# NathanBWaters/playaid_core

Hardware: AMD Instinct MI355X
Metric: 1080p frames/sec end-to-end (higher is better)
Workload: dtype f32; 1 GPU; configs[1]: 64 x 1080x1920 BGR frames per GPU per clip; parallelism=single GPU, lanes=2, ingest=raw BGR frames resident in HBM

## Files before the change

include/playaid_hip.h:

```cpp
#ifndef PLAYAID_HIP_H
#define PLAYAID_HIP_H

#include <stddef.h>
#include <stdint.h>

#ifdef __cplusplus
extern "C" {
#endif

#define PA_ABI_VERSION 15
#define PA_WEIGHT_MAGIC 0x31574150
#define PA_LSTM_MAGIC 0x314c4150
#define PA_ENCODER_MAGIC 0x31454150
#define PA_FEATURE_STRIDE 1024
#define PA_CROP 128

typedef enum pa_status {
    PA_OK = 0,
    PA_ERR_INVALID_ARG = -1,
    PA_ERR_HIP = -2,
    PA_ERR_BAD_WEIGHTS = -3,
    PA_ERR_CAPACITY = -4,
    PA_ERR_NO_DEVICE = -5,
    PA_ERR_NOT_READY = -6,
// ... 142 lines not shown
int pa_detector_layer_forms(const pa_detector* h, int32_t* forms, int32_t cap);

int pa_clean_detections(pa_engine* e, const float* dets, const int32_t* counts, int32_t n_labels, int32_t max_det, int32_t n_decoded_frames,
                        double* labels, int32_t* pixel_frame, double* pixel_box, int32_t* crop_kind, float* crop_row, int32_t* info4,
                        void* stream);

int pa_detector_plan(pa_engine* e, const int32_t* pixel_frame, const double* pixel_box, const int32_t* crop_kind, const int32_t* info4,
                     int32_t n_labels, int32_t* det_index, int32_t* src_own, int32_t* rep_entry, double* rep_boxes, int32_t* rep_src,
                     int32_t* words5, void* stream);
int pa_detector_plan_desc(pa_engine* e, pa_crop_image* desc, const int32_t* crop_kind, int32_t n_frames, int32_t step_frames,
                          long long region_bytes, const int32_t* rep_entry, int32_t n_rep, long long rep_base, void* stream);
int pa_square_crops_src(pa_engine* e, const uint8_t* frames, int32_t n_src, int32_t height, int32_t width, const double* boxes,
                        const int32_t* src_frame, int32_t n, int32_t padding, int32_t swap_rb, uint8_t* crops, int32_t* status, void* stream);

int pa_save_one_box_crops(pa_engine* e, const uint8_t* frames, int32_t n_src, int32_t height, int32_t width, const float* dets,
                          const int32_t* counts, int32_t max_det, const int32_t* det_index, const int32_t* src_frame, int32_t n,
                          int32_t jpeg_quality, uint8_t* images, size_t images_capacity, pa_crop_image* desc, void* stream);

int pa_project_boxes(pa_engine* e, const double* log_rows, int32_t n_rows, double* boxes, void* stream);


int pa_clip_begin(pa_engine* e, int32_t clip_frames);
int pa_clip_begin_batch(pa_engine* e, int32_t n_clips, int32_t clip_frames);

int pa_backbone_frames(pa_engine* e, const uint8_t* frames, int32_t n, int32_t height, int32_t width,
                       const double* boxes, int32_t frame0, uint8_t* crops_rgb, int32_t* status,
                       void* stream);

int pa_preprocess_frames(pa_engine* e, const uint8_t* frames, int32_t n, int32_t height, int32_t width,
                         const double* boxes, int32_t slot, uint8_t* crops_rgb, int32_t* status,
                         void* stream);
int pa_backbone_slot(pa_engine* e, int32_t slot, int32_t n, int32_t frame0, void* stream);


typedef struct pa_crop_window {
    int64_t offset;
    int32_t pitch;
    int32_t rows;
    int64_t src_offset;
    int32_t src_pitch;
    int32_t row_bytes;
} pa_crop_window;
int pa_upload_crop_windows(pa_engine* e, const uint8_t* frames_host, int32_t n, int32_t height, int32_t width,
                           const double* boxes_host, int32_t padding, uint8_t* windows_dev, size_t windows_capacity,
                           pa_crop_window* desc_host, pa_crop_window* desc_dev, size_t* bytes_used, void* stream);
int pa_preprocess_windows(pa_engine* e, const uint8_t* windows_dev, const pa_crop_window* desc_dev, int32_t n, int32_t height,
                          int32_t width, const double* boxes, int32_t slot, uint8_t* crops_rgb, int32_t* status, void* stream);


typedef struct pa_mjpeg pa_mjpeg;
int pa_mjpeg_create(int32_t device, int32_t max_frames, int32_t max_height, int32_t max_width, size_t max_bytes, pa_mjpeg** out);
void pa_mjpeg_destroy(pa_mjpeg* h);
const char* pa_mjpeg_last_error(const pa_mjpeg* h);
int pa_mjpeg_probe(const uint8_t* data_host, size_t nbytes, int32_t* info8, char* why, size_t why_bytes);
int pa_mjpeg_set_sync_rounds(pa_mjpeg* h, int32_t rounds);
int pa_mjpeg_last_sync_rounds(const pa_mjpeg* h);
int pa_mjpeg_set_groups(pa_mjpeg* h, int32_t groups);
int pa_mjpeg_debug_counters(unsigned long long* out8_host);
int pa_mjpeg_decode(pa_mjpeg* h, const uint8_t* data_host, const int64_t* spans_host, int32_t n, int32_t height, int32_t width,
                    int32_t rgb, uint8_t* frames_dev, int32_t* status_dev, void* stream);


typedef struct pa_jpeg_file {
    int64_t offset;
    int32_t nbytes;
    int32_t reserved;
} pa_jpeg_file;
typedef struct pa_jpegenc pa_jpegenc;
int pa_jpegenc_create(int32_t device, int32_t max_images, int64_t max_blocks, size_t scratch_bytes, pa_jpegenc** out);
void pa_jpegenc_destroy(pa_jpegenc* h);
const char* pa_jpegenc_last_error(const pa_jpegenc* h);
int pa_jpeg_header(int32_t height, int32_t width, int32_t quality, int32_t subsampling, uint8_t* out_host, size_t cap, int32_t* nbytes);
size_t pa_jpeg_file_bytes_bound(int32_t height, int32_t width, int32_t subsampling);
int pa_jpegenc_encode(pa_jpegenc* h, const uint8_t* images, size_t images_bytes, const pa_crop_image* desc, int32_t n, int32_t max_height,
                      int32_t max_width, int32_t bgr, int32_t quality, int32_t subsampling, uint8_t* files, size_t files_capacity,
                      pa_jpeg_file* out, void* stream);
int pa_jpegenc_overflows(pa_jpegenc* h, int32_t* count_host, void* stream);


typedef struct pa_jpegdec pa_jpegdec;
int pa_jpegdec_create(int32_t device, int32_t max_images, int64_t max_blocks, size_t max_bytes, pa_jpegdec** out);
void pa_jpegdec_destroy(pa_jpegdec* h);
const char* pa_jpegdec_last_error(const pa_jpegdec* h);
int pa_jpegdec_set_sync_rounds(pa_jpegdec* h, int32_t rounds);
int pa_jpegdec_plan(const uint8_t* data_host, const int64_t* spans_host, int32_t n, pa_crop_image* desc_host, size_t* images_bytes,
                    int64_t* blocks, char* why, size_t why_bytes);
int pa_jpegdec_decode(pa_jpegdec* h, const uint8_t* data_host, const int64_t* spans_host, int32_t n, int32_t bgr, uint8_t* images_dev,
                      size_t images_capacity, pa_crop_image* desc_dev, int32_t* status_dev, void* stream);

int pa_backbone_frames_indexed(pa_engine* e, const uint8_t* frames, int32_t n, int32_t height, int32_t width,
                               const double* boxes, const int32_t* frame_ids, uint8_t* crops_rgb,
                               int32_t* status, void* stream);
int pa_clip_mark_ready(pa_engine* e, const int32_t* frame_ids_host, int32_t n);
int pa_device_errors(pa_engine* e, int32_t* bad_frame_ids_host, void* stream);

int pa_backbone_frames_src(pa_engine* e, const uint8_t* frames, int32_t n_src, int32_t height, int32_t width,
                           const double* boxes, const int32_t* src_frame, int32_t n, int32_t frame0,
                           uint8_t* crops_rgb, int32_t* status, void* stream);

int pa_head_frames(pa_engine* e, int32_t frame_num_lo, int32_t frame_num_hi, pa_record* records,
                   float* logp, void* stream);

int pa_infer_clip(pa_engine* e, const uint8_t* frames, int32_t n, int32_t height, int32_t width,
                  const double* boxes, pa_record* records, float* logp, uint8_t* crops_rgb,
                  int32_t* status, void* stream);

int pa_features_export(pa_engine* e, int32_t frame0, int32_t n, float* feats, void* stream);
int pa_features_import(pa_engine* e, int32_t frame0, int32_t n, const float* feats, void* stream);

int pa_crop_resize_width(pa_engine* e, const uint8_t* frames, int32_t n, int32_t height, int32_t width, const int32_t* rects_host,
                         int32_t n_rects, int32_t out_w, uint8_t* out, int32_t out_h_cap, int32_t* out_h_host, void* stream);

int pa_backbone_windows(pa_engine* e, const float* x, int32_t n_crops, float* feats, void* stream);

#define PA_TRACE_STAGES 20
int pa_backbone_trace(pa_engine* e, const float* x, int32_t n_crops, int32_t stage, void* out, size_t out_bytes, void* aux,
                      size_t aux_bytes, void* stream);

typedef struct pa_lstm pa_lstm;
size_t pa_lstm_blob_bytes(int32_t input_dim, int32_t hidden_dim, int32_t num_layers, int32_t num_actions);
int pa_lstm_create(int32_t device, int32_t input_dim, int32_t hidden_dim, int32_t num_layers, int32_t num_actions,
                   int32_t max_rows, const void* blob_host, size_t blob_bytes, pa_lstm** out);
void pa_lstm_destroy(pa_lstm* h);
const char* pa_lstm_last_error(const pa_lstm* h);
int pa_lstm_forward(pa_lstm* h, const float* x, int32_t ld, int32_t seq_len, int32_t batch, float* logp, void* stream);
int pa_lstm_last_status(pa_lstm* h);
typedef enum pa_lstm_form {
    PA_LSTM_FORM_NOT_RUN = 0,
    PA_LSTM_FORM_STEPS = 1,
    PA_LSTM_FORM_U1 = 2,
    PA_LSTM_FORM_U2 = 3,
    PA_LSTM_FORM_U4 = 4,
    PA_LSTM_FORM_U8 = 5,
    PA_LSTM_FORM_MFMA = 6
} pa_lstm_form;
int pa_lstm_layer_forms(const pa_lstm* h, int32_t* forms, int32_t cap);

typedef struct pa_conv_desc {
    int32_t kind;
    int32_t cin, cout;
    int32_t ksize, stride;
    int32_t in_hw;
    int32_t in_buf, in_pad;
    int32_t out_buf, out_pad;
    int32_t res_buf;
    int32_t relu;
    int64_t w_off, b_off;
} pa_conv_desc;
typedef struct pa_convnet pa_convnet;
int pa_convnet_create(int32_t device, const pa_conv_desc* descs, int32_t n_descs, const int64_t* buf_floats_per_crop,
                      int32_t n_bufs, const float* weights_host, size_t n_weights, int32_t max_crops, pa_convnet** out);
int pa_convnet_create_dtype(int32_t device, const pa_conv_desc* descs, int32_t n_descs, const int64_t* buf_floats_per_crop,
                            int32_t n_bufs, const float* weights_host, size_t n_weights, int32_t max_crops, int32_t compute_dtype,
                            pa_convnet** out);
void pa_convnet_destroy(pa_convnet* h);
const char* pa_convnet_last_error(const pa_convnet* h);
int pa_convnet_forward(pa_convnet* h, const float* x, int32_t n, float* out, int32_t out_floats_per_crop, void* stream);
int pa_convnet_trace(pa_convnet* h, const float* x, int32_t n, int32_t last_row, int32_t buf, void* out, size_t out_bytes, void* stream);
typedef enum pa_cn_form {
    PA_CN_FORM_NOT_RUN = 0,
    PA_CN_FORM_STEM_POOL = 1,
    PA_CN_FORM_AVGPOOL = 2,
    PA_CN_FORM_WINO = 3,
    PA_CN_FORM_PATCH = 4,
    PA_CN_FORM_IGEMM_128x128 = 5,
    PA_CN_FORM_IGEMM_128x64 = 6,
    PA_CN_FORM_IGEMM_64x64 = 7,
    PA_CN_FORM_PSGEMM = 8,
    PA_CN_FORM_BGEMM = 9,
    PA_CN_FORM_BGEMM_SPLITK = 10,
    PA_CN_FORM_AVGPOOL_BF16 = 11
} pa_cn_form;
#define PA_CN_FORM_STEM_POOL_ANY 12
int pa_convnet_layer_forms(const pa_convnet* h, int32_t* forms, int32_t cap);

size_t pa_wino_weight_floats(int32_t cin, int32_t cout);
int pa_wino_channels_per_workgroup(int32_t cout, int64_t sub_blocks);
int pa_wino_transform_weights(const float* w_host, int32_t cin, int32_t cout, int32_t bn, float* ug_host);
int pa_wino_conv3x3(const float* x, const float* ug, const float* bias, const float* residual, float* out, int32_t n,
                    int32_t height, int32_t width, int32_t cin, int32_t cout, int32_t bn, int32_t in_px_stride,
                    int32_t out_px_stride, int32_t out_pad, int32_t act, int32_t res_after, void* stream);
int pa_wino_conv3x3_splitk(const float* x, const float* ug, const float* bias, const float* residual, float* out, int32_t n,
                           int32_t height, int32_t width, int32_t cin, int32_t cout, int32_t bn, int32_t in_px_stride, int32_t out_px_stride,
                           int32_t out_pad, int32_t act, int32_t res_after, float* slab, size_t slab_floats, int32_t* tickets,
                           int32_t n_tickets, void* stream);

size_t pa_conv_weight_bytes(int32_t cin, int32_t cout, int32_t ksize, int32_t compute_dtype, int32_t has_residual);
int pa_conv_pack_weights(const float* w_host, int32_t cin, int32_t cout, int32_t ksize, int32_t compute_dtype, int32_t has_residual,
                         void* out_host);
int pa_conv2d(const float* x, const void* w, const float* bias, const float* residual, float* out, int32_t n, int32_t height,
              int32_t width, int32_t cin, int32_t cout, int32_t ksize, int32_t stride, int32_t in_pad, int32_t in_px_stride,
              int32_t out_px_stride, int32_t out_pad, int32_t act, int32_t res_after, int32_t compute_dtype, void* stream);
int pa_conv2d_branch(const float* x, const void* w, const float* bias, const float* residual, float* out, const float* w2, float* out2,
                     int32_t n, int32_t height, int32_t width, int32_t cin, int32_t cout, int32_t ksize, int32_t stride, int32_t in_pad,
                     int32_t in_px_stride, int32_t out_px_stride, int32_t out_pad, int32_t act, int32_t res_after, int32_t compute_dtype,
                     void* stream);

int pa_stem_int_pack_weights(const float* w_host, uint16_t* out_host);
int pa_stem_int(const uint8_t* crops_u8, const void* w_slices, const float* bias, void* packed, float* out, int32_t n, void* stream);

typedef struct pa_encoder pa_encoder;
size_t pa_encoder_blob_bytes(int32_t in_dim, int32_t hidden_dim, int32_t slots, int32_t enc_dim, int32_t num_layers,
                             int32_t ff_dim, int32_t num_actions);
int pa_encoder_create(int32_t device, int32_t in_dim, int32_t hidden_dim, int32_t slots, int32_t enc_dim, int32_t num_heads,
                      int32_t num_layers, int32_t ff_dim, int32_t num_actions, int32_t max_rows, const void* blob_host,
                      size_t blob_bytes, pa_encoder** out);
void pa_encoder_destroy(pa_encoder* h);
const char* pa_encoder_last_error(const pa_encoder* h);
int pa_encoder_forward(pa_encoder* h, const float* feats, int32_t ld, int32_t seq_len, int32_t batch, float* logp, void* stream);


int pa_profile_enable(pa_engine* e, int32_t on);
int pa_profile_read(pa_engine* e, pa_kernel_stat* stats, int32_t max_stats, int32_t* n_stats);

int pa_set_crop_jpeg_quality(pa_engine* e, int32_t quality);

int pa_stream_spin(pa_engine* e, int32_t microseconds, void* stream);

int pa_stream_gate(pa_engine* e, int32_t max_microseconds, void* stream);
int pa_stream_gate_open(pa_engine* e);

int pa_stream_sync(pa_engine* e, void* stream);


typedef struct pa_eval pa_eval;
typedef struct pa_eval_totals {
    int64_t rows, correct, ignored, bad_labels;
    double nll_sum, conf_sum;
} pa_eval_totals;
#define PA_EVAL_IGNORE (-100)
int pa_eval_create(int32_t device, int32_t num_actions, pa_eval** out);
void pa_eval_destroy(pa_eval* h);
int pa_eval_reset(pa_eval* h, void* stream);
int pa_eval_update(pa_eval* h, const float* logp_dev, int32_t ld, int32_t n, const int32_t* labels_dev, int32_t label_stride,
                   void* stream);
int pa_eval_read(pa_eval* h, pa_eval_totals* totals_host, int64_t* confusion_host, void* stream);


#define PA_ANNOT_MAX_ITEMS 16
typedef struct pa_annot pa_annot;
typedef struct pa_annot_item {
    int32_t box[4];
    int32_t draw_box;
    int32_t line_width;
    int32_t has_color;
    int32_t text_off;
    int32_t text_len;
    uint8_t rgb[3];
    uint8_t reserved;
} pa_annot_item;
int pa_annot_create(int32_t device, const uint8_t* atlas_host, int32_t cell_w, int32_t cell_h, int32_t first_char, int32_t n_chars,
                    int32_t max_frames, int32_t max_items, int32_t max_text, pa_annot** out);
int pa_annotate_frames(pa_annot* h, const uint8_t* frames_in, int32_t n, int32_t height, int32_t width, const pa_annot_item* items_host,
                       const int32_t* counts_host, const uint8_t* text_host, int32_t text_bytes, int32_t pad_left, int32_t pad_right,
                       int32_t pad_bottom, uint8_t* frames_out, void* stream);
void pa_annot_destroy(pa_annot* h);


typedef struct pa_head_trainer pa_head_trainer;
typedef struct pa_adam_config {
    float lr, beta1, beta2, eps;
} pa_adam_config;
typedef struct pa_train_stats {
    float loss;
    int32_t valid;
    int32_t correct;
    int32_t pad;
} pa_train_stats;
#define PA_TRAIN_WEIGHTS 0
#define PA_TRAIN_M 1
#define PA_TRAIN_V 2
#define PA_TRAIN_RAW 16
int pa_head_trainer_create(pa_engine* e, const pa_adam_config* cfg, int32_t max_batch, pa_head_trainer** out);
void pa_head_trainer_destroy(pa_head_trainer* t);
const char* pa_head_trainer_last_error(const pa_head_trainer* t);
int64_t pa_head_trainer_steps(const pa_head_trainer* t);
int pa_head_train_step(pa_head_trainer* t, const float* feats, int32_t n_rows, const int32_t* gather, const int32_t* labels, int32_t batch,
                       int32_t apply, float* grads_out, pa_train_stats* stats_dev, void* stream);
int pa_head_trainer_read(pa_head_trainer* t, int32_t which, float* out_dev, size_t floats, void* stream);


typedef struct pa_lstm_trainer pa_lstm_trainer;
int pa_lstm_trainer_create(pa_lstm* h, const pa_adam_config* cfg, pa_lstm_trainer** out);
void pa_lstm_trainer_destroy(pa_lstm_trainer* t);
const char* pa_lstm_trainer_last_error(const pa_lstm_trainer* t);
int64_t pa_lstm_trainer_steps(const pa_lstm_trainer* t);
int pa_lstm_train_step(pa_lstm_trainer* t, const float* x, int32_t ld, int32_t seq_len, int32_t batch, const int32_t* labels, int32_t apply,
                       float* grads_out, pa_train_stats* stats_dev, void* stream);
int pa_lstm_trainer_read(pa_lstm_trainer* t, int32_t which, float* out_dev, size_t floats, void* stream);
size_t pa_lstm_trainer_floats(const pa_lstm* h);


typedef struct pa_encoder_trainer pa_encoder_trainer;
int pa_encoder_trainer_create(pa_encoder* h, const pa_adam_config* cfg, float dropout, uint64_t seed, pa_encoder_trainer** out);
void pa_encoder_trainer_destroy(pa_encoder_trainer* t);
const char* pa_encoder_trainer_last_error(const pa_encoder_trainer* t);
int64_t pa_encoder_trainer_steps(const pa_encoder_trainer* t);
int pa_encoder_train_step(pa_encoder_trainer* t, const float* feats, int32_t ld, int32_t seq_len, int32_t batch, const int32_t* labels,
                          int32_t apply, float* grads_out, pa_train_stats* stats_dev, void* stream);
int pa_encoder_trainer_read(pa_encoder_trainer* t, int32_t which, float* out_dev, size_t floats, void* stream);
size_t pa_encoder_trainer_floats(const pa_encoder* h);
int32_t pa_encoder_trainer_max_windows(const pa_encoder* h);

#ifdef __cplusplus
}
#endif
#endif
```

playaid_core_amd/_build.py:

```python
from __future__ import annotations

import os
import subprocess
import sys

HERE = os.path.dirname(os.path.abspath(__file__))
CSRC = os.path.join(HERE, "csrc")
LIB = os.path.join(HERE, "libplayaid_hip.so")
ARCH = "gfx950"

SOURCES = [
    ("igemm.hip", []),
    ("pigemm.hip", []),
    ("psgemm.hip", []),
    ("bgemm.hip", []),
    ("igemm_bf16.hip", []),
    ("patchconv.hip", []),
    ("patchconv_bf16.hip", []),
    ("wino.hip", []),
    ("stem.hip", []),
    ("stem_pool.hip", []),
    ("stem_pool_any.hip", []),
    ("misc.hip", []),
    ("preprocess.hip", ["-ffp-contract=off"]),
    ("crop_sized.hip", ["-ffp-contract=off"]),
    ("detect.hip", ["-ffp-contract=off"]),
    ("conv_rows.hip", []),
    ("lstm.hip", []),
    ("convnet.hip", []),
    ("transformer.hip", []),
    ("metrics.hip", []),
    ("jpeg.hip", ["-ffp-contract=off"]),
    ("mjpeg.hip", []),
    ("savebox.hip", ["-ffp-contract=off"]),
    ("jpegenc.hip", ["-ffp-contract=off"]),
    ("jpegdec.hip", []),
    ("yolo.hip", ["-ffp-contract=off"]),
    ("annotate.hip", []),
    ("head_train.hip", []),
    ("lstm_train.hip", []),
    ("encoder_train.hip", []),
    ("pa_api.hip", []),
]


def _newer(target: str, deps) -> bool:
    if not os.path.exists(target):
        return False
    t = os.path.getmtime(target)
    return all(os.path.getmtime(d) <= t for d in deps)


def build(force: bool = False, verbose: bool = False) -> str:
    hipcc = os.environ.get("HIPCC", "hipcc")
    headers = [os.path.join(CSRC, "pa_kernels.h"), os.path.join(CSRC, "gemm_tile.h"), os.path.join(CSRC, "engine_plan.h"), os.path.join(CSRC, "conv_rows.h"), os.path.join(CSRC, "pgemm_common.h"), os.path.join(CSRC, "tile_common.h"), os.path.join(CSRC, "crop_common.h"), os.path.join(CSRC, "jpeg_dct.h"), os.path.join(CSRC, "jpeg_entropy.h"), os.path.join(CSRC, "train_common.h"), os.path.join(CSRC, "lstm_handle.h"), os.path.join(CSRC, "encoder_handle.h"), os.path.join(HERE, "..", "include", "playaid_hip.h")]
    objs = []
    rebuilt = False
    for src, extra in SOURCES:
        s = os.path.join(CSRC, src)
        o = os.path.join(CSRC, src.replace(".hip", ".o"))
        objs.append(o)
        if force or not _newer(o, [s] + headers + [os.path.abspath(__file__)]):
            cmd = [hipcc, f"--offload-arch={ARCH}", "-O3", "-fPIC", "-std=c++17", "-c", s, "-o", o] + extra
            if verbose:
                print(" ".join(cmd), flush=True)
            subprocess.check_call(cmd)
            rebuilt = True
    if rebuilt or force or not _newer(LIB, objs):
        cmd = [hipcc, f"--offload-arch={ARCH}", "-shared", "-fPIC", "-o", LIB] + objs
        if verbose:
            print(" ".join(cmd), flush=True)
        subprocess.check_call(cmd)
    return LIB


if __name__ == "__main__":
    print(build(force="--force" in sys.argv, verbose=True))
```

playaid_core_amd/_lib.py:

```python
from __future__ import annotations

import ctypes as C
import os

HERE = os.path.dirname(os.path.abspath(__file__))
LIB_PATH = os.environ.get("PA_LIB_PATH") or os.path.join(HERE, "libplayaid_hip.so")

PA_ABI_VERSION = 15
PA_DTYPE_F32 = 0
PA_DTYPE_BF16 = 1
PA_DTYPE_EMULATED_F32 = 2
DTYPES = {"f32": PA_DTYPE_F32, "bf16": PA_DTYPE_BF16, "emulated_f32": PA_DTYPE_EMULATED_F32}
PA_WEIGHT_MAGIC = 0x31574150
PA_LSTM_MAGIC = 0x314C4150
PA_ENCODER_MAGIC = 0x31454150
PA_FEATURE_STRIDE = 1024
PA_TRACE_STAGES = 20
DET_FORMS = ("not_run", "stem_direct", "stem_bf16", "wino", "patch", "pgemm", "pgemm_up", "psgemm", "psgemm_up", "igemm", "sppf",
             "maxpool", "upsample", "absorbed", "decode", "bgemm", "bgemm_up")
CN_FORMS = ("not_run", "stem_pool", "avgpool", "wino", "patch", "igemm_128x128", "igemm_128x64", "igemm_64x64", "psgemm",
            "bgemm", "bgemm_splitk", "avgpool_bf16")
PA_CN_FORM_STEM_POOL_ANY = 12
CN_FORM_NAMES = CN_FORMS + ("stem_pool_any",)
LSTM_FORMS = ("not_run", "steps", "u1", "u2", "u4", "u8", "mfma")

PA_OK = 0
PA_ERR_INVALID_ARG = -1
PA_ERR_HIP = -2
PA_ERR_BAD_WEIGHTS = -3
PA_ERR_CAPACITY = -4
PA_ERR_NO_DEVICE = -5
PA_ERR_NOT_READY = -6
PA_ERR_BAD_LABELS = -7
PA_EVAL_IGNORE = -100
PA_ANNOT_MAX_ITEMS = 16
PA_TRAIN_WEIGHTS = 0
PA_TRAIN_M = 1
PA_TRAIN_V = 2
PA_TRAIN_RAW = 16

PA_CROP_OK = 0
PA_CROP_EMPTY = 1
PA_CROP_BAD_BOX = 2
PA_CROP_UPSCALE = 3
PA_CROP_FILTER_TOO_WIDE = 4
PA_CROP_BAD_FRAME = 5
PA_CROP_SIZE_MIN = 16
PA_CROP_SIZE_MAX = 512


class HipLibraryError(RuntimeError):
    pass


class pa_config(C.Structure):
    _fields_ = [
        ("abi_version", C.c_int32),
        ("device_id", C.c_int32),
        ("sequence_length", C.c_int32),
        ("frame_delta", C.c_int32),
        ("num_actions", C.c_int32),
        ("num_fighters", C.c_int32),
        ("crop_padding", C.c_int32),
        ("max_batch_frames", C.c_int32),
        ("max_clip_frames", C.c_int32),
        ("max_frame_height", C.c_int32),
        ("max_frame_width", C.c_int32),
        ("fighter_class_ids", C.c_int32 * 4),
        ("compute_dtype", C.c_int32),
    ]


class pa_record(C.Structure):
    _fields_ = [
        ("char_id", C.c_int32),
        ("action_id", C.c_int32),
        ("prob", C.c_float),
        ("status", C.c_int32),
    ]


class pa_crop_image(C.Structure):
    _fields_ = [("offset", C.c_int64), ("height", C.c_int32), ("width", C.c_int32)]


class pa_jpeg_file(C.Structure):
    _fields_ = [("offset", C.c_int64), ("nbytes", C.c_int32), ("reserved", C.c_int32)]


class pa_crop_window(C.Structure):
    _fields_ = [("offset", C.c_int64), ("pitch", C.c_int32), ("rows", C.c_int32), ("src_offset", C.c_int64),
                ("src_pitch", C.c_int32), ("row_bytes", C.c_int32)]


class pa_conv_desc(C.Structure):
    _fields_ = [(n, C.c_int32) for n in ("kind", "cin", "cout", "ksize", "stride", "in_hw", "in_buf", "in_pad", "out_buf", "out_pad",
                                        "res_buf", "relu")] + [("w_off", C.c_int64), ("b_off", C.c_int64)]


class pa_net_layer(C.Structure):
    _fields_ = [(n, C.c_int32) for n in ("kind", "cin", "cout", "ksize", "stride", "in_h", "in_w", "in_buf", "in_coff", "in_cstride", "in_pad",
                                        "out_buf", "out_coff", "out_cstride", "out_pad", "res_buf", "res_coff", "act", "res_after",
                                        "reserved")] + [("w_off", C.c_int64), ("b_off", C.c_int64), ("aux", C.c_float * 8)]


class pa_eval_totals(C.Structure):
    _fields_ = [("rows", C.c_int64), ("correct", C.c_int64), ("ignored", C.c_int64), ("bad_labels", C.c_int64),
                ("nll_sum", C.c_double), ("conf_sum", C.c_double)]


class pa_annot_item(C.Structure):
    _fields_ = [("box", C.c_int32 * 4), ("draw_box", C.c_int32), ("line_width", C.c_int32), ("has_color", C.c_int32),
                ("text_off", C.c_int32), ("text_len", C.c_int32), ("rgb", C.c_uint8 * 3), ("reserved", C.c_uint8)]


class pa_adam_config(C.Structure):
    _fields_ = [("lr", C.c_float), ("beta1", C.c_float), ("beta2", C.c_float), ("eps", C.c_float)]


class pa_train_stats(C.Structure):
    _fields_ = [("loss", C.c_float), ("valid", C.c_int32), ("correct", C.c_int32), ("pad", C.c_int32)]


class pa_kernel_stat(C.Structure):
    _fields_ = [
        ("name", C.c_char * 48),
        ("launches", C.c_int32),
        ("total_ms", C.c_float),
        ("flops", C.c_double),
        ("bytes", C.c_double),
        ("flops_executed", C.c_double),
    ]


_P = C.c_void_p
SYMBOLS = [
    ("pa_create", C.c_int, [C.POINTER(pa_config), _P, C.c_size_t, C.POINTER(_P)]),
    ("pa_create_from_arena", C.c_int, [C.POINTER(pa_config), _P, C.c_size_t, C.POINTER(_P)]),
    ("pa_weights_arena_bytes", C.c_size_t, [_P]),
    ("pa_weights_export", C.c_int, [_P, _P, C.c_size_t, _P]),
    ("pa_destroy", None, [_P]),
    ("pa_last_error", C.c_char_p, [_P]),
    ("pa_status_string", C.c_char_p, [C.c_int]),
    ("pa_abi_version", C.c_int, []),
    ("pa_weight_blob_bytes", C.c_size_t, [C.c_int, C.c_int]),
    ("pa_infer_windows", C.c_int, [_P, _P, C.c_int32, _P, _P]),
    ("pa_square_crops", C.c_int, [_P, _P, C.c_int32, C.c_int32, C.c_int32, _P, C.c_int32, C.c_int32, _P, _P, _P]),
    ("pa_square_crops_sized", C.c_int, [_P, _P, C.c_int32, C.c_int32, C.c_int32, _P, C.c_int32, C.c_int32, C.c_int32, _P, _P, _P]),
    ("pa_runner_inputs", C.c_int, [_P, _P, C.c_size_t, _P, C.c_int32, C.c_int32, _P, _P, _P]),
    ("pa_backbone_crop_images", C.c_int, [_P, _P, C.c_size_t, _P, C.c_int32, C.c_int32, _P, _P, _P]),
    ("pa_detect_postprocess", C.c_int, [_P, _P, C.c_int32, C.c_int32, C.c_int32, C.c_float, C.c_float, C.c_uint32, C.c_int32,
                                        C.c_int32, C.c_int32, C.c_int32, C.c_int32, _P, _P, _P]),
    ("pa_detect_postprocess_classes", C.c_int, [_P, _P, C.c_int32, C.c_int32, C.c_int32, C.c_float, C.c_float, _P, C.c_int32,
                                                C.c_int32, C.c_int32, C.c_int32, C.c_int32, _P, _P, _P]),
    ("pa_detector_create", C.c_int, [C.c_int32, C.POINTER(pa_net_layer), C.c_int32, C.POINTER(C.c_int64), C.c_int32, _P, C.c_size_t,
                                     C.c_int32, C.c_int32, C.c_int32, C.c_int32, C.POINTER(_P)]),
    ("pa_detector_create_dtype", C.c_int, [C.c_int32, C.POINTER(pa_net_layer), C.c_int32, C.POINTER(C.c_int64), C.c_int32, _P, C.c_size_t,
                                           C.c_int32, C.c_int32, C.c_int32, C.c_int32, C.c_int32, C.POINTER(_P)]),
    ("pa_detector_destroy", None, [_P]),
    ("pa_detector_last_error", C.c_char_p, [_P]),
    ("pa_detector_rows", C.c_int, [_P]),
    ("pa_detector_forward", C.c_int, [_P, _P, C.c_int32, C.c_int32, C.c_int32, _P, _P]),
    ("pa_detector_forward_timed", C.c_int, [_P, _P, C.c_int32, C.c_int32, C.c_int32, _P, _P, _P, C.c_int32]),
    ("pa_detector_trace", C.c_int, [_P, _P, C.c_int32, C.c_int32, C.c_int32, C.c_int32, C.c_int32, C.c_int32, C.c_int32, _P, C.c_size_t, _P,
                                    _P, _P]),
    ("pa_detector_layer_forms", C.c_int, [_P, _P, C.c_int32]),
    ("pa_clean_detections", C.c_int, [_P, _P, _P, C.c_int32, C.c_int32, C.c_int32, _P, _P, _P, _P, _P, _P, _P]),
    ("pa_save_one_box_crops", C.c_int, [_P, _P, C.c_int32, C.c_int32, C.c_int32, _P, _P, C.c_int32, _P, _P, C.c_int32, C.c_int32, _P,
                                        C.c_size_t, _P, _P]),
    ("pa_project_boxes", C.c_int, [_P, _P, C.c_int32, _P, _P]),
    ("pa_clip_begin", C.c_int, [_P, C.c_int32]),
    ("pa_clip_begin_batch", C.c_int, [_P, C.c_int32, C.c_int32]),
    ("pa_backbone_frames", C.c_int, [_P, _P, C.c_int32, C.c_int32, C.c_int32, _P, C.c_int32, _P, _P, _P]),
    ("pa_preprocess_frames", C.c_int, [_P, _P, C.c_int32, C.c_int32, C.c_int32, _P, C.c_int32, _P, _P, _P]),
    ("pa_backbone_slot", C.c_int, [_P, C.c_int32, C.c_int32, C.c_int32, _P]),
    ("pa_upload_crop_windows", C.c_int, [_P, _P, C.c_int32, C.c_int32, C.c_int32, _P, C.c_int32, _P, C.c_size_t, _P, _P,
                                         C.POINTER(C.c_size_t), _P]),
    ("pa_preprocess_windows", C.c_int, [_P, _P, _P, C.c_int32, C.c_int32, C.c_int32, _P, C.c_int32, _P, _P, _P]),
    ("pa_backbone_frames_indexed", C.c_int, [_P, _P, C.c_int32, C.c_int32, C.c_int32, _P, _P, _P, _P, _P]),
    ("pa_clip_mark_ready", C.c_int, [_P, _P, C.c_int32]),
    ("pa_device_errors", C.c_int, [_P, C.POINTER(C.c_int32), _P]),
    ("pa_backbone_frames_src", C.c_int, [_P, _P, C.c_int32, C.c_int32, C.c_int32, _P, _P, C.c_int32, C.c_int32, _P, _P, _P]),
    ("pa_head_frames", C.c_int, [_P, C.c_int32, C.c_int32, _P, _P, _P]),
    ("pa_infer_clip", C.c_int, [_P, _P, C.c_int32, C.c_int32, C.c_int32, _P, _P, _P, _P, _P, _P]),
    ("pa_features_export", C.c_int, [_P, C.c_int32, C.c_int32, _P, _P]),
    ("pa_features_import", C.c_int, [_P, C.c_int32, C.c_int32, _P, _P]),
    ("pa_profile_enable", C.c_int, [_P, C.c_int32]),
    ("pa_profile_read", C.c_int, [_P, C.POINTER(pa_kernel_stat), C.c_int32, C.POINTER(C.c_int32)]),
    ("pa_set_crop_jpeg_quality", C.c_int, [_P, C.c_int32]),
    ("pa_stream_spin", C.c_int, [_P, C.c_int32, _P]),
    ("pa_stream_gate", C.c_int, [_P, C.c_int32, _P]),
    ("pa_stream_gate_open", C.c_int, [_P]),
    ("pa_stream_sync", C.c_int, [_P, _P]),
    ("pa_backbone_windows", C.c_int, [_P, _P, C.c_int32, _P, _P]),
    ("pa_backbone_trace", C.c_int, [_P, _P, C.c_int32, C.c_int32, _P, C.c_size_t, _P, C.c_size_t, _P]),
    ("pa_lstm_blob_bytes", C.c_size_t, [C.c_int32, C.c_int32, C.c_int32, C.c_int32]),
    ("pa_lstm_create", C.c_int, [C.c_int32, C.c_int32, C.c_int32, C.c_int32, C.c_int32, C.c_int32, _P, C.c_size_t, C.POINTER(_P)]),
    ("pa_lstm_destroy", None, [_P]),
    ("pa_lstm_last_error", C.c_char_p, [_P]),
    ("pa_lstm_last_status", C.c_int, [_P]),
    ("pa_lstm_forward", C.c_int, [_P, _P, C.c_int32, C.c_int32, C.c_int32, _P, _P]),
    ("pa_lstm_layer_forms", C.c_int, [_P, _P, C.c_int32]),
    ("pa_convnet_create", C.c_int, [C.c_int32, C.POINTER(pa_conv_desc), C.c_int32, C.POINTER(C.c_int64), C.c_int32, _P, C.c_size_t,
                                    C.c_int32, C.POINTER(_P)]),
    ("pa_convnet_create_dtype", C.c_int, [C.c_int32, C.POINTER(pa_conv_desc), C.c_int32, C.POINTER(C.c_int64), C.c_int32, _P, C.c_size_t,
                                          C.c_int32, C.c_int32, C.POINTER(_P)]),
    ("pa_convnet_destroy", None, [_P]),
    ("pa_convnet_last_error", C.c_char_p, [_P]),
    ("pa_convnet_forward", C.c_int, [_P, _P, C.c_int32, _P, C.c_int32, _P]),
    ("pa_convnet_trace", C.c_int, [_P, _P, C.c_int32, C.c_int32, C.c_int32, _P, C.c_size_t, _P]),
    ("pa_convnet_layer_forms", C.c_int, [_P, _P, C.c_int32]),
    ("pa_detector_plan", C.c_int, [_P] * 5 + [C.c_int32] + [_P] * 7),
    ("pa_detector_plan_desc", C.c_int, [_P, _P, _P, C.c_int32, C.c_int32, C.c_longlong, _P, C.c_int32, C.c_longlong, _P]),
    ("pa_square_crops_src", C.c_int, [_P, _P, C.c_int32, C.c_int32, C.c_int32, _P, _P, C.c_int32, C.c_int32, C.c_int32, _P, _P, _P]),
    ("pa_wino_weight_floats", C.c_size_t, [C.c_int32, C.c_int32]),
    ("pa_wino_channels_per_workgroup", C.c_int, [C.c_int32, C.c_int64]),
    ("pa_wino_transform_weights", C.c_int, [_P, C.c_int32, C.c_int32, C.c_int32, _P]),
    ("pa_wino_conv3x3", C.c_int, [_P, _P, _P, _P, _P] + [C.c_int32] * 11 + [_P]),
    ("pa_conv_weight_bytes", C.c_size_t, [C.c_int32] * 5),
    ("pa_conv_pack_weights", C.c_int, [_P] + [C.c_int32] * 5 + [_P]),
    ("pa_conv2d", C.c_int, [_P, _P, _P, _P, _P] + [C.c_int32] * 14 + [_P]),
    ("pa_conv2d_branch", C.c_int, [_P, _P, _P, _P, _P, _P, _P] + [C.c_int32] * 14 + [_P]),
    ("pa_stem_int_pack_weights", C.c_int, [_P, _P]),
    ("pa_stem_int", C.c_int, [_P, _P, _P, _P, _P, C.c_int32, _P]),
    ("pa_wino_conv3x3_splitk", C.c_int, [_P, _P, _P, _P, _P] + [C.c_int32] * 11 + [_P, C.c_size_t, _P, C.c_int32, _P]),
    ("pa_crop_resize_width", C.c_int, [_P, _P, C.c_int32, C.c_int32, C.c_int32, C.POINTER(C.c_int32), C.c_int32, C.c_int32, _P, C.c_int32,
                                       C.POINTER(C.c_int32), _P]),
    ("pa_encoder_blob_bytes", C.c_size_t, [C.c_int32] * 7),
    ("pa_encoder_create", C.c_int, [C.c_int32] * 10 + [_P, C.c_size_t, C.POINTER(_P)]),
    ("pa_encoder_destroy", None, [_P]),
    ("pa_encoder_last_error", C.c_char_p, [_P]),
    ("pa_encoder_forward", C.c_int, [_P, _P, C.c_int32, C.c_int32, C.c_int32, _P, _P]),
    ("pa_mjpeg_create", C.c_int, [C.c_int32, C.c_int32, C.c_int32, C.c_int32, C.c_size_t, C.POINTER(_P)]),
    ("pa_mjpeg_destroy", None, [_P]),
    ("pa_mjpeg_last_error", C.c_char_p, [_P]),
    ("pa_mjpeg_probe", C.c_int, [_P, C.c_size_t, C.POINTER(C.c_int32), C.c_char_p, C.c_size_t]),
    ("pa_mjpeg_set_sync_rounds", C.c_int, [_P, C.c_int32]),
    ("pa_mjpeg_set_groups", C.c_int, [_P, C.c_int32]),
    ("pa_mjpeg_last_sync_rounds", C.c_int, [_P]),
    ("pa_mjpeg_debug_counters", C.c_int, [_P]),
    ("pa_mjpeg_decode", C.c_int, [_P, _P, _P, C.c_int32, C.c_int32, C.c_int32, C.c_int32, _P, _P, _P]),
    ("pa_jpegenc_create", C.c_int, [C.c_int32, C.c_int32, C.c_int64, C.c_size_t, C.POINTER(_P)]),
    ("pa_jpegenc_destroy", None, [_P]),
    ("pa_jpegenc_last_error", C.c_char_p, [_P]),
    ("pa_jpeg_header", C.c_int, [C.c_int32, C.c_int32, C.c_int32, C.c_int32, _P, C.c_size_t, C.POINTER(C.c_int32)]),
    ("pa_jpeg_file_bytes_bound", C.c_size_t, [C.c_int32, C.c_int32, C.c_int32]),
    ("pa_jpegenc_encode", C.c_int, [_P, _P, C.c_size_t, _P, C.c_int32, C.c_int32, C.c_int32, C.c_int32, C.c_int32, C.c_int32, _P, C.c_size_t,
                                    _P, _P]),
    ("pa_jpegenc_overflows", C.c_int, [_P, C.POINTER(C.c_int32), _P]),
    ("pa_jpegdec_create", C.c_int, [C.c_int32, C.c_int32, C.c_int64, C.c_size_t, C.POINTER(_P)]),
    ("pa_jpegdec_destroy", None, [_P]),
    ("pa_jpegdec_last_error", C.c_char_p, [_P]),
    ("pa_jpegdec_set_sync_rounds", C.c_int, [_P, C.c_int32]),
    ("pa_jpegdec_plan", C.c_int, [_P, _P, C.c_int32, _P, C.POINTER(C.c_size_t), C.POINTER(C.c_int64), C.c_char_p, C.c_size_t]),
    ("pa_jpegdec_decode", C.c_int, [_P, _P, _P, C.c_int32, C.c_int32, _P, C.c_size_t, _P, _P, _P]),
    ("pa_eval_create", C.c_int, [C.c_int32, C.c_int32, C.POINTER(_P)]),
    ("pa_eval_destroy", None, [_P]),
    ("pa_eval_reset", C.c_int, [_P, _P]),
    ("pa_eval_update", C.c_int, [_P, _P, C.c_int32, C.c_int32, _P, C.c_int32, _P]),
    ("pa_eval_read", C.c_int, [_P, C.POINTER(pa_eval_totals), _P, _P]),
    ("pa_annot_create", C.c_int, [C.c_int32, _P] + [C.c_int32] * 7 + [C.POINTER(_P)]),
    ("pa_annotate_frames", C.c_int, [_P, _P, C.c_int32, C.c_int32, C.c_int32, _P, _P, _P] + [C.c_int32] * 4 + [_P, _P]),
    ("pa_annot_destroy", None, [_P]),
    ("pa_head_trainer_create", C.c_int, [_P, C.POINTER(pa_adam_config), C.c_int32, C.POINTER(_P)]),
    ("pa_head_trainer_destroy", None, [_P]),
    ("pa_head_trainer_last_error", C.c_char_p, [_P]),
    ("pa_head_trainer_steps", C.c_int64, [_P]),
    ("pa_head_train_step", C.c_int, [_P, _P, C.c_int32, _P, _P, C.c_int32, C.c_int32, _P, _P, _P]),
    ("pa_head_trainer_read", C.c_int, [_P, C.c_int32, _P, C.c_size_t, _P]),
    ("pa_lstm_trainer_create", C.c_int, [_P, C.POINTER(pa_adam_config), C.POINTER(_P)]),
    ("pa_lstm_trainer_destroy", None, [_P]),
    ("pa_lstm_trainer_last_error", C.c_char_p, [_P]),
    ("pa_lstm_trainer_steps", C.c_int64, [_P]),
    ("pa_lstm_train_step", C.c_int, [_P, _P, C.c_int32, C.c_int32, C.c_int32, _P, C.c_int32, _P, _P, _P]),
    ("pa_lstm_trainer_read", C.c_int, [_P, C.c_int32, _P, C.c_size_t, _P]),
    ("pa_lstm_trainer_floats", C.c_size_t, [_P]),
    ("pa_encoder_trainer_create", C.c_int, [_P, C.POINTER(pa_adam_config), C.c_float, C.c_uint64, C.POINTER(_P)]),
    ("pa_encoder_trainer_destroy", None, [_P]),
    ("pa_encoder_trainer_last_error", C.c_char_p, [_P]),
    ("pa_encoder_trainer_steps", C.c_int64, [_P]),
    ("pa_encoder_train_step", C.c_int, [_P, _P, C.c_int32, C.c_int32, C.c_int32, _P, C.c_int32, _P, _P, _P]),
    ("pa_encoder_trainer_read", C.c_int, [_P, C.c_int32, _P, C.c_size_t, _P]),
    ("pa_encoder_trainer_floats", C.c_size_t, [_P]),
    ("pa_encoder_trainer_max_windows", C.c_int32, [_P]),
]

_lib = None


def load() -> C.CDLL:
    global _lib
    if _lib is not None:
        return _lib
    import torch

    if not os.path.exists(LIB_PATH):
        raise HipLibraryError(
            f"{LIB_PATH} not found: build it with `python -m playaid_core_amd._build` "
            "(hipcc, --offload-arch=gfx950). There is no CPU fallback for this path."
        )
    try:
        lib = C.CDLL(LIB_PATH)
    except OSError as exc:
        raise HipLibraryError(f"cannot load {LIB_PATH}: {exc}") from exc
    for name, restype, argtypes in SYMBOLS:
        try:
            fn = getattr(lib, name)
        except AttributeError as exc:
            raise HipLibraryError(f"{LIB_PATH} does not export {name}") from exc
        fn.restype = restype
        fn.argtypes = argtypes
    if lib.pa_abi_version() != PA_ABI_VERSION:
        raise HipLibraryError("libplayaid_hip.so ABI version mismatch; rebuild it")
    _lib = lib
    return lib
```

playaid_core_amd/csrc/engine_plan.h:

```cpp
#pragma once
#include "gemm_tile.h"

#include <algorithm>
#include <cstddef>
#include <cstdlib>

namespace pa {

struct EngineKnobs {
    int patch = 1;
    int bf16_patch = 1;
    int bf16_t256 = 1;
    int s2_pgemm = 2;
    int stem_igemm = 0;
    int stem_pool = 1;
    int pool_overlap = 1;
    int ds_side = 0;
    int stem_int = 1;
    int wino = 1;
    int wino_min_hw = 4;
    int wino_ds = 1;
    int bf16_ds_fuse = 1;
    int f32_ds_fuse = 1;
    bool profile_layers = false;
    int force_tile = -1;
    int force_splitk = 0;
    int fc_splitk = 0;
    int head_splitk = 0;
    int interleave = 0;
};

inline int env_int(const char* name, int unset) {
    const char* v = getenv(name);
    return v ? atoi(v) : unset;
}
inline int env_min1(const char* name) {
    const char* v = getenv(name);
    return v ? std::max(1, atoi(v)) : 0;
}

inline EngineKnobs engine_knobs() {
    static const EngineKnobs once = [] {
        EngineKnobs k;
        k.patch = env_int("PA_PATCH", k.patch);
        k.bf16_patch = env_int("PA_BF16_PATCH", k.bf16_patch);
        k.bf16_t256 = env_int("PA_BF16_T256", k.bf16_t256);
        k.s2_pgemm = env_int("PA_S2_PGEMM", k.s2_pgemm);
        k.stem_igemm = env_int("PA_STEM_IGEMM", k.stem_igemm);
        k.stem_pool = env_int("PA_STEM_POOL", k.stem_pool);
        k.pool_overlap = env_int("PA_POOL_OVERLAP", k.pool_overlap);
        k.ds_side = env_int("PA_DS_SIDE", k.ds_side);
        k.stem_int = env_int("PA_STEM_INT", k.stem_int);
        k.wino = env_int("PA_WINO", k.wino);
        k.wino_min_hw = env_int("PA_WINO_MIN_HW", k.wino_min_hw);
        k.wino_ds = env_int("PA_WINO_DS", k.wino_ds);
        k.bf16_ds_fuse = env_int("PA_BF16_DS_FUSE", k.bf16_ds_fuse);
        k.f32_ds_fuse = env_int("PA_F32_DS_FUSE", k.f32_ds_fuse);
        return k;
    }();
    EngineKnobs k = once;
    const char* pl = getenv("PA_PROFILE_LAYERS");
    k.profile_layers = pl && pl[0] == '1';
    k.force_tile = env_int("PA_FORCE_TILE", -1);
    k.force_splitk = env_min1("PA_FORCE_SPLITK");
    k.fc_splitk = env_min1("PA_FC_SPLITK");
    k.head_splitk = env_min1("PA_HEAD_SPLITK");
    k.interleave = env_int("PA_INTERLEAVE", 0);
    return k;
}

enum ComputeDtype { DT_F32, DT_EMULATED_F32, DT_BF16 };

struct EngineForms {
    bool stem_fused;
    bool stem_int;
    bool opener_branch;
};
inline EngineForms engine_forms(const EngineKnobs& k, ComputeDtype dt) {
    EngineForms f;
    f.stem_fused = k.stem_pool && !k.stem_igemm;
    f.stem_int = dt != DT_BF16 && k.stem_int && f.stem_fused;
    f.opener_branch = dt == DT_BF16 ? k.bf16_ds_fuse != 0 : dt == DT_F32 && k.f32_ds_fuse && !k.ds_side && k.s2_pgemm;
    return f;
}

enum BranchPlace {
    BRANCH_NONE,
    BRANCH_SECOND_K,
    BRANCH_OWN_GEMM,
    BRANCH_OPENER,
    BRANCH_OPENER_PROBE,
};
enum BranchLaunch {
    BL_NONE,
    BL_SECOND_K,
    BL_GEMM_BEFORE,
    BL_STORED,
    BL_ON_OPENER,
    BL_GEMM_BEHIND,
};

struct LayerDesc {
    int cin = 0, cout = 0, kh = 0, kw = 0, stride = 1;
    int in_hw = 0, out_hw = 0;
    int in_pad = 0, out_pad = 0;
    int off = 0;
    int taps = 0, kw_taps = 0, chunk = 0;
    int in_px_stride = 0;
    int relu = 1;
    double k_alg = 0;
    GemmTile tile = TILE_128x64;
    int splitk = 1;
    bool forced = false;
    bool adds_residual = false;
    bool wino = false;
    bool split = false;
    struct {
        BranchPlace place = BRANCH_NONE;
        int c = 0, hw = 0, stride = 1;
        bool split = false;
    } branch;
    BranchPlace carries = BRANCH_NONE;
};

inline void choose_tile(int M, int N, int nk, GemmTile* tile, int* splitk) {
    *tile = im2col_tile(M, N);
    const int tm = (M + 127) / 128;
    const int tiles = *tile == TILE_128x128 ? tm * (N / 128) : *tile == TILE_128x64 ? tm * (N / 64) : ((M + 63) / 64) * (N / 64);
    int sk = 1;
    while (tiles * sk < 512 && nk / (sk * 2) >= 8) sk *= 2;
    *splitk = sk;
}

inline LayerDesc conv_desc(const EngineKnobs& k, ComputeDtype dt, int max_crops, int cin, int cout, int ksize, int stride, int in_hw, bool residual) {
    LayerDesc L;
    L.cin = cin; L.cout = cout; L.kh = L.kw = ksize; L.stride = stride;
    L.in_hw = in_hw; L.out_hw = in_hw / stride;
    L.adds_residual = residual;
    if (ksize == 7) {
        L.in_pad = 3; L.out_pad = 1; L.off = 0;
        L.taps = 7; L.kw_taps = 1; L.chunk = 32; L.in_px_stride = 4;
    } else if (ksize == 3) {
        L.in_pad = 1; L.out_pad = 1; L.off = 0;
        L.taps = 9; L.kw_taps = 3; L.chunk = cin; L.in_px_stride = cin;
    } else {
        L.in_pad = 1; L.out_pad = 1; L.off = 1;
        L.taps = 1; L.kw_taps = 1; L.chunk = cin; L.in_px_stride = cin;
    }
    L.k_alg = (double)cin * ksize * ksize;
    choose_tile(max_crops * L.out_hw * L.out_hw, cout, L.taps * L.chunk / ((dt == DT_BF16 && ksize == 3) ? 64 : 32), &L.tile, &L.splitk);
    if (k.force_tile >= 0 && k.force_tile <= 4 && !(k.force_tile == 0 && cout % 128 != 0)) { L.tile = (GemmTile)k.force_tile; L.forced = true; }
    if (k.force_splitk) { L.splitk = k.force_splitk; L.forced = true; }
    return L;
}

inline LayerDesc fc_desc(const EngineKnobs& k, int n_pad) {
    LayerDesc L;
    L.cin = 512; L.cout = n_pad; L.kh = L.kw = 1;
    L.in_hw = L.out_hw = 1;
    L.taps = 1; L.kw_taps = 1; L.chunk = 512; L.in_px_stride = 512;
    L.relu = 0;
    L.k_alg = 512.0 * 1000.0 / n_pad;
    L.tile = TILE_64x64;
    L.splitk = k.fc_splitk ? k.fc_splitk : 4;
    L.forced = true;
    return L;
}

inline bool wino_layer(const EngineKnobs& k, ComputeDtype dt, const LayerDesc& L) {
    return dt != DT_BF16 && L.kh == 3 && L.stride == 1 && k.wino && L.out_hw >= k.wino_min_hw && L.out_hw % 4 == 0;
}

inline bool opener_can_carry(const LayerDesc& opener, const LayerDesc& conv2, bool same_input, bool extras) {
    return same_input && opener.stride == 2 && opener.cout == conv2.cout && opener.out_hw == conv2.out_hw && opener.out_pad == conv2.out_pad &&
           opener.chunk == conv2.branch.c && !opener.forced && extras;
}

inline BranchPlace place_branch(const EngineKnobs& k, ComputeDtype dt, const LayerDesc& opener, const LayerDesc& conv2, bool same_input, int li) {
    if (dt != DT_BF16 && !conv2.wino) return BRANCH_SECOND_K;
    const bool extras = dt == DT_BF16 ? opener.chunk % 64 == 0
                                      : li < 3 && opener.kh == 3 && opener.cin == conv2.branch.c && opener.in_hw == conv2.branch.hw && opener.in_pad == 1;
    if (!engine_forms(k, dt).opener_branch || !opener_can_carry(opener, conv2, same_input, extras)) return BRANCH_OWN_GEMM;
    return dt == DT_BF16 && k.bf16_ds_fuse == 2 ? BRANCH_OPENER_PROBE : BRANCH_OPENER;
}

enum ConvForm { CONV_PSGEMM, CONV_BF16_PATCH, CONV_BF16_IM2COL, CONV_WINO, CONV_PATCH, CONV_PGEMM, CONV_IM2COL };

struct LaunchAccount {
    double flops = 0, bytes = 0;
    double flops_executed = 0;
};

struct BranchPlan {
    GemmTile tile = TILE_128x64;
    bool psgemm = false;
    LaunchAccount acct;
};
inline BranchPlan plan_branch(bool bf, bool psgemm, int ncrops, int M, int N, int hw, int c, int stride) {
    BranchPlan b;
    b.psgemm = psgemm;
    int sk;
    if (!bf) choose_tile(M, N, c / 32, &b.tile, &sk);
    b.acct.flops = b.acct.flops_executed = 2.0 * M * N * c;
    b.acct.bytes = (bf ? 2.0 : 4.0) * ((double)ncrops * hw * hw * c / (stride * stride) + (double)M * N + (double)N * c);
    return b;
}

inline BranchPlan plan_branch(ComputeDtype dt, const LayerDesc& conv2, int ncrops) {
    return plan_branch(dt == DT_BF16, dt == DT_EMULATED_F32 && conv2.branch.split, ncrops, ncrops * conv2.out_hw * conv2.out_hw, conv2.cout,
                       conv2.branch.hw, conv2.branch.c, conv2.branch.stride);
}

struct ConvPlan {
    ConvForm form = CONV_IM2COL;
    int M = 0, N = 0, ktot = 0;
    GemmTile tile = TILE_64x64;
    int splitk = 1;
    bool tile_256 = false;
    int patch_bm = 0;
    int pgemm_bm = 0;
    BranchLaunch branch = BL_NONE;
    LaunchAccount acct;
    BranchPlan branch_gemm;
};

inline ConvPlan plan_conv(const EngineKnobs& k, ComputeDtype dt, const LayerDesc& L, int ncrops, size_t slab_floats, bool branch_on_side) {
    ConvPlan P;
    const bool bf = dt == DT_BF16 && L.kh == 3;
    const bool emu = dt == DT_EMULATED_F32;
    const BranchPlace place = L.branch.place;
    const bool stored = place == BRANCH_OWN_GEMM || place == BRANCH_OPENER || place == BRANCH_OPENER_PROBE;
    P.M = ncrops * L.out_hw * L.out_hw;
    P.N = L.cout;
    P.ktot = L.taps * L.chunk;
    if (place == BRANCH_OPENER || (stored && !bf && branch_on_side)) {
        P.branch = BL_STORED;
    } else if (stored) {
        P.branch = BL_GEMM_BEFORE;
        P.branch_gemm = plan_branch(dt, L, ncrops);
    } else if (place == BRANCH_SECOND_K) {
        P.branch = BL_SECOND_K;
        P.ktot += L.branch.c;
    }
    const bool second_k = P.branch == BL_SECOND_K, has_residual = L.adds_residual || stored;
    P.tile = L.tile;
    P.splitk = L.splitk;
    if (!L.forced) choose_tile(P.M, P.N, P.ktot / (bf ? 64 : 32), &P.tile, &P.splitk);
    if ((size_t)P.splitk * P.M * P.N > slab_floats) P.splitk = 1;
    const bool f32_opener = !bf && !emu && L.carries == BRANCH_OPENER;
    const bool f32_here = f32_opener && P.splitk <= 1;
    const bool bf_opener = bf && L.carries == BRANCH_OPENER;
    const bool branch_here = bf_opener || f32_here;
    if (bf && L.carries != BRANCH_NONE) {
        P.tile = (P.N % 128 == 0 && ((P.M + 127) / 128) * (P.N / 128) >= 256) ? TILE_128x128 : TILE_128x64;
        P.splitk = 1;
    }
    const double es = bf ? 2 : 4;
    const double k_main = (stored ? L.k_alg - L.branch.c : L.k_alg) + (branch_here ? L.cin : 0);
    P.acct.flops = P.acct.flops_executed = 2.0 * P.M * P.N * k_main;
    P.acct.bytes = es * ((double)ncrops * L.in_hw * L.in_hw * L.cin + (double)P.M * P.N * ((has_residual || branch_here) ? 2 : 1) + (double)P.N * k_main +
                         (second_k ? (double)ncrops * L.branch.hw * L.branch.hw * L.branch.c : 0.0));
    if (emu && L.split && !second_k && !has_residual) {
        P.form = CONV_PSGEMM;
    } else if (bf) {
        P.form = (k.bf16_patch && L.stride == 1 && !second_k) ? CONV_BF16_PATCH : CONV_BF16_IM2COL;
        P.tile_256 = k.bf16_t256 && !bf_opener && P.tile == TILE_128x128 && P.splitk == 1 && ((P.M + 255) / 256) * (P.N / 128) >= 256;
    } else if (L.wino && !second_k) {
        P.form = CONV_WINO;
        P.acct.flops_executed = P.acct.flops * 4.0 / 9.0;
    } else if (k.patch && L.kh == 3 && L.stride == 1) {
        P.form = CONV_PATCH;
        P.patch_bm = P.tile == TILE_64x64 || P.tile == TILE_64x64_K64 ? 64 : 128;
        const int howo = L.out_hw * L.out_hw, in_w2 = L.out_hw + 2;
        const int px128 = howo >= 128 ? (128 / L.out_hw + 2) * in_w2 : (128 / howo) * in_w2 * in_w2;
        if (P.patch_bm == 128 && px128 > 224) P.patch_bm = 64;
    } else if (k.s2_pgemm && L.kh == 3 && L.stride == 2 && !second_k && !has_residual && P.splitk <= 1) {
        P.form = CONV_PGEMM;
        P.pgemm_bm = k.s2_pgemm == 2 ? 64 : 0;
    }
    if (bf_opener || (f32_here && P.form == CONV_PGEMM)) P.branch = BL_ON_OPENER;
    else if (f32_opener) P.branch = BL_GEMM_BEHIND;
    if (f32_opener) P.branch_gemm = plan_branch(false, false, ncrops, P.M, P.N, L.in_hw, L.cin, L.stride);
    return P;
}

}
```

playaid_core_amd/csrc/pa_api.hip:

```cpp
#include "../../include/playaid_hip.h"
#include "conv_rows.h"
#include "engine_plan.h"
#include "train_common.h"

#include <algorithm>
#include <cmath>
#include <cstdio>
#include <cstdlib>
#include <cstring>
#include <string>
#include <vector>

using namespace pa;

namespace {

constexpr int WINO_TICKETS = 4096;

struct ConvLayer : LayerDesc {
    std::string name;
    float* in = nullptr;
    float* out = nullptr;
    float* residual = nullptr;
    float* wgt = nullptr;
    float* wino_wgt = nullptr;
    int wino_bn = 0;
    float* bias = nullptr;
    unsigned short* split_wgt = nullptr;
    struct {
        float* src = nullptr;
        float* wgt = nullptr;
        float* out = nullptr;
        unsigned short* split_wgt = nullptr;
    } ds;
    int carries_of = -1;
};

struct ProfEntry {
    int name_id;
    hipEvent_t start, stop;
    double flops, bytes;
    double flops_executed;
};

}

struct pa_engine {
    pa_config cfg;
    std::string last_error;
    int max_crops = 0;
    EngineKnobs knobs;
    ComputeDtype dtype = DT_F32;
    bool emu = false;
    bool bf16 = false;
    int cache_rows = 0;
    int clip_frames = 0;
    int sub_frames = 0;
    int* gate_flag = nullptr;
    int jpeg_quality = 0;
    int32_t* jpeg_qtab = nullptr;
    uint8_t* crops_tmp = nullptr;
    std::vector<char> ready;
    std::vector<void*> allocs;
    uint8_t* arena = nullptr;
    size_t arena_cap = 0, arena_used = 0;
    std::vector<uint8_t> arena_stage;
    bool adopt = false;
    int32_t* dev_errors = nullptr;
    int32_t* savebox_rects = nullptr;
    double* clean_g6 = nullptr;
    size_t clean_g6_cap = 0;
    float* x0 = nullptr;
    float* x0_slot[2] = {nullptr, nullptr};
    bool stem_int = false;
    uint16_t* xi_slot[2] = {nullptr, nullptr};
    int slot_form[2] = {0, 0};
    uint16_t* stem_wgt_int = nullptr;
    int32_t* pre_status[2] = {nullptr, nullptr};
    float* pooled = nullptr;
    float* feats_tmp = nullptr;
    float* cache = nullptr;
    int32_t* cache_status = nullptr;
    float* h1 = nullptr;
    int32_t* gather = nullptr;
    int gather_key[4] = {-1, -1, -1, -1};
    float* slab = nullptr;
    size_t slab_floats = 0;
    float* wino_tickets = nullptr;
    std::vector<ConvLayer> convs;
    ConvLayer fc;
    float* stem_wgt_bf16 = nullptr;
    float* c1 = nullptr;
    float* p1 = nullptr;
    float* layer4_out = nullptr;
    float* w1d = nullptr;
    float* b1d = nullptr;
    float *w2 = nullptr, *b2 = nullptr, *w3 = nullptr, *b3 = nullptr;
    GemmTile head_tile = TILE_64x64;
    int head_splitk = 16;
    CropPlan* plans = nullptr;
    int32_t* coef = nullptr;
    int coef_dim = 0;
    int32_t* coef_cache = nullptr;
    int coef_cache_pad = -1, coef_cache_dmax = 0;
    AreaTabPacked* area_tabs = nullptr;
    uint8_t* hop = nullptr;
    uint8_t *t1 = nullptr, *t2 = nullptr;
    size_t t_stride = 0;
    int32_t* status_tmp = nullptr;
    int32_t* fallback = nullptr;
    hipStream_t side = nullptr;
    hipEvent_t ev_fork = nullptr, ev_join = nullptr;
    hipEvent_t ev_ds_fork = nullptr, ev_ds_join = nullptr;
    bool profiling = false;
    std::vector<std::string> prof_names;
    std::vector<ProfEntry> prof_log;
    std::vector<hipEvent_t> event_pool;
};

namespace {

int fail(pa_engine* e, int code, const std::string& msg) {
    if (e) e->last_error = msg;
    return code;
}

float* slot_dst(pa_engine* e, int slot) {
    e->slot_form[slot] = e->stem_int ? 2 : 0;
    return e->stem_int ? reinterpret_cast<float*>(e->xi_slot[slot]) : e->x0_slot[slot];
}
const float* slot_src(const pa_engine* e, int slot) {
    return e->slot_form[slot] == 2 ? reinterpret_cast<const float*>(e->xi_slot[slot]) : e->x0_slot[slot];
}
int input_form(const pa_engine* e, const void* x) {
    if (x && e->stem_int && (x == e->xi_slot[0] || x == e->xi_slot[1])) return 2;
    return e->bf16 ? 1 : 0;
}

#define HIPCHK(e, call)                                                                              \
    do {                                                                                             \
        hipError_t err__ = (call);                                                                   \
        if (err__ != hipSuccess)                                                                     \
            return fail((e), PA_ERR_HIP, std::string(#call) + ": " + hipGetErrorString(err__));      \
    } while (0)

template <typename T>
int dev_alloc(pa_engine* e, T** ptr, size_t count, bool zero) {
    void* p = nullptr;
    size_t bytes = count * sizeof(T);
    if (bytes == 0) bytes = sizeof(T);
    HIPCHK(e, hipMalloc(&p, bytes));
    e->allocs.push_back(p);
    if (zero) HIPCHK(e, hipMemset(p, 0, bytes));
    *ptr = reinterpret_cast<T*>(p);
    return PA_OK;
}

int arena_put(pa_engine* e, void** dst, const void* host, size_t bytes) {
    const size_t off = (e->arena_used + 255) & ~(size_t)255;
    if (off + bytes > e->arena_cap) return fail(e, PA_ERR_BAD_WEIGHTS, "weight arena overflow");
    e->arena_used = off + bytes;
    *dst = e->arena + off;
    if (!e->adopt) memcpy(e->arena_stage.data() + off, host, bytes);
    return PA_OK;
}

int upload(pa_engine* e, float** dst, const std::vector<float>& host) {
    return arena_put(e, reinterpret_cast<void**>(dst), host.data(), host.size() * sizeof(float));
}

int upload_bf16(pa_engine* e, float** dst, const std::vector<float>& host) {
    std::vector<uint16_t> h(host.size());
    if (!e->adopt)
        for (size_t i = 0; i < host.size(); ++i) h[i] = bf16_rne(host[i]);
    return arena_put(e, reinterpret_cast<void**>(dst), h.data(), h.size() * sizeof(uint16_t));
}

int upload_split(pa_engine* e, unsigned short** dst, const std::vector<float>& host, int cout, int ktot, bool residual) {
    std::vector<unsigned short> h(psgemm_weight_elems(cout, ktot, residual), 0);
    if (h.empty()) return PA_ERR_INVALID_ARG;
    if (!e->adopt) psgemm_pack_weights(host.data(), cout, ktot, residual, h.data());
    return arena_put(e, reinterpret_cast<void**>(dst), h.data(), h.size() * sizeof(unsigned short));
}

struct BlobReader {
    const float* base;
    size_t pos, limit;
    bool dry;
    const float* take(size_t n) {
        if (pos + n > limit) return nullptr;
        const float* r = dry ? base : base + pos;
        pos += n;
        return r;
    }
};

size_t blob_float_count(int S, int A) {
    size_t n = 0;
    auto conv = [&](int co, int ci, int k) { n += (size_t)co * ci * k * k; };
    auto bn = [&](int c) { n += 4 * (size_t)c; };
    conv(64, 3, 7);
    bn(64);
    int cin = 64;
    const int widths[4] = {64, 128, 256, 512};
    for (int li = 0; li < 4; ++li) {
        const int co = widths[li];
        for (int b = 0; b < 2; ++b) {
            const int ci = b == 0 ? cin : co;
            conv(co, ci, 3);
            bn(co);
            conv(co, co, 3);
            bn(co);
            if (b == 0 && li > 0) {
                conv(co, ci, 1);
                bn(co);
            }
        }
        cin = co;
    }
    n += 1000 * 512 + 1000;
    n += (size_t)512 * 1000 * S + 512;
    n += 128 * 512 + 128;
    n += (size_t)A * 128 + A;
    return n;
}

bool fold_conv(BlobReader& br, const ConvLayer& L, std::vector<float>& w_out, std::vector<float>& b_out) {
    const size_t wn = (size_t)L.cout * L.cin * L.kh * L.kw;
    const float* w = br.take(wn);
    const float* gamma = br.take(L.cout);
    const float* beta = br.take(L.cout);
    const float* mean = br.take(L.cout);
    const float* var = br.take(L.cout);
    if (!w || !gamma || !beta || !mean || !var) return false;
    const int ktot = L.taps * L.chunk;
    w_out.assign((size_t)L.cout * ktot, 0.f);
    b_out.assign(L.cout, 0.f);
    if (br.dry) return true;
    const bool stem = (L.kh == 7);
    for (int co = 0; co < L.cout; ++co) {
        const double scale = (double)gamma[co] / std::sqrt((double)var[co] + 1e-5);
        b_out[co] = (float)((double)beta[co] - (double)mean[co] * scale);
        for (int ci = 0; ci < L.cin; ++ci)
            for (int ky = 0; ky < L.kh; ++ky)
                for (int kx = 0; kx < L.kw; ++kx) {
                    const double v = (double)w[(((size_t)co * L.cin + ci) * L.kh + ky) * L.kw + kx] * scale;
                    size_t k;
                    if (stem)
                        k = (size_t)ky * L.chunk + kx * 4 + ci;
                    else
                        k = (size_t)(ky * L.kw + kx) * L.chunk + ci;
                    w_out[(size_t)co * ktot + k] = (float)v;
                }
    }
    return true;
}

int prof_name_id(pa_engine* e, const char* name) {
    for (size_t i = 0; i < e->prof_names.size(); ++i)
        if (e->prof_names[i] == name) return (int)i;
    e->prof_names.push_back(name);
    return (int)e->prof_names.size() - 1;
}

hipEvent_t get_event(pa_engine* e) {
    if (!e->event_pool.empty()) {
        hipEvent_t ev = e->event_pool.back();
        e->event_pool.pop_back();
        return ev;
    }
    hipEvent_t ev;
    if (hipEventCreate(&ev) != hipSuccess) return nullptr;
    return ev;
}

struct ProfScope {
    pa_engine* e;
    hipStream_t s;
    ProfEntry ent;
    bool on;
    ProfScope(pa_engine* e_, hipStream_t s_, const char* name, double flops, double bytes, double executed = -1.0)
        : e(e_), s(s_), on(e_->profiling) {
        if (!on) return;
        ent.name_id = prof_name_id(e, name);
        ent.flops = flops;
        ent.flops_executed = executed >= 0.0 ? executed : flops;
        ent.bytes = bytes;
        ent.start = get_event(e);
        ent.stop = get_event(e);
        if (!ent.start || !ent.stop) {
            on = false;
            return;
        }
        (void)hipEventRecord(ent.start, s);
    }
    ~ProfScope() {
        if (!on) return;
        (void)hipEventRecord(ent.stop, s);
        e->prof_log.push_back(ent);
    }
};

float* buf_at(float* base, size_t elems, bool bf) { return reinterpret_cast<float*>(reinterpret_cast<char*>(base) + elems * (bf ? 2 : 4)); }

bool branch_on_side(const pa_engine* e, hipStream_t s) { return e->knobs.ds_side && !e->profiling && !e->bf16 && e->side && s != e->side; }

int run_branch_gemm(pa_engine* e, const ConvLayer& L, const BranchPlan& b, int crop0, int ncrops, size_t slab_off, hipStream_t s, const char* prof_name) {
    const int hw = L.branch.hw, c = L.branch.c, out_w = L.out_hw + 2 * L.out_pad;
    const size_t out_crop = (size_t)out_w * out_w * L.cout;
    GemmParams d = conv_row_params({ ncrops,  hw, hw, 1, c,
                                     c, L.cout, 1, L.branch.stride,
                                     L.out_pad, L.cout,  0, 0});
    d.act = buf_at(L.ds.src, (size_t)crop0 * (hw + 2) * (hw + 2) * c, e->bf16);
    d.wgt = L.ds.wgt;
    d.out = buf_at(L.ds.out, crop0 * out_crop, e->bf16);
    d.slab = e->slab + slab_off;
    ProfScope ps(e, s, prof_name, b.acct.flops, b.acct.bytes);
    if (e->bf16) HIPCHK(e, launch_igemm_bf16(d, b.tile, s));
    else if (b.psgemm) HIPCHK(e, launch_psgemm(d, L.ds.split_wgt, (size_t)ncrops * out_crop, 0, s));
    else HIPCHK(e, launch_igemm(d, b.tile, s));
    return PA_OK;
}

int run_conv(pa_engine* e, const ConvLayer& L, int crop0, int ncrops, size_t slab_off, hipStream_t s, const char* prof_name) {
    const size_t slab_avail = e->slab_floats > slab_off ? e->slab_floats - slab_off : 0;
    const ConvPlan P = plan_conv(e->knobs, e->dtype, L, ncrops, slab_avail, branch_on_side(e, s));
    const bool bf = e->bf16 && L.kh == 3;
    const int in_w = L.in_hw + 2 * L.in_pad;
    const int out_w = L.out_hw + 2 * L.out_pad;
    const size_t in_crop = (size_t)in_w * in_w * L.in_px_stride;
    const size_t out_crop = (size_t)out_w * out_w * L.cout;
    GemmParams p;
    memset(&p, 0, sizeof(p));
    p.act = buf_at(L.in, crop0 * in_crop, bf);
    p.wgt = L.wgt;
    p.bias = L.bias;
    p.residual = L.residual ? buf_at(L.residual, crop0 * out_crop, bf) : nullptr;
    p.out = buf_at(L.out, crop0 * out_crop, bf);
    p.slab = e->slab + slab_off;
    p.gather = nullptr;
    p.M = P.M;
    p.N = P.N;
    p.taps = L.taps;
    p.kw_taps = L.kw_taps;
    p.chunk = L.chunk;
    p.ktot = P.ktot;
    p.skip_w = L.kh == 7;
    p.howo = L.out_hw * L.out_hw;
    p.wo = L.out_hw;
    p.in_px_stride = L.in_px_stride;
    p.in_row_stride = in_w * L.in_px_stride;
    p.in_img_stride = (int)in_crop;
    p.stride = L.stride;
    p.off_y = L.off;
    p.off_x = L.off;
    p.out_px_stride = L.cout;
    p.out_row_stride = out_w * L.cout;
    p.out_img_stride = (int)out_crop;
    p.out_pad = L.out_pad;
    p.relu = L.relu;
    p.splitk = P.splitk;
    if (P.branch == BL_GEMM_BEFORE) {
        const int rc = run_branch_gemm(e, L, P.branch_gemm, crop0, ncrops, slab_off, s, prof_name);
        if (rc) return rc;
    }
    if (P.branch == BL_GEMM_BEFORE || P.branch == BL_STORED) {
        p.residual = buf_at(L.ds.out, crop0 * out_crop, bf);
    } else if (P.branch == BL_SECOND_K) {
        const int w2 = L.branch.hw + 2;
        p.act2 = buf_at(L.ds.src, (size_t)crop0 * w2 * w2 * L.branch.c, bf);
        p.k2_steps = L.branch.c / (bf ? 64 : 32);
        p.in2_px_stride = L.branch.c;
        p.in2_row_stride = w2 * L.branch.c;
        p.in2_img_stride = w2 * w2 * L.branch.c;
        p.stride2 = L.branch.stride;
        p.off2 = 1;
    }
    const ConvLayer* C2 = L.carries_of >= 0 ? &e->convs[L.carries_of] : nullptr;
    if (bf && P.branch == BL_ON_OPENER) {
        p.wgt2 = C2->ds.wgt;
        p.out2 = buf_at(C2->ds.out, crop0 * out_crop, bf);
    }
    bool branch_left = P.branch == BL_GEMM_BEHIND;
    {
        ProfScope ps(e, s, prof_name, P.acct.flops, P.acct.bytes, P.acct.flops_executed);
        hipError_t pe = hipErrorInvalidValue;
        if (P.form == CONV_PSGEMM) {
            pe = launch_psgemm(p, L.split_wgt, (size_t)ncrops * out_crop, 0, s);
        } else if (P.form == CONV_WINO) {
            WinoParams q = wino_params(p, ncrops, L.out_hw, L.out_hw, L.cin, L.wino_wgt, L.wino_bn);
            if (e->wino_tickets && e->slab) {
                q.slab = e->slab + slab_off;
                q.slab_floats = e->slab_floats > slab_off ? std::min(e->slab_floats - slab_off, e->slab_floats / 2) : 0;
                q.tickets = reinterpret_cast<int32_t*>(e->wino_tickets) + (slab_off ? WINO_TICKETS : 0);
                q.tickets_cap = WINO_TICKETS;
            }
            pe = launch_wino3x3(q, s);
        } else if (bf) {
            if (P.form == CONV_BF16_PATCH) pe = launch_conv3x3_bf16_patch(p, s);
            if (pe == hipErrorInvalidValue) pe = launch_igemm_bf16(p, P.tile_256 ? TILE_256x128 : P.tile, s);
        } else {
            if (P.form == CONV_PATCH) pe = launch_conv3x3_patch(p, P.patch_bm, s);
            if (P.form == CONV_PGEMM && P.branch == BL_ON_OPENER) {
                p.wgt2 = C2->ds.wgt;
                p.out2 = buf_at(C2->ds.out, crop0 * out_crop, bf);
                pe = launch_pgemm(p, 64, s);
                branch_left = pe != hipSuccess;
                p.wgt2 = nullptr;
                p.out2 = nullptr;
            }
            if (P.form == CONV_PGEMM && pe == hipErrorInvalidValue) pe = launch_pgemm(p, P.pgemm_bm, s);
            if (pe == hipErrorInvalidValue) pe = launch_igemm(p, P.tile, s);
        }
        HIPCHK(e, pe);
    }
    if (branch_left) return run_branch_gemm(e, *C2, P.branch_gemm, crop0, ncrops, slab_off, s, e->knobs.profile_layers ? C2->name.c_str() : prof_name);
    return PA_OK;
}

int run_backbone_part(pa_engine* e, int crop0, int ncrops, const float* x_in, float* feats_out, size_t slab_off, hipStream_t s,
                      int stop = PA_TRACE_STAGES) {
    int rc;
    ConvLayer stem = e->convs[0];
    stem.in = const_cast<float*>(x_in);
    const EngineKnobs& K = e->knobs;
    auto stem_part = [&](int c0, int n, hipStream_t st) -> int {
        if (K.stem_igemm && !e->bf16) return run_conv(e, stem, c0, n, slab_off, st, "igemm_conv7x7_stem");
        StemParams sp;
        memset(&sp, 0, sizeof(sp));
        sp.x = x_in + (size_t)c0 * 134 * 134 * 4;
        sp.wgt = stem.wgt;
        sp.bias = stem.bias;
        sp.out = reinterpret_cast<float*>(reinterpret_cast<char*>(e->c1) + (size_t)c0 * 66 * 66 * 64 * (e->bf16 ? 2 : 4));
        sp.tiles = n * 32;
        sp.out_bf16 = e->bf16 ? 1 : 0;
        const double px = (double)n * 64 * 64;
        ProfScope ps(e, st, "stem_conv7x7", 2.0 * px * 64 * 147, 4.0 * ((double)n * 128 * 128 * 3 + px * 64 + 64.0 * 147));
        HIPCHK(e, launch_stem7x7(sp, st));
        return PA_OK;
    };
    auto pool_part = [&](int c0, int n, hipStream_t st) -> int {
        ProfScope ps(e, st, "maxpool3x3", 0.0, (e->bf16 ? 2.0 : 4.0) * n * (64.0 * 64 * 64 + 32.0 * 32 * 64));
        if (e->bf16)
            HIPCHK(e, launch_maxpool_bf16(reinterpret_cast<uint16_t*>(e->c1) + (size_t)c0 * 66 * 66 * 64,
                                          reinterpret_cast<uint16_t*>(e->p1) + (size_t)c0 * 34 * 34 * 64, n, st));
        else
            HIPCHK(e, launch_maxpool(e->c1 + (size_t)c0 * 66 * 66 * 64, e->p1 + (size_t)c0 * 34 * 34 * 64, n, st));
        return PA_OK;
    };
    const int x_form = input_form(e, x_in);
    if (engine_forms(K, e->dtype).stem_fused) {
        StemPoolParams sp;
        memset(&sp, 0, sizeof(sp));
        const size_t es_in = x_form ? 2 : 4, es_out = e->bf16 ? 2 : 4;
        sp.x = reinterpret_cast<const char*>(x_in) + (size_t)crop0 * 134 * 134 * 4 * es_in;
        sp.wgt = x_form == 2 ? (const void*)e->stem_wgt_int : e->bf16 ? (const void*)e->stem_wgt_bf16 : (const void*)stem.wgt;
        sp.bias = stem.bias;
        sp.out = reinterpret_cast<char*>(e->p1) + (size_t)crop0 * 34 * 34 * 64 * es_out;
        sp.crops = ncrops;
        sp.in_bf16 = x_form;
        sp.out_bf16 = e->bf16 ? 1 : 0;
        const double px = (double)ncrops * 64 * 64;
        ProfScope ps(e, s, "stem_conv7x7_pool", 2.0 * px * 64 * 147,
                     (double)es_in * ((double)ncrops * 128 * 128 * 4 + 64.0 * 147 * (x_form == 2 ? 3 : 1)) + (double)es_out * ncrops * 32 * 32 * 64);
        HIPCHK(e, launch_stem_pool(sp, s));
    } else if (x_form == 2) {
        return fail(e, PA_ERR_INVALID_ARG, "integer pixels reached an unfused stem (PA_STEM_POOL=0 / PA_STEM_IGEMM=1 switch the integer stem off)");
    } else if (e->bf16) {
        return fail(e, PA_ERR_INVALID_ARG, "the bf16 path has no unfused stem (PA_STEM_POOL=0 / PA_STEM_IGEMM=1 are fp32 A/B knobs)");
    } else if (K.pool_overlap && !e->profiling && !K.interleave && e->side && s != e->side && ncrops >= 64) {
        const int half = (ncrops / 2 + 7) & ~7;
        if ((rc = stem_part(crop0, half, s))) return rc;
        HIPCHK(e, hipEventRecord(e->ev_fork, s));
        HIPCHK(e, hipStreamWaitEvent(e->side, e->ev_fork, 0));
        if ((rc = pool_part(crop0, half, e->side))) return rc;
        HIPCHK(e, hipEventRecord(e->ev_join, e->side));
        if ((rc = stem_part(crop0 + half, ncrops - half, s))) return rc;
        if ((rc = pool_part(crop0 + half, ncrops - half, s))) return rc;
        HIPCHK(e, hipStreamWaitEvent(s, e->ev_join, 0));
    } else {
        if ((rc = stem_part(crop0, ncrops, s))) return rc;
        if ((rc = pool_part(crop0, ncrops, s))) return rc;
    }
    if (stop <= 1) return PA_OK;
    const bool on_side = branch_on_side(e, s);
    for (size_t i = 1; i < e->convs.size(); ++i) {
        const ConvLayer& L = e->convs[i];
        const char* pn = K.profile_layers ? L.name.c_str() : (L.kh == 3 ? "igemm_conv3x3" : "igemm_conv1x1_ds");
        const bool side_next = on_side && i + 1 < e->convs.size() && e->convs[i + 1].branch.place == BRANCH_OWN_GEMM;
        if (side_next) {
            const ConvLayer& Nx = e->convs[i + 1];
            HIPCHK(e, hipEventRecord(e->ev_ds_fork, s));
            HIPCHK(e, hipStreamWaitEvent(e->side, e->ev_ds_fork, 0));
            if ((rc = run_branch_gemm(e, Nx, plan_branch(e->dtype, Nx, ncrops), crop0, ncrops, slab_off, e->side, "igemm_conv1x1_ds"))) return rc;
            HIPCHK(e, hipEventRecord(e->ev_ds_join, e->side));
        }
        if (on_side && L.branch.place == BRANCH_OWN_GEMM) HIPCHK(e, hipStreamWaitEvent(s, e->ev_ds_join, 0));
        if ((rc = run_conv(e, L, crop0, ncrops, slab_off, s, pn))) return rc;
        if (stop <= (int)i + 1) {
            if (side_next) HIPCHK(e, hipStreamWaitEvent(s, e->ev_ds_join, 0));
            return PA_OK;
        }
    }
    {
        ProfScope ps(e, s, "avgpool", 0.0, ncrops * ((e->bf16 ? 2.0 : 4.0) * 16.0 * 512 + 4.0 * 512));
        if (e->bf16)
            HIPCHK(e, launch_avgpool_bf16(reinterpret_cast<uint16_t*>(e->layer4_out) + (size_t)crop0 * 36 * 512,
                                          e->pooled + (size_t)crop0 * 512, ncrops, s));
        else
            HIPCHK(e, launch_avgpool(e->layer4_out + (size_t)crop0 * 36 * 512, e->pooled + (size_t)crop0 * 512, ncrops, s));
    }
    if (stop <= 18) return PA_OK;
    ConvLayer fc = e->fc;
    fc.out = feats_out;
    rc = run_conv(e, fc, crop0, ncrops, slab_off, s, "igemm_fc");
    return rc;
}

int run_backbone(pa_engine* e, int ncrops, const float* x_in, float* feats_out, hipStream_t s, int stop = PA_TRACE_STAGES) {
    if (!e->knobs.interleave || ncrops < 64 || !e->side) return run_backbone_part(e, 0, ncrops, x_in, feats_out, 0, s, stop);
    const int half = (ncrops / 2 + 7) & ~7;
    HIPCHK(e, hipEventRecord(e->ev_fork, s));
    HIPCHK(e, hipStreamWaitEvent(e->side, e->ev_fork, 0));
    int rc = run_backbone_part(e, 0, half, x_in, feats_out, 0, s, stop);
    if (rc) return rc;
    rc = run_backbone_part(e, half, ncrops - half, x_in, feats_out, e->slab_floats / 2, e->side, stop);
    if (rc) return rc;
    HIPCHK(e, hipEventRecord(e->ev_join, e->side));
    HIPCHK(e, hipStreamWaitEvent(s, e->ev_join, 0));
    return PA_OK;
}

int run_head(pa_engine* e, int nwin, const float* feats, const int32_t* gather, const int32_t* crop_status,
             pa_record* records, float* logp, hipStream_t s) {
    const int S = e->cfg.sequence_length;
    GemmParams p;
    memset(&p, 0, sizeof(p));
    p.act = feats;
    p.wgt = e->w1d;
    p.bias = e->b1d;
    p.out = e->h1;
    p.slab = e->slab;
    p.gather = gather;
    p.M = nwin;
    p.N = 512;
    p.taps = S;
    p.kw_taps = 1;
    p.chunk = PA_FEATURE_STRIDE;
    p.ktot = S * PA_FEATURE_STRIDE;
    p.howo = 1;
    p.wo = 1;
    p.in_px_stride = PA_FEATURE_STRIDE;
    p.out_px_stride = 512;
    p.out_row_stride = 512;
    p.out_img_stride = 512;
    p.relu = 1;
    p.splitk = e->head_splitk;
    if ((size_t)p.splitk * p.M * p.N > e->slab_floats) p.splitk = 1;
    int32_t splitk_used = 1;
    p.defer_reduce = 1;
    p.splitk_used = &splitk_used;
    {
        ProfScope ps(e, s, "igemm_conv1d_head", 2.0 * nwin * 512.0 * 1000.0 * S,
                     4.0 * (512.0 * 1000 * S + (double)nwin * S * 1000 + nwin * 512.0));
        HIPCHK(e, launch_igemm(p, e->head_tile, s));
    }
    HeadParams h;
    memset(&h, 0, sizeof(h));
    h.h1 = splitk_used > 1 ? nullptr : e->h1;
    h.slab = e->slab;
    h.b1 = e->b1d;
    h.splitk = splitk_used;
    h.w2 = e->w2;
    h.b2 = e->b2;
    h.w3 = e->w3;
    h.b3 = e->b3;
    h.logp = logp;
    h.records = records;
    h.crop_status = crop_status;
    h.gather = gather;
    h.nwin = nwin;
    h.num_actions = e->cfg.num_actions;
    h.fighters = e->cfg.num_fighters;
    h.seq = S;
    for (int i = 0; i < 4; ++i) h.class_ids[i] = e->cfg.fighter_class_ids[i];
    {
        ProfScope ps(e, s, "head_mlp_logsoftmax", 2.0 * nwin * (512.0 * 128 + 128.0 * e->cfg.num_actions),
                     4.0 * (nwin * 512.0 + 512.0 * 128 + 128.0 * e->cfg.num_actions));
        HIPCHK(e, launch_head_mlp(h, s));
    }
    return PA_OK;
}

int run_preprocess(pa_engine* e, const uint8_t* frames, int n, int height, int width, const double* boxes, int padding,
                   int swap_rb, uint8_t* crops_u8, float* crops_f32, int32_t* status, hipStream_t s,
                   const int32_t* src_frame = nullptr, int n_src = 0, const pa_crop_window* windows = nullptr) {
    PreprocParams p;
    memset(&p, 0, sizeof(p));
    p.frames = frames;
    p.windows = reinterpret_cast<const CropWindow*>(windows);
    p.boxes = boxes;
    p.src_frame = src_frame;
    p.n_src = src_frame ? n_src : n;
    p.n_frames = n;
    p.height = height;
    p.width = width;
    p.fighters = e->cfg.num_fighters;
    p.padding = padding;
    p.swap_rb = swap_rb;
    p.plans = e->plans;
    p.coef = e->coef;
    p.coef_dim = e->coef_dim;
    p.coef_cache = e->coef_cache_pad == padding ? e->coef_cache : nullptr;
    p.coef_cache_pad = padding;
    p.coef_cache_dmax = e->coef_cache_dmax;
    p.area_tabs = e->area_tabs;
    p.hop = e->hop;
    p.t1 = e->t1;
    p.t2 = e->t2;
    p.t_stride = e->t_stride;
    p.crops_u8 = crops_u8;
    p.crops_f32 = crops_f32;
    p.crops_f32_is_bf16 = input_form(e, crops_f32);
    p.status = status;
    p.fallback_count = e->fallback;
    p.fallback_list = e->fallback + 4;
    const double ncrops = (double)n * e->cfg.num_fighters;
    ProfScope ps(e, s, "preprocess_crops", 0.0, ncrops * (375.0 * 375 * 3 + 49152.0 * 5));
    if (e->jpeg_quality > 0 && !p.crops_u8) p.crops_u8 = e->crops_tmp;
    HIPCHK(e, launch_preprocess(p, s));
    if (e->jpeg_quality > 0) {
        JpegParams j;
        memset(&j, 0, sizeof(j));
        j.crops_u8 = p.crops_u8;
        j.qtab = e->jpeg_qtab;
        j.x0 = crops_f32;
        j.x0_bf16 = input_form(e, crops_f32);
        j.bgr = swap_rb ? 0 : 1;
        ProfScope pj(e, s, "jpeg_roundtrip", 0.0, ncrops * 49152.0 * 2);
        HIPCHK(e, launch_jpeg_roundtrip(j, (int)ncrops, s));
    }
    return PA_OK;
}

}


extern "C" {

int pa_abi_version(void) { return PA_ABI_VERSION; }

const char* pa_status_string(int status) {
    switch (status) {
        case PA_OK: return "ok";
        case PA_ERR_INVALID_ARG: return "invalid argument";
        case PA_ERR_HIP: return "HIP runtime error";
        case PA_ERR_BAD_WEIGHTS: return "weight blob does not match the expected layout";
        case PA_ERR_CAPACITY: return "request exceeds the capacity the engine was created with";
        case PA_ERR_NO_DEVICE: return "no usable HIP device";
        case PA_ERR_NOT_READY: return "features of a required frame are not in the cache";
        case PA_ERR_BAD_LABELS: return "labels outside [0, num_actions) were skipped";
        default: return "unknown status";
    }
}

const char* pa_last_error(const pa_engine* e) { return e ? e->last_error.c_str() : "null engine"; }

size_t pa_weight_blob_bytes(int S, int A) { return 8 * sizeof(int32_t) + blob_float_count(S, A) * sizeof(float); }

}

namespace {

int create_impl(const pa_config* cfg, const void* blob, size_t src_bytes, const void* arena_dev, pa_engine** out) {
    if (!cfg || (!blob && !arena_dev) || !out) return PA_ERR_INVALID_ARG;
    *out = nullptr;
    if (cfg->abi_version != PA_ABI_VERSION) return PA_ERR_INVALID_ARG;
    const int S = cfg->sequence_length, A = cfg->num_actions, F = cfg->num_fighters;
    if (S < 1 || S % 2 == 0 || S > 15 || A < 1 || A > 64 || F < 1 || F > 4 || cfg->max_batch_frames < 1 ||
        cfg->max_clip_frames < 1 || cfg->max_frame_height < 1 || cfg->max_frame_width < 1 || cfg->crop_padding < 0 ||
        (cfg->compute_dtype != PA_DTYPE_F32 && cfg->compute_dtype != PA_DTYPE_BF16 && cfg->compute_dtype != PA_DTYPE_EMULATED_F32))
        return PA_ERR_INVALID_ARG;
    const int32_t* hdr = reinterpret_cast<const int32_t*>(blob);
    if (blob && (src_bytes != pa_weight_blob_bytes(S, A) || hdr[0] != PA_WEIGHT_MAGIC || hdr[1] != 1 || hdr[2] != S || hdr[3] != A))
        return PA_ERR_BAD_WEIGHTS;
    pa_engine* e = new pa_engine();
    e->cfg = *cfg;
    e->bf16 = cfg->compute_dtype == PA_DTYPE_BF16;
    e->emu = cfg->compute_dtype == PA_DTYPE_EMULATED_F32;
    e->dtype = e->bf16 ? DT_BF16 : e->emu ? DT_EMULATED_F32 : DT_F32;
    e->adopt = blob == nullptr;
    e->knobs = engine_knobs();
    const EngineKnobs& K = e->knobs;
    *out = e;
    {
        int ndev = 0;
        const hipError_t derr = hipGetDeviceCount(&ndev);
        if (derr != hipSuccess || ndev <= 0 || cfg->device_id < 0 || cfg->device_id >= ndev)
            return fail(e, PA_ERR_NO_DEVICE,
                        std::string("hipGetDeviceCount: ") + hipGetErrorString(derr) + ", devices=" + std::to_string(ndev) +
                            ", requested device " + std::to_string(cfg->device_id));
    }
    HIPCHK(e, hipSetDevice(cfg->device_id));
    HIPCHK(e, preprocess_init_device());
    const int NC = cfg->max_batch_frames * F;
    e->max_crops = NC;
    e->cache_rows = cfg->max_clip_frames * F;
    int rc;
#define ALLOC(ptr, count, zero)                         \
    do {                                                \
        rc = dev_alloc(e, &(ptr), (size_t)(count), zero); \
        if (rc != PA_OK) return rc;                     \
    } while (0)

    ALLOC(e->x0_slot[0], (size_t)NC * 134 * 134 * 4, true);
    ALLOC(e->x0_slot[1], (size_t)NC * 134 * 134 * 4, true);
    e->x0 = e->x0_slot[0];
    e->stem_int = engine_forms(K, e->dtype).stem_int;
    if (e->stem_int) {
        ALLOC(e->xi_slot[0], (size_t)NC * 134 * 134 * 4, true);
        ALLOC(e->xi_slot[1], (size_t)NC * 134 * 134 * 4, true);
    }
    ALLOC(e->savebox_rects, (size_t)NC * 4, true);
    ALLOC(e->pre_status[0], (size_t)NC, true);
    ALLOC(e->pre_status[1], (size_t)NC, true);
    ALLOC(e->c1, (size_t)NC * 66 * 66 * 64, true);
    ALLOC(e->p1, (size_t)NC * 34 * 34 * 64, true);
    ALLOC(e->pooled, (size_t)NC * 512, true);
    ALLOC(e->feats_tmp, (size_t)NC * PA_FEATURE_STRIDE, true);
    ALLOC(e->jpeg_qtab, 128, true);
    ALLOC(e->crops_tmp, (size_t)NC * PA_CROP * PA_CROP * 3, true);
    ALLOC(e->cache, (size_t)e->cache_rows * PA_FEATURE_STRIDE, true);
    ALLOC(e->cache_status, (size_t)e->cache_rows, true);
    ALLOC(e->h1, (size_t)NC * 512, true);
    ALLOC(e->gather, (size_t)NC * S, true);
    ALLOC(e->status_tmp, (size_t)NC, true);
    ALLOC(e->dev_errors, 4, true);
    e->clean_g6_cap = (size_t)cfg->max_clip_frames * 8 * 6;
    ALLOC(e->clean_g6, e->clean_g6_cap, false);

    e->arena_cap = pa_weight_blob_bytes(S, A) / 4 * 13 + (1u << 20);
    {
        void* ar = nullptr;
        HIPCHK(e, hipMalloc(&ar, e->arena_cap));
        e->allocs.push_back(ar);
        e->arena = reinterpret_cast<uint8_t*>(ar);
    }
    if (!e->adopt) e->arena_stage.assign(e->arena_cap, 0);
    static const float dry_source[1] = {0.f};
    const float* blob_f = e->adopt ? dry_source : reinterpret_cast<const float*>(hdr + 8);
    BlobReader br{blob_f, 0, blob_float_count(S, A), e->adopt};
    std::vector<float> keep_w, keep_b;
    auto add_conv = [&](const std::string& name, int cin, int cout, int k, int stride, int in_hw, float* in, float* outb,
                        float* residual, int relu, bool keep = false) -> int {
        ConvLayer L;
        static_cast<LayerDesc&>(L) = conv_desc(K, e->dtype, NC, cin, cout, k, stride, in_hw, residual != nullptr);
        L.name = name;
        L.in = in;
        L.out = outb;
        L.residual = residual;
        L.relu = relu;
        std::vector<float> w, b;
        if (!fold_conv(br, L, w, b)) return fail(e, PA_ERR_BAD_WEIGHTS, "weight blob too short at " + name);
        int r2 = PA_OK;
        if (keep) {
            keep_w.swap(w);
            keep_b.swap(b);
        } else {
            r2 = (e->bf16 && k == 3) ? upload_bf16(e, &L.wgt, w) : upload(e, &L.wgt, w);
            if (r2) return r2;
            if (wino_layer(K, e->dtype, L)) {
                L.wino = true;
                L.wino_bn = wino_pick_bn(cout, (long long)NC * (L.out_hw / 4) * (L.out_hw / 4), cin);
                std::vector<float> ug(wino_weight_floats(cin, cout), 0.f);
                if (!br.dry) wino_transform_weights(w.data(), cin, cout, L.wino_bn, ug.data());
                r2 = upload(e, &L.wino_wgt, ug);
                if (r2) return r2;
            }
            L.split = e->emu && k == 3 && stride == 2 && cin % 32 == 0;
            if (L.split && (r2 = upload_split(e, &L.split_wgt, w, cout, 9 * cin, false))) return r2;
            if (e->bf16 && k == 7 && (r2 = upload_bf16(e, &e->stem_wgt_bf16, w))) return r2;
            r2 = upload(e, &L.bias, b);
            if (r2) return r2;
        }
        e->convs.push_back(L);
        return PA_OK;
    };

    rc = add_conv("conv1", 3, 64, 7, 2, 128, e->x0, e->c1, nullptr, 1);
    if (rc) return rc;
    {
        const int widths[4] = {64, 128, 256, 512};
        const int hw_in[4] = {32, 32, 16, 8};
        float* cur = e->p1;
        int cin = 64;
        for (int li = 0; li < 4; ++li) {
            const int co = widths[li];
            const int stride = li == 0 ? 1 : 2;
            const int hw_out = hw_in[li] / stride;
            const size_t buf = (size_t)NC * (hw_out + 2) * (hw_out + 2) * co;
            float *mid, *outA, *outB;
            ALLOC(mid, buf, true);
            ALLOC(outA, buf, true);
            ALLOC(outB, buf, true);
            const std::string pre = "layer" + std::to_string(li + 1);
            rc = add_conv(pre + ".0.conv1", cin, co, 3, stride, hw_in[li], cur, mid, nullptr, 1);
            if (rc) return rc;
            if (li == 0) {
                rc = add_conv(pre + ".0.conv2", co, co, 3, 1, hw_out, mid, outA, cur, 1);
                if (rc) return rc;
            } else {
                rc = add_conv(pre + ".0.conv2", co, co, 3, 1, hw_out, mid, outA, nullptr, 1, true);
                if (rc) return rc;
                ConvLayer D;
                D.name = pre + ".0.downsample";
                D.cin = cin; D.cout = co; D.kh = D.kw = 1; D.taps = 1; D.kw_taps = 1; D.chunk = cin;
                std::vector<float> wd, bd;
                if (!fold_conv(br, D, wd, bd)) return fail(e, PA_ERR_BAD_WEIGHTS, "weight blob too short at " + D.name);
                ConvLayer& L = e->convs.back();
                const int k_main = 9 * co, k_all = k_main + cin;
                std::vector<float> wf((size_t)co * k_all), bf(co);
                for (int o = 0; o < co; ++o) {
                    memcpy(&wf[(size_t)o * k_all], &keep_w[(size_t)o * k_main], sizeof(float) * k_main);
                    memcpy(&wf[(size_t)o * k_all + k_main], &wd[(size_t)o * cin], sizeof(float) * cin);
                    bf[o] = (float)((double)keep_b[o] + (double)bd[o]);
                }
                L.ds.src = cur;
                L.branch.c = cin;
                L.branch.hw = hw_in[li];
                L.branch.stride = stride;
                if (e->bf16) {
                    rc = upload_bf16(e, &L.wgt, keep_w);
                    if (rc) return rc;
                    rc = upload_bf16(e, &L.ds.wgt, wd);
                    if (rc) return rc;
                    ALLOC(L.ds.out, buf, true);
                } else {
                    rc = upload(e, &L.wgt, wf);
                    if (rc) return rc;
                    if (K.wino_ds && wino_layer(K, e->dtype, L)) {
                        L.wino = true;
                        L.wino_bn = wino_pick_bn(co, (long long)NC * (hw_out / 4) * (hw_out / 4), co);
                        std::vector<float> ug(wino_weight_floats(co, co), 0.f);
                        if (!br.dry) wino_transform_weights(keep_w.data(), co, co, L.wino_bn, ug.data());
                        rc = upload(e, &L.wino_wgt, ug);
                        if (rc) return rc;
                        rc = upload(e, &L.ds.wgt, wd);
                        if (rc) return rc;
                        L.branch.split = e->emu;
                        if (e->emu && (rc = upload_split(e, &L.ds.split_wgt, wd, co, cin, false))) return rc;
                        ALLOC(L.ds.out, buf, true);
                    }
                }
                ConvLayer& C1 = e->convs[e->convs.size() - 2];
                L.branch.place = place_branch(K, e->dtype, C1, L, C1.in == cur, li);
                if (L.branch.place == BRANCH_OPENER || L.branch.place == BRANCH_OPENER_PROBE) {
                    C1.carries = L.branch.place;
                    C1.carries_of = (int)e->convs.size() - 1;
                }
                rc = upload(e, &L.bias, bf);
                if (rc) return rc;
                L.k_alg += cin;
            }
            rc = add_conv(pre + ".1.conv1", co, co, 3, 1, hw_out, outA, mid, nullptr, 1);
            if (rc) return rc;
            rc = add_conv(pre + ".1.conv2", co, co, 3, 1, hw_out, mid, outB, outA, 1);
            if (rc) return rc;
            cur = outB;
            cin = co;
        }
        e->layer4_out = cur;
    }
    {
        const float* w = br.take((size_t)1000 * 512);
        const float* b = br.take(1000);
        if (!w || !b) return fail(e, PA_ERR_BAD_WEIGHTS, "weight blob too short at fc");
        std::vector<float> wp((size_t)PA_FEATURE_STRIDE * 512, 0.f), bp(PA_FEATURE_STRIDE, 0.f);
        if (!br.dry) {
            memcpy(wp.data(), w, sizeof(float) * 1000 * 512);
            memcpy(bp.data(), b, sizeof(float) * 1000);
        }
        ConvLayer& L = e->fc;
        static_cast<LayerDesc&>(L) = fc_desc(K, PA_FEATURE_STRIDE);
        L.name = "fc";
        L.in = e->pooled; L.out = nullptr; L.residual = nullptr;
        rc = upload(e, &L.wgt, wp);
        if (rc) return rc;
        rc = upload(e, &L.bias, bp);
        if (rc) return rc;
    }
    {
        const float* w = br.take((size_t)512 * 1000 * S);
        const float* b = br.take(512);
        if (!w || !b) return fail(e, PA_ERR_BAD_WEIGHTS, "weight blob too short at cnn1d");
        std::vector<float> wp((size_t)512 * S * PA_FEATURE_STRIDE, 0.f);
        for (int o = 0; o < 512 && !br.dry; ++o)
            for (int c = 0; c < 1000; ++c)
                for (int t = 0; t < S; ++t)
                    wp[((size_t)o * S + t) * PA_FEATURE_STRIDE + c] = w[((size_t)o * 1000 + c) * S + t];
        rc = upload(e, &e->w1d, wp);
        if (rc) return rc;
        rc = upload(e, &e->b1d, br.dry ? std::vector<float>(512) : std::vector<float>(b, b + 512));
        if (rc) return rc;
        choose_tile(NC, 512, S * 32, &e->head_tile, &e->head_splitk);
        if (e->head_splitk > 16) e->head_splitk = 16;
        if (K.head_splitk) e->head_splitk = K.head_splitk;
    }
    {
        const float* w2 = br.take(128 * 512);
        const float* b2 = br.take(128);
        const float* w3 = br.take((size_t)A * 128);
        const float* b3 = br.take(A);
        if (!w2 || !b2 || !w3 || !b3 || br.pos != br.limit) return fail(e, PA_ERR_BAD_WEIGHTS, "weight blob size mismatch at classifier");
        std::vector<float> w2t((size_t)512 * 128), w3t((size_t)128 * 64, 0.f);
        for (int o = 0; o < 128 && !br.dry; ++o)
            for (int k = 0; k < 512; ++k) w2t[(size_t)k * 128 + o] = w2[(size_t)o * 512 + k];
        for (int a = 0; a < A && !br.dry; ++a)
            for (int k = 0; k < 128; ++k) w3t[(size_t)k * 64 + a] = w3[(size_t)a * 128 + k];
        if ((rc = upload(e, &e->w2, w2t))) return rc;
        if ((rc = upload(e, &e->b2, br.dry ? std::vector<float>(128) : std::vector<float>(b2, b2 + 128)))) return rc;
        if ((rc = upload(e, &e->w3, w3t))) return rc;
        if ((rc = upload(e, &e->b3, br.dry ? std::vector<float>(A) : std::vector<float>(b3, b3 + A)))) return rc;
    }
    if (e->adopt) {
        if (src_bytes != e->arena_used) return fail(e, PA_ERR_BAD_WEIGHTS, "weight arena size does not match this configuration");
        HIPCHK(e, hipMemcpy(e->arena, arena_dev, e->arena_used, hipMemcpyDeviceToDevice));
    } else {
        HIPCHK(e, hipMemcpy(e->arena, e->arena_stage.data(), e->arena_used, hipMemcpyHostToDevice));
        std::vector<uint8_t>().swap(e->arena_stage);
    }
    if (e->stem_int) {
        const size_t nw = (size_t)64 * 224;
        std::vector<float> w(nw);
        HIPCHK(e, hipMemcpy(w.data(), e->convs[0].wgt, nw * sizeof(float), hipMemcpyDeviceToHost));
        std::vector<uint16_t> sl(3 * nw);
        for (size_t i = 0; i < nw; ++i) {
            float x = w[i];
            for (int k = 0; k < 3; ++k) {
                const uint16_t hq = bf16_rne(x);
                sl[k * nw + i] = hq;
                const uint32_t u = (uint32_t)hq << 16;
                float f;
                memcpy(&f, &u, 4);
                x -= f;
            }
        }
        ALLOC(e->stem_wgt_int, 3 * nw, false);
        HIPCHK(e, hipMemcpy(e->stem_wgt_int, sl.data(), sl.size() * sizeof(uint16_t), hipMemcpyHostToDevice));
    }
    {
        size_t need = 0;
        for (const ConvLayer& L : e->convs)
            if (L.splitk > 1) need = std::max(need, (size_t)L.splitk * NC * L.out_hw * L.out_hw * L.cout);
        if (e->fc.splitk > 1) need = std::max(need, (size_t)e->fc.splitk * NC * PA_FEATURE_STRIDE);
        if (e->head_splitk > 1) need = std::max(need, (size_t)e->head_splitk * NC * 512);
        bool any_wino = false;
        for (const ConvLayer& L : e->convs) any_wino = any_wino || L.wino_wgt;
        if (any_wino) {
            need = std::max(need, (size_t)256 * 512 * 32);
            ALLOC(e->wino_tickets, (size_t)2 * WINO_TICKETS, true);
        }
        need *= 2;
        e->slab_floats = need;
        ALLOC(e->slab, need, false);
    }
    e->coef_dim = std::max(cfg->max_frame_height, cfg->max_frame_width);
    e->t_stride = std::max((size_t)cfg->max_frame_height * cfg->max_frame_width * 3, (size_t)(448 + 128) * PA_CROP * 3);
    ALLOC(e->plans, (size_t)NC, true);
    ALLOC(e->fallback, (size_t)NC + 4, true);
    ALLOC(e->coef, (size_t)NC * 2 * e->coef_dim * (2 + PA_KSIZE_MAX), false);
    e->coef_cache_dmax = std::min(std::min(cfg->max_frame_height, cfg->max_frame_width), 1024);
    ALLOC(e->coef_cache, coef_cache_ints(e->coef_cache_dmax), false);
    e->coef_cache_pad = 30;
    HIPCHK(e, launch_build_coef_cache(e->coef_cache, e->coef_cache_pad, e->coef_cache_dmax, nullptr));
    ALLOC(e->area_tabs, (size_t)NC * 2 * PA_CROP, true);
    ALLOC(e->hop, (size_t)NC * PA_HOP_BLOCKS_MAX * PA_HOP_BLOCK_BYTES, true);
    ALLOC(e->t1, (size_t)NC * e->t_stride, false);
    ALLOC(e->t2, (size_t)NC * e->t_stride, false);
#undef ALLOC
    HIPCHK(e, hipStreamCreateWithFlags(&e->side, hipStreamNonBlocking));
    HIPCHK(e, hipEventCreateWithFlags(&e->ev_fork, hipEventDisableTiming));
    HIPCHK(e, hipEventCreateWithFlags(&e->ev_join, hipEventDisableTiming));
    HIPCHK(e, hipEventCreateWithFlags(&e->ev_ds_fork, hipEventDisableTiming));
    HIPCHK(e, hipEventCreateWithFlags(&e->ev_ds_join, hipEventDisableTiming));
    HIPCHK(e, hipDeviceSynchronize());
    return PA_OK;
}

}

extern "C" {

int pa_create(const pa_config* cfg, const void* blob, size_t blob_bytes, pa_engine** out) {
    if (!blob) return PA_ERR_INVALID_ARG;
    return create_impl(cfg, blob, blob_bytes, nullptr, out);
}

int pa_create_from_arena(const pa_config* cfg, const void* arena_dev, size_t arena_bytes, pa_engine** out) {
    if (!arena_dev) return PA_ERR_INVALID_ARG;
    return create_impl(cfg, nullptr, arena_bytes, arena_dev, out);
}

size_t pa_weights_arena_bytes(const pa_engine* e) { return e ? e->arena_used : 0; }

int pa_weights_export(pa_engine* e, void* dst_dev, size_t bytes, void* stream) {
    if (!e || !dst_dev || bytes != e->arena_used) return fail(e, PA_ERR_INVALID_ARG, "pa_weights_export: size must be pa_weights_arena_bytes()");
    HIPCHK(e, hipMemcpyAsync(dst_dev, e->arena, bytes, hipMemcpyDeviceToDevice, (hipStream_t)stream));
    return PA_OK;
}

void pa_destroy(pa_engine* e) {
    if (!e) return;
    (void)hipSetDevice(e->cfg.device_id);
    (void)hipDeviceSynchronize();
    for (ProfEntry& p : e->prof_log) {
        (void)hipEventDestroy(p.start);
        (void)hipEventDestroy(p.stop);
    }
    for (hipEvent_t ev : e->event_pool) (void)hipEventDestroy(ev);
    if (e->ev_fork) (void)hipEventDestroy(e->ev_fork);
    if (e->ev_join) (void)hipEventDestroy(e->ev_join);
    if (e->ev_ds_fork) (void)hipEventDestroy(e->ev_ds_fork);
    if (e->ev_ds_join) (void)hipEventDestroy(e->ev_ds_join);
    if (e->side) (void)hipStreamDestroy(e->side);
    if (e->gate_flag) (void)hipHostFree(e->gate_flag);
    for (void* p : e->allocs) (void)hipFree(p);
    delete e;
}

int pa_infer_windows(pa_engine* e, const float* x, int32_t batch, float* logp, void* stream) {
    if (!e || !x || !logp || batch < 1) return fail(e, PA_ERR_INVALID_ARG, "pa_infer_windows: bad argument");
    const int S = e->cfg.sequence_length;
    hipStream_t s = (hipStream_t)stream;
    const int win_per_pass = e->max_crops / S;
    if (win_per_pass < 1) return fail(e, PA_ERR_CAPACITY, "pa_infer_windows: engine smaller than one window");
    for (int w0 = 0; w0 < batch; w0 += win_per_pass) {
        const int nw = std::min(win_per_pass, batch - w0);
        const int ncrops = nw * S;
        {
            ProfScope ps(e, s, "nchw_to_nhwc4", 0.0, ncrops * (49152.0 * 4 + 134.0 * 134 * 16));
            HIPCHK(e, launch_nchw_to_padded(x + (size_t)w0 * S * 3 * 128 * 128, e->x0, ncrops, e->bf16 ? 1 : 0, s));
        }
        int rc = run_backbone(e, ncrops, e->x0, e->feats_tmp, s);
        if (rc) return rc;
        HIPCHK(e, launch_identity_gather(e->gather, ncrops, s));
        e->gather_key[0] = -1;
        rc = run_head(e, nw, e->feats_tmp, e->gather, nullptr, nullptr, logp + (size_t)w0 * e->cfg.num_actions, s);
        if (rc) return rc;
    }
    return PA_OK;
}

int pa_backbone_windows(pa_engine* e, const float* x, int32_t n_crops, float* feats, void* stream) {
    if (!e || !x || !feats || n_crops < 1) return fail(e, PA_ERR_INVALID_ARG, "pa_backbone_windows: bad argument");
    hipStream_t s = (hipStream_t)stream;
    for (int c0 = 0; c0 < n_crops; c0 += e->max_crops) {
        const int n = std::min(e->max_crops, n_crops - c0);
        {
            ProfScope ps(e, s, "nchw_to_nhwc4", 0.0, n * (49152.0 * 4 + 134.0 * 134 * 16));
            HIPCHK(e, launch_nchw_to_padded(x + (size_t)c0 * 3 * 128 * 128, e->x0, n, e->bf16 ? 1 : 0, s));
        }
        const int rc = run_backbone(e, n, e->x0, feats + (size_t)c0 * PA_FEATURE_STRIDE, s);
        if (rc) return rc;
    }
    return PA_OK;
}

int pa_backbone_trace(pa_engine* e, const float* x, int32_t n_crops, int32_t stage, void* out, size_t out_bytes, void* aux,
                      size_t aux_bytes, void* stream) {
    if (!e || !x || !out) return fail(e, PA_ERR_INVALID_ARG, "pa_backbone_trace: bad argument");
    if (stage < 0 || stage >= PA_TRACE_STAGES) return fail(e, PA_ERR_INVALID_ARG, "pa_backbone_trace: stage out of range");
    if (n_crops < 1 || n_crops > e->max_crops) return fail(e, PA_ERR_INVALID_ARG, "pa_backbone_trace: n_crops outside 1..max_crops");
    if (e->convs.size() != 17) return fail(e, PA_ERR_INVALID_ARG, "pa_backbone_trace: unexpected layer table");
    const size_t n = (size_t)n_crops, es = e->bf16 ? 2 : 4;
    const void* src;
    const void* aux_src = nullptr;
    size_t bytes;
    bool has_branch = false;
    if (stage == 0) {
        src = e->x0;
        bytes = n * 134 * 134 * 4 * es;
    } else if (stage == 1) {
        src = e->p1;
        bytes = n * 34 * 34 * 64 * es;
    } else if (stage <= 17) {
        const ConvLayer& L = e->convs[stage - 1];
        const size_t w = (size_t)L.out_hw + 2 * L.out_pad;
        src = L.out;
        bytes = n * w * w * L.cout * es;
        has_branch = L.branch.place != BRANCH_NONE;
        aux_src = L.ds.out;
    } else if (stage == 18) {
        src = e->pooled;
        bytes = n * 512 * sizeof(float);
    } else {
        src = e->feats_tmp;
        bytes = n * PA_FEATURE_STRIDE * sizeof(float);
    }
    if (out_bytes < bytes) return fail(e, PA_ERR_INVALID_ARG, "pa_backbone_trace: out is smaller than the stage");
    if (has_branch && aux) {
        if (!aux_src) return fail(e, PA_ERR_INVALID_ARG, "pa_backbone_trace: this stage stores no downsample branch");
        if (aux_bytes < bytes) return fail(e, PA_ERR_INVALID_ARG, "pa_backbone_trace: aux is smaller than the stage");
    }
    hipStream_t s = (hipStream_t)stream;
    HIPCHK(e, launch_nchw_to_padded(x, e->x0, n_crops, e->bf16 ? 1 : 0, s));
    if (stage > 0) {
        const int rc = run_backbone(e, n_crops, e->x0, e->feats_tmp, s, stage);
        if (rc) return rc;
    }
    HIPCHK(e, hipMemcpyAsync(out, src, bytes, hipMemcpyDeviceToDevice, s));
    if (has_branch && aux) HIPCHK(e, hipMemcpyAsync(aux, aux_src, bytes, hipMemcpyDeviceToDevice, s));
    return PA_OK;
}

int pa_crop_resize_width(pa_engine* e, const uint8_t* frames, int32_t n, int32_t height, int32_t width, const int32_t* rects_host,
                         int32_t n_rects, int32_t out_w, uint8_t* out, int32_t out_h_cap, int32_t* out_h_host, void* stream) {
    if (!e || !frames || !rects_host || !out || !out_h_host || n < 1 || height < 1 || width < 1 || n_rects < 1 || n_rects > 4 || out_w < 1 ||
        out_h_cap < 1)
        return fail(e, PA_ERR_INVALID_ARG, "pa_crop_resize_width: bad argument");
    RectResizeParams q;
    memset(&q, 0, sizeof(q));
    q.frames = frames;
    q.height = height;
    q.width = width;
    q.n_rects = n_rects;
    q.out_w = out_w;
    q.out_h_cap = out_h_cap;
    q.out = out;
    for (int r = 0; r < n_rects; ++r) {
        const int x1 = rects_host[4 * r], y1 = rects_host[4 * r + 1], x2 = rects_host[4 * r + 2], y2 = rects_host[4 * r + 3];
        if (x1 < 0 || y1 < 0 || x2 > width || y2 > height || x2 <= x1 || y2 <= y1)
            return fail(e, PA_ERR_INVALID_ARG, "pa_crop_resize_width: empty rectangle or outside the frame (cv2.resize raises on an empty image)");
        const double ratio = (double)out_w / (double)(x2 - x1);
        const int oh = (int)((double)(y2 - y1) * ratio);
        if (oh < 1) return fail(e, PA_ERR_INVALID_ARG, "pa_crop_resize_width: destination height 0");
        if (oh > out_h_cap) return fail(e, PA_ERR_CAPACITY, "pa_crop_resize_width: out_h_cap too small");
        q.x1[r] = x1; q.y1[r] = y1; q.x2[r] = x2; q.y2[r] = y2;
        q.out_h[r] = oh;
        out_h_host[r] = oh;
    }
    HIPCHK(e, launch_rect_resize(q, n, (hipStream_t)stream));
    return PA_OK;
}

int pa_square_crops(pa_engine* e, const uint8_t* frames, int32_t n, int32_t height, int32_t width, const double* boxes,
                    int32_t padding, int32_t swap_rb, uint8_t* crops, int32_t* status, void* stream) {
    if (!e || !frames || !boxes || !crops || n < 1 || height < 1 || width < 1 || padding < 0)
        return fail(e, PA_ERR_INVALID_ARG, "pa_square_crops: bad argument");
    if (n > e->cfg.max_batch_frames || height > e->cfg.max_frame_height || width > e->cfg.max_frame_width)
        return fail(e, PA_ERR_CAPACITY, "pa_square_crops: frames exceed engine capacity");
    return run_preprocess(e, frames, n, height, width, boxes, padding, swap_rb, crops, nullptr, status, (hipStream_t)stream);
}

int pa_square_crops_sized(pa_engine* e, const uint8_t* frames, int32_t n, int32_t height, int32_t width, const double* boxes,
                          int32_t padding, int32_t swap_rb, int32_t output_size, uint8_t* crops, int32_t* status, void* stream) {
    if (!e || !frames || !boxes || !crops || n < 1 || height < 1 || width < 1 || padding < 0)
        return fail(e, PA_ERR_INVALID_ARG, "pa_square_crops_sized: bad argument");
    if (output_size < PA_CROP_SIZE_MIN || output_size > PA_CROP_SIZE_MAX)
        return fail(e, PA_ERR_INVALID_ARG, "pa_square_crops_sized: output_size outside " + std::to_string(PA_CROP_SIZE_MIN) + ".." + std::to_string(PA_CROP_SIZE_MAX));
    if (n > e->cfg.max_batch_frames || height > e->cfg.max_frame_height || width > e->cfg.max_frame_width)
        return fail(e, PA_ERR_CAPACITY, "pa_square_crops_sized: frames exceed engine capacity");
    PreprocParams p;
    memset(&p, 0, sizeof(p));
    p.frames = frames;
    p.boxes = boxes;
    p.n_src = n;
    p.n_frames = n;
    p.height = height;
    p.width = width;
    p.fighters = e->cfg.num_fighters;
    p.padding = padding;
    p.swap_rb = swap_rb;
    p.plans = e->plans;
    p.coef = e->coef;
    p.coef_dim = e->coef_dim;
    p.coef_cache = e->coef_cache_pad == padding ? e->coef_cache : nullptr;
    p.coef_cache_pad = padding;
    p.coef_cache_dmax = e->coef_cache_dmax;
    p.t1 = e->t1;
    p.t2 = e->t2;
    p.t_stride = e->t_stride;
    p.crops_u8 = crops;
    p.status = status;
    hipStream_t s = (hipStream_t)stream;
    const double ncrops = (double)n * e->cfg.num_fighters;
    ProfScope ps(e, s, "square_crops_sized", 0.0, ncrops * (375.0 * 375 * 3 * 3 + 3.0 * output_size * output_size));
    HIPCHK(e, launch_crop_sized(p, output_size, s));
    return PA_OK;
}

namespace {
int run_runner_inputs(pa_engine* e, const uint8_t* images, size_t images_bytes, const pa_crop_image* desc, int n, int swap_rb,
                      uint8_t* inputs_u8, float* inputs_f32, int32_t* status, hipStream_t s) {
    RunnerInParams q;
    memset(&q, 0, sizeof(q));
    q.images = images;
    q.images_bytes = (long long)images_bytes;
    q.desc = reinterpret_cast<const CropImageDesc*>(desc);
    q.n = n;
    q.swap_rb = swap_rb;
    q.max_h = e->cfg.max_frame_height;
    q.max_w = e->cfg.max_frame_width;
    q.t1 = e->t1;
    q.t2 = e->t2;
    q.t_stride = e->t_stride;
    q.inputs_u8 = inputs_u8;
    q.inputs_f32 = inputs_f32;
    q.inputs_f32_is_bf16 = input_form(e, inputs_f32);
    q.status = status;
    ProfScope ps(e, s, "runner_inputs", 0.0, (double)images_bytes + (double)n * 49152.0 * 5);
    HIPCHK(e, launch_runner_inputs(q, s));
    return PA_OK;
}
}

int pa_runner_inputs(pa_engine* e, const uint8_t* images, size_t images_bytes, const pa_crop_image* desc, int32_t n_crops,
                     int32_t swap_rb, uint8_t* inputs_u8, int32_t* status, void* stream) {
    static_assert(sizeof(pa_crop_image) == sizeof(CropImageDesc), "descriptor layouts must agree");
    if (!e || !images || !desc || !inputs_u8 || n_crops < 1) return fail(e, PA_ERR_INVALID_ARG, "pa_runner_inputs: bad argument");
    if (n_crops > e->max_crops) return fail(e, PA_ERR_CAPACITY, "pa_runner_inputs: more crops than max_batch_frames * num_fighters");
    return run_runner_inputs(e, images, images_bytes, desc, n_crops, swap_rb, inputs_u8, nullptr, status, (hipStream_t)stream);
}

int pa_backbone_crop_images(pa_engine* e, const uint8_t* images, size_t images_bytes, const pa_crop_image* desc, int32_t n,
                            int32_t frame0, uint8_t* crops_rgb, int32_t* status, void* stream) {
    if (!e || !images || !desc || n < 1 || frame0 < 0) return fail(e, PA_ERR_INVALID_ARG, "pa_backbone_crop_images: bad argument");
    if (e->clip_frames < 1) return fail(e, PA_ERR_INVALID_ARG, "pa_backbone_crop_images: call pa_clip_begin first");
    if (n > e->cfg.max_batch_frames || frame0 + n > e->clip_frames)
        return fail(e, PA_ERR_CAPACITY, "pa_backbone_crop_images: frames exceed engine / clip capacity");
    hipStream_t s = (hipStream_t)stream;
    const int F = e->cfg.num_fighters;
    int rc = run_runner_inputs(e, images, images_bytes, desc, n * F, 1, crops_rgb, slot_dst(e, 0), e->pre_status[0], s);
    if (rc) return rc;
    if (status) HIPCHK(e, hipMemcpyAsync(status, e->pre_status[0], sizeof(int32_t) * n * F, hipMemcpyDeviceToDevice, s));
    return pa_backbone_slot(e, 0, n, frame0, stream);
}

namespace {
void host_slice(const double* b, int W, int H, int pad, int* sy0, int* sx0, int* sh, int* sw) {
    *sy0 = *sx0 = *sh = *sw = 0;
    const double v[4] = {b[0] * W, b[1] * H, b[2] * W, b[3] * H};
    int iv[4];
    for (int k = 0; k < 4; ++k) {
        if (!(v[k] > -2.0e9 && v[k] < 2.0e9)) return;
        iv[k] = (int)v[k];
    }
    const int cx = iv[0], cy = iv[1], d = iv[2] > iv[3] ? iv[2] : iv[3];
    if (d <= 0 || d > 16384) return;
    const int half = d / 2;
    auto np_slice = [](int start, int stop, int size, int* s0, int* len) {
        if (start > size) start = size;
        if (stop < 0) {
            stop += size;
            if (stop < 0) stop = 0;
        }
        if (stop > size) stop = size;
        *s0 = start;
        *len = stop > start ? stop - start : 0;
    };
    np_slice(std::max(cy - half - pad, 0), std::min(cy + half + pad, H), H, sy0, sh);
    np_slice(std::max(cx - half - pad, 0), std::min(cx + half + pad, W), W, sx0, sw);
}
}

// ... 788 lines not shown
```

playaid_core_amd/csrc/pa_kernels.h:

```cpp
#pragma once
#include "gemm_tile.h"
#include <hip/hip_runtime.h>
#include <stdint.h>

namespace pa {

__device__ __forceinline__ float silu_fast(float x) {
    return x * __builtin_amdgcn_rcpf(1.0f + __builtin_amdgcn_exp2f(x * -1.44269504088896341f));
}

struct GemmParams {
    const float* act;
    const float* wgt;
    const float* bias;
    const float* residual;
    float* out;
    float* slab;
    const int32_t* gather;
    int32_t M, N, ktot;
    int32_t taps, kw_taps, chunk;
    int32_t howo, wo;
    int32_t howo_shift, wo_shift;
    int32_t in_img_stride, in_row_stride, in_px_stride, stride, off_y, off_x;
    int32_t out_img_stride, out_row_stride, out_px_stride, out_pad;
    int32_t relu;
    int32_t res_after;
    const float* act2;
    int32_t k2_steps, in2_img_stride, in2_row_stride, in2_px_stride, stride2, off2;
    int32_t splitk, ksteps_per_split;
    int32_t defer_reduce;
    int32_t* splitk_used;
    int32_t skip_w;
    int32_t tiles_m, tiles_n;
    int32_t pg_per, pg_ho, pg_nwx, pg_nwy;
    uint32_t pg_magic_howo, pg_magic_wo;
    float* up_out;
    int32_t up_img_stride, up_row_stride, up_px_stride, up_pad;
    int32_t patch_slots, patch_pitch, img_px, tiles_per_img, p0_img, p0_row, total_px;
    int32_t swz_a, magic_pitch, magic_img, img_px_patch;
    int32_t xcd_m, xcd_n;
    int32_t blk_rows, blk_cols, blk_shift_c, blk_shift_px, blk_per_row, blk_per_img, n_blocks, src_pitch;
    const float* wgt2;
    float* out2;
    unsigned long long* clk;
    int32_t* tickets;
};

hipError_t launch_igemm(const GemmParams& p, GemmTile tile, hipStream_t s);
hipError_t launch_pgemm(const GemmParams& p, int bm, hipStream_t s);
int psgemm_pick_bn(int N, int residual);
size_t psgemm_weight_elems(int N, int ktot, int residual);
void psgemm_pack_weights(const float* w, int N, int ktot, int residual, unsigned short* out);
hipError_t launch_psgemm(const GemmParams& p, const unsigned short* wsp, size_t out_floats, size_t up_floats, hipStream_t s);
size_t bgemm_weight_elems(int N, int ktot, int residual);
void bgemm_pack_weights(const float* w, int N, int ktot, int residual, unsigned short* out);
hipError_t launch_bgemm(const GemmParams& p, const unsigned short* wsp, size_t out_elems, size_t up_elems, bool out_f32, hipStream_t s);
constexpr int BGEMM_SLAB_ITEMS = 256, BGEMM_TICKETS = 4 * 128, BGEMM_SPLIT_MAX_GRID = 64, BGEMM_SPLIT_MIN_KSTEPS = 72;
int bgemm_pick_split(const GemmParams& p, int force);
hipError_t launch_igemm_bf16(const GemmParams& p, GemmTile tile, hipStream_t s);

hipError_t launch_conv3x3_bf16_patch(const GemmParams& p, hipStream_t s);

struct StemParams {
    const float* x;
    const float* wgt;
    const float* bias;
    float* out;
    int32_t tiles;
    int32_t out_bf16;
    unsigned long long* clk;
};
hipError_t launch_stem7x7(const StemParams& p, hipStream_t s);
struct StemPoolParams {
    const void* x;
    const void* wgt;
    const float* bias;
    void* out;
    int32_t crops;
    int32_t run;
    int32_t in_bf16;
    int32_t out_bf16;
};
hipError_t launch_stem_pool(const StemPoolParams& p, hipStream_t s);
struct StemPoolAnyParams {
    const float* x;
    const float* wgt;
    const float* bias;
    float* out;
    int32_t crops;
    int32_t in_hw;
    int32_t run;
};
hipError_t launch_stem_pool_any(const StemPoolAnyParams& p, hipStream_t s);
hipError_t launch_splitk_reduce(const GemmParams& p, hipStream_t s, bool out_bf16 = false);
hipError_t launch_conv3x3_patch(const GemmParams& p, int bm, hipStream_t s);
hipError_t launch_conv3x3_patch_blocked(const GemmParams& p, hipStream_t s);

struct WinoParams {
    const float* act;
    const float* wgt;
    const float* bias;
    const float* residual;
    float* out;
    int32_t n_img, height, width, cin, cout;
    int32_t bn;
    int32_t in_px_stride, in_row_stride, in_img_stride;
    int32_t out_px_stride, out_row_stride, out_img_stride, out_pad;
    int32_t relu, res_after;
    int32_t n_sb, sb_per_row, sb_per_img, tiles_n;
    unsigned long long* clk;
    float* slab;
    size_t slab_floats;
    int32_t* tickets;
    int32_t tickets_cap, ksplit;
    int32_t tiles_m, xcd_gm, xcd_gn;
};
size_t wino_weight_floats(int cin, int cout);
int wino_pick_bn(int cout, long long n_sb, int cin_split = 0);
void wino_transform_weights(const float* w, int cin, int cout, int bn, float* ug);
hipError_t launch_wino3x3(const WinoParams& p, hipStream_t s);

#define PA_KSIZE_MAX 15
#define PA_CROP_BLANK 0x100
#define PA_FUSED_LDS_BYTES 77824

struct CropPlan {
    int32_t status;
    int32_t frame;
    int32_t sx0, sy0, sw, sh;
    int32_t d;
    int32_t rw, rh;
    int32_t px, py;
    int32_t need_h, need_v;
    int32_t ksize_h, ksize_v;
    int32_t out_h;
    int32_t area_mode;
    int32_t iscale_x, iscale_y;
    int32_t fused_rb;
    int32_t mfma_v;
    int32_t mfma_h, h_mis;
    double scale_x, scale_y;
    const int32_t* coef_h;
    const int32_t* coef_v;
};

struct AreaTabPacked {
    uint32_t bits;
    float a_first, a_mid, a_last;
};

#define PA_HOP_BLOCKS_MAX 48
#define PA_HOP_PIXELS 10
#define PA_HOP_WINDOW 64
#define PA_HOP_BLOCK_BYTES (6 * 1024 + 32 * 4 + 16)
#define PA_CROP_MFMA_H_DEFAULT 1

struct CropWindow {
    int64_t offset;
    int32_t pitch;
    int32_t rows;
    int64_t src_offset;
    int32_t src_pitch;
    int32_t row_bytes;
};
hipError_t launch_slice_upload(const uint8_t* frames_host, long long frames_bytes, const CropWindow* desc, uint8_t* windows, int ncrops,
                               hipStream_t s);

struct PreprocParams {
    const uint8_t* frames;
    const CropWindow* windows;
    const double* boxes;
    const int32_t* src_frame;
    int32_t n_src;
    int32_t n_frames, height, width, fighters, padding, swap_rb;
    CropPlan* plans;
    int32_t* coef;
    int32_t coef_dim;
    const int32_t* coef_cache;
    int32_t coef_cache_pad, coef_cache_dmax;
    AreaTabPacked* area_tabs;
    uint8_t* t1;
    uint8_t* t2;
    size_t t_stride;
    uint8_t* crops_u8;
    float* crops_f32;
    int32_t crops_f32_is_bf16;
    int32_t* status;
    int32_t* fallback_count;
    int32_t* fallback_list;
    int32_t fused_lds;
    int32_t ablate;
    int32_t crop_mfma;
    int32_t crop_mfma_h;
    int32_t crop_xcd;
    uint8_t* hop;
    uint8_t* dbg;
    int32_t dbg_crop, dbg_row;
};

hipError_t launch_preprocess(const PreprocParams& p, hipStream_t s);
hipError_t launch_crop_sized(const PreprocParams& p, int out_size, hipStream_t s);
size_t coef_cache_ints(int dmax);
hipError_t launch_build_coef_cache(int32_t* cache, int padding, int dmax, hipStream_t s);

struct CropImageDesc {
    int64_t offset;
    int32_t height, width;
};
struct RunnerInParams {
    const uint8_t* images;
    long long images_bytes;
    const CropImageDesc* desc;
    int32_t n, swap_rb, max_h, max_w;
    uint8_t* t1;
    uint8_t* t2;
    size_t t_stride;
    uint8_t* inputs_u8;
    float* inputs_f32;
    int32_t inputs_f32_is_bf16;
    int32_t* status;
};
hipError_t launch_runner_inputs(const RunnerInParams& q, hipStream_t s);

struct JpegParams {
    uint8_t* crops_u8;
    const int32_t* qtab;
    void* x0;
    int32_t x0_bf16;
    int32_t bgr;
};
hipError_t launch_jpeg_roundtrip(const JpegParams& p, int ncrops, hipStream_t s);

struct CleanParams {
    const float* dets;
    const int32_t* counts;
    int32_t n_labels, max_det, n_decoded, fighters;
    int32_t class_ids[4];
    double* lab;
    int32_t* pixel_frame;
    double* pixel_box;
    int32_t* crop_kind;
    float* crop_row;
    int32_t* info;
    double* g6v;
};
hipError_t launch_clean_labels(const CleanParams& p, hipStream_t s);
struct CropImageDesc;
hipError_t launch_detector_plan(const int32_t* pixel_frame, const double* pixel_box, const int32_t* crop_kind, const int32_t* info4, int n_labels, int F,
                                int32_t* det_index, int32_t* src_own, int32_t* rep_entry, double* rep_boxes, int32_t* rep_src, int32_t* words5,
                                hipStream_t s);
hipError_t launch_detector_desc(CropImageDesc* desc, const int32_t* crop_kind, int n_entries, int F, int step_frames, long long region,
                                const int32_t* rep_entry, int n_rep, long long rep_base, hipStream_t s);

struct SaveBoxRect { int32_t x1, y1, w, h; };
struct SaveBoxParams {
    const uint8_t* frames;
    int32_t height, width, fighters, n_entries;
    const float* dets;
    const int32_t* counts;
    int32_t max_det;
    const int32_t* det_index;
    const int32_t* src_frame;
    int32_t n_src;
    int32_t class_ids[4];
    float gain, pad;
    uint8_t* images;
    unsigned long long capacity;
    CropImageDesc* desc;
    SaveBoxRect* rects;
    int32_t* overflow;
    int32_t quality;
    int32_t qtab[128];
};
hipError_t launch_save_one_box(const SaveBoxParams& p, hipStream_t s);

struct RectResizeParams {
    const uint8_t* frames;
    int32_t height, width;
    int32_t n_rects;
    int32_t x1[4], y1[4], x2[4], y2[4];
    int32_t out_w, out_h[4];
    int32_t out_h_cap;
    uint8_t* out;
};
hipError_t launch_rect_resize(const RectResizeParams& q, int n_frames, hipStream_t s);
hipError_t preprocess_init_device();
hipError_t launch_project_boxes(const double* log, double* boxes, int32_t n, hipStream_t s);

struct DetectParams {
    const float* pred;
    int32_t n_frames, rows, nc, max_det;
    float conf_thres, iou_thres;
    uint32_t class_mask;
    uint32_t class_words[3];
    float pad_x, pad_y, gain;
    float img_w, img_h;
    float* dets;
    int32_t* counts;
};
hipError_t launch_detect_nms(const DetectParams& q, hipStream_t s);
constexpr int DETECT_MAX_CLASSES = 80;
hipError_t launch_detect_nms_classes(const DetectParams& q, hipStream_t s);

hipError_t launch_linear_f32(const float* X, int ld, const float* W, const float* bias, float* C, int ldc, int M, int N, int K, int relu,
                             hipStream_t s);
hipError_t launch_spin(int32_t microseconds, hipStream_t s);
hipError_t launch_gate(const int* flag, int32_t max_microseconds, hipStream_t s);
hipError_t launch_nchw_to_padded(const float* x, float* out, int32_t n, int32_t out_bf16, hipStream_t s);
hipError_t launch_nchw_to_padded_sized(const float* x, float* out, int32_t n, int32_t hw, hipStream_t s);
hipError_t launch_maxpool(const float* in, float* out, int32_t n, hipStream_t s);
hipError_t launch_avgpool(const float* in, float* out, int32_t n, hipStream_t s);
hipError_t launch_maxpool_bf16(const void* in, void* out, int32_t n, hipStream_t s);
hipError_t launch_avgpool_bf16(const void* in, float* out, int32_t n, hipStream_t s);
hipError_t launch_window_gather(int32_t* gather, int32_t frame_num_lo, int32_t count, int32_t fighters,
                                int32_t seq, int32_t delta, int32_t max_frames, int32_t min_frame, int32_t sub_frames, hipStream_t s);
hipError_t launch_identity_gather(int32_t* gather, int32_t n, hipStream_t s);
hipError_t launch_scatter_rows(const float* feats, const int32_t* st, const int32_t* ids, float* cache, int32_t* cache_st,
                               int32_t n, int32_t fighters, int32_t clip_frames, int32_t* bad_ids, hipStream_t s);

struct HeadParams {
    const float* h1;
    const float* slab;
    const float* b1;
    int32_t splitk;
    const float* w2;
    const float* b2;
    const float* w3;
    const float* b3;
    float* logp;
    void* records;
    const int32_t* crop_status;
    const int32_t* gather;
    int32_t nwin, num_actions, fighters, seq;
    int32_t class_ids[4];
};
hipError_t launch_head_mlp(const HeadParams& p, hipStream_t s);

constexpr int EVAL_SLAB_PARTS = 1024;
hipError_t launch_eval_rows(const float* logp, int ld, int n, int A, const int32_t* labels, int label_stride, unsigned long long* counts,
                            double* sums, unsigned long long* confusion, double* slab, hipStream_t s);

struct AnnotParams {
    const unsigned char* in;
    unsigned char* out;
    const void* items;
    const int* counts;
    const unsigned char* text;
    const unsigned char* atlas;
    int n, H, W, pad_left, pad_right, pad_bottom;
    int cell_w, cell_h, n_chars;
};
hipError_t launch_annotate(const AnnotParams& p, hipStream_t s);

struct AdamScalars {
    double one_minus_b1, b2, one_minus_b2;
    float step_size, bc2_sqrt, eps;
};
struct HeadTensors {
    const float* p[6];
};
struct HeadTrainParams {
    const float* feats;
    const int32_t* gather;
    const int32_t* labels;
    int32_t n_rows, B, S, A, apply;
    float* w[6];
    float* m[6];
    float* v[6];
    float *h1, *h2, *dz3, *dz2, *dz1, *loss_b, *gs, *stats;
    int32_t* hit_b;
    float* stats_out;
    float* grads_out;
};
size_t head_tensor_floats(int S, int A);
hipError_t launch_head_train_step(const HeadTrainParams& p, const AdamScalars& ak, hipStream_t s);
hipError_t launch_head_export(const HeadTensors& src, int S, int A, float* out, hipStream_t s);

}
```

playaid_core_amd/csrc/pigemm.hip:

```cpp
#include "pgemm_common.h"

#include <algorithm>
#include <type_traits>
#include <cstdio>
#include <cstdlib>
#include <vector>

namespace pa {


namespace {

typedef __attribute__((address_space(3))) float lds_f32;
typedef __attribute__((address_space(3))) f32x4 lds_f32x4;

template <int N> __device__ __forceinline__ void pg_wait_vm() { wait_vmcnt<(N > 63 ? 63 : N)>(); }

}

template <int BM, int BN, bool SILU, bool STAMP, bool UP, bool DS>
__device__ __forceinline__ void pgemm_body(const GemmParams& p) {
    static_assert(!DS || (!UP && !STAMP && !SILU), "the branch form is the ResNet openers': ReLU, no up-sampled copy");
    auto stamp = [&](int i) {
        if (STAMP) {
            const unsigned long long t = __builtin_amdgcn_s_memtime();
            if ((threadIdx.x & 63) == 0) p.clk[((size_t)blockIdx.x * 4 + (threadIdx.x >> 6)) * 64 + i] = t;
        }
    };
    stamp(0);
    constexpr int WM = BN == 64 ? 2 : 4;
    constexpr int MI = BM / WM / 32;
    constexpr int A_ROWS = BM / 32, B_ROWS = BN / 32;
    constexpr int NLD = A_ROWS + B_ROWS;
    constexpr int NST = MI * 4 * (UP ? 5 : (DS ? 2 : 1));
    constexpr int STAGE = (BM + BN + (DS ? BN : 0)) * 32;
    __shared__ __attribute__((aligned(16))) float lds[3 * STAGE];

    const TileRun run = tile_run(p);
    const int tile_n = run.tile_n, nt = run.nt;
    {
        const float *pa_ = p.act, *pw_ = p.wgt, *pb_ = p.bias;
        float* po_ = p.out;
        const int i0 = p.M, i1 = p.ktot, i2 = p.kw_taps, i3 = p.chunk, i4 = p.howo, i5 = p.wo, i6 = p.in_img_stride, i7 = p.in_row_stride,
                  i8 = p.in_px_stride, i9 = p.stride, i10 = p.off_y, i11 = p.off_x, i12 = p.out_img_stride, i13 = p.out_row_stride,
                  i14 = p.out_px_stride, i15 = p.out_pad, i16 = p.pg_ho, i17 = p.pg_nwx, i18 = p.pg_nwy;
        const unsigned u0 = p.pg_magic_howo, u1 = p.pg_magic_wo;
        asm volatile("" ::"s"(pa_), "s"(pw_), "s"(pb_), "s"(po_), "s"(i0), "s"(i1), "s"(i2), "s"(i3), "s"(i4), "s"(i5), "s"(i6), "s"(i7), "s"(i8), "s"(i9),
                     "s"(i10), "s"(i11), "s"(i12), "s"(i13), "s"(i14), "s"(i15), "s"(i16), "s"(i17), "s"(i18), "s"(u0), "s"(u1));
        if (DS) {
            const float* pw2_ = p.wgt2;
            float* po2_ = p.out2;
            asm volatile("" ::"s"(pw2_), "s"(po2_));
        }
    }
    if (nt == 0) return;
    stamp(60);
    const int nk = p.ktot >> 5;
    const int total = nt * nk;
    const int nkc = p.chunk >> 5;
    const int c_lo = 4 * nkc, c_hi = 5 * nkc;

    const int tid = threadIdx.x;
    const int wave_id = __builtin_amdgcn_readfirstlane(tid >> 6);
    const int row0 = tid >> 3;
    const int colq = (tid & 7) ^ ((row0 >> 1) & 7);
    const int lane = tid & 63, lr = lane & 31, lh = lane >> 5;
    const int wm = BN == 64 ? wave_id >> 1 : wave_id, wn = BN == 64 ? wave_id & 1 : 0;

    const __amdgpu_buffer_rsrc_t act_rs = glds_rsrc(p.act), wgt_rs = glds_rsrc(p.wgt);
    const __amdgpu_buffer_rsrc_t wgt2_rs = glds_rsrc(DS ? p.wgt2 : p.wgt);

    const int ch0 = tile_n * BN + wn * 32 + 4 * lh;
    f32x2 nl2e = f32x2{-1.44269504088896341f, -1.44269504088896341f}, one2 = f32x2{1.f, 1.f};
    asm volatile("" : "+v"(nl2e), "+v"(one2));

    int b_off[B_ROWS];
#pragma unroll
    for (int i = 0; i < B_ROWS; ++i) b_off[i] = ((tile_n * BN + row0 + 32 * i) * p.ktot + colq * 4) * 4;
    int b2_off[B_ROWS];
#pragma unroll
    for (int i = 0; i < B_ROWS; ++i) b2_off[i] = DS ? ((tile_n * BN + row0 + 32 * i) * p.chunk + colq * 4) * 4 : 0;

    const int in_ps = p.in_px_stride * p.stride * 4, in_rs = p.in_row_stride * p.stride * 4;
    const int in_wrap_x = in_rs - p.wo * in_ps;
    const int in_wrap_y = p.in_img_stride * 4 - p.pg_ho * in_rs;
    const int in_org = (p.off_y * p.in_row_stride + p.off_x * p.in_px_stride) * 4;
    int in_lane = row0 * in_ps + colq * 16;
    asm volatile("" : "+v"(in_lane));
    const PixelGeom geom = pixel_geom(p);
    int in_last;
    {
        int oy, ox;
        in_last = pixel_base(geom, p.M - 1, p.in_img_stride * 4, in_rs, in_ps, oy, ox) + in_org + colq * 16;
    }
    auto in_offset = [&](int m_base) {
        const int off = pixel_walk(geom, m_base, row0, p.in_img_stride * 4, in_rs, in_ps, in_wrap_x, in_wrap_y, in_org + in_lane);
        return m_base + row0 < p.M ? off : in_last;
    };
    const int out_wrap_x = p.out_row_stride - p.wo * p.out_px_stride;
    const int out_wrap_y = p.out_img_stride - p.pg_ho * p.out_row_stride;
    int out_lane = lr * p.out_px_stride + p.out_pad * (p.out_row_stride + p.out_px_stride) + ch0;
    asm volatile("" : "+v"(out_lane));
    auto out_offset = [&](int m_base) { return pixel_walk(geom, m_base, lr, p.out_img_stride, p.out_row_stride, p.out_px_stride, out_wrap_x, out_wrap_y, out_lane); };
    const int up_rs = 2 * p.up_row_stride, up_ps = 2 * p.up_px_stride;
    const int up_wrap_x = up_rs - p.wo * up_ps, up_wrap_y = p.up_img_stride - p.pg_ho * up_rs;
    int up_lane = lr * up_ps + p.up_pad * (p.up_row_stride + p.up_px_stride) + ch0;
    asm volatile("" : "+v"(up_lane));
    IssueCursor cur{run.first, 0, 0, 0, 0};
    int a_off[A_ROWS];
    auto rows_of = [&](int tile_m) {
#pragma unroll
        for (int i = 0; i < A_ROWS; ++i) a_off[i] = in_offset(tile_m * BM + 32 * i);
    };
    rows_of(cur.tile);
    stamp(61);
    auto issue = [&](int slot) {
        float* As_w = lds + slot * STAGE + wave_id * 256;
        float* Bs_w = As_w + BM * 32;
        const int tapoff = cur.tap_offset(p) * 4;
#pragma unroll
        for (int i = 0; i < A_ROWS; ++i) glds16(act_rs, a_off[i], tapoff, As_w + i * 1024);
        const int koff = ((cur.ky * p.kw_taps + cur.kx) * p.chunk + cur.kc) * 4;
#pragma unroll
        for (int i = 0; i < B_ROWS; ++i) glds16(wgt_rs, b_off[i], koff, Bs_w + i * 1024);
        if (DS && cur.ky == 1 && cur.kx == 1) {
#pragma unroll
            for (int i = 0; i < B_ROWS; ++i) glds16(wgt2_rs, b2_off[i], cur.kc * 4, Bs_w + BN * 32 + i * 1024);
        }
        cur.advance(p, nk, run, rows_of);
    };

    unsigned a_k[4], b_k[4];
    {
        const int a_rd = (wm * (BM / WM) + lr) * 32, b_rd = BM * 32 + (wn * 32 + lr) * 32;
        const int swz = (lr >> 1) & 7;
        const unsigned base = (unsigned)(size_t)(lds_f32*)lds;
#pragma unroll
        for (int kk = 0; kk < 4; ++kk) {
            const int ch_ = ((kk * 2 + lh) ^ swz) * 4;
            a_k[kk] = base + (a_rd + ch_) * 4;
            b_k[kk] = base + (b_rd + ch_) * 4;
            asm volatile("" : "+v"(a_k[kk]), "+v"(b_k[kk]));
        }
    }

    issue(0);
    stamp(62);
    if (total > 1) issue(1);
    f32x16 biasv;
#pragma unroll
    for (int g = 0; g < 4; ++g) {
        const f32x4 b4 = p.bias ? *reinterpret_cast<const f32x4*>(p.bias + ch0 + 8 * g) : f32x4{0.f, 0.f, 0.f, 0.f};
        biasv[4 * g] = b4.x; biasv[4 * g + 1] = b4.y; biasv[4 * g + 2] = b4.z; biasv[4 * g + 3] = b4.w;
    }
    asm volatile("" : "+v"(biasv));
    stamp(1);

    f32x16 acc[MI];
    f32x16 acc2[MI];
    auto kstep = [&](int sb, auto first_c, auto branch_c) {
        constexpr bool FIRST = decltype(first_c)::value;
        constexpr int BR = decltype(branch_c)::value;
        f32x16 zero16;
        if (BR == 1) {
#pragma unroll
            for (int e = 0; e < 16; ++e) zero16[e] = 0.f;
        }
        f32x4 b2f[2];
        unsigned ra[4], rb[4];
#pragma unroll
        for (int kk = 0; kk < 4; ++kk) {
            ra[kk] = a_k[kk] + sb;
            rb[kk] = b_k[kk] + sb;
            asm volatile("" : "+v"(ra[kk]), "+v"(rb[kk]));
        }
        f32x4 af[2][MI], bf[2];
#define PG_FRAGS(SET, KK)                                                                                    \
    {                                                                                                        \
        _Pragma("unroll") for (int mi = 0; mi < MI; ++mi)                                                    \
            af[SET][mi] = *(const lds_f32x4*)(size_t)(ra[KK] + mi * 4096);                                   \
        bf[SET] = *(const lds_f32x4*)(size_t)(rb[KK]);                                                       \
        if (BR) b2f[SET] = *(const lds_f32x4*)(size_t)(rb[KK] + BN * 128);                                    \
    }
        PG_FRAGS(0, 0);
#pragma unroll
        for (int kk = 0; kk < 4; ++kk) {
#pragma unroll
            for (int mi = 0; mi < MI; ++mi) {
                const f32x4 a4 = af[kk & 1][mi], b4 = bf[kk & 1];
                acc[mi] = __builtin_amdgcn_mfma_f32_32x32x2f32(b4.x, a4.x, FIRST && kk == 0 ? biasv : acc[mi], 0, 0, 0);
                acc[mi] = __builtin_amdgcn_mfma_f32_32x32x2f32(b4.y, a4.y, acc[mi], 0, 0, 0);
                if (mi == 0 && kk + 1 < 4) {
                    __builtin_amdgcn_sched_barrier(0);
                    if (kk == 0) { PG_FRAGS(1, 1); } else if (kk == 1) { PG_FRAGS(0, 2); } else { PG_FRAGS(1, 3); }
                    __builtin_amdgcn_sched_barrier(0);
                }
                acc[mi] = __builtin_amdgcn_mfma_f32_32x32x2f32(b4.z, a4.z, acc[mi], 0, 0, 0);
                acc[mi] = __builtin_amdgcn_mfma_f32_32x32x2f32(b4.w, a4.w, acc[mi], 0, 0, 0);
                if (BR) {
                    const f32x4 c4 = b2f[kk & 1];
                    acc2[mi] = __builtin_amdgcn_mfma_f32_32x32x2f32(c4.x, a4.x, BR == 1 && kk == 0 ? zero16 : acc2[mi], 0, 0, 0);
                    acc2[mi] = __builtin_amdgcn_mfma_f32_32x32x2f32(c4.y, a4.y, acc2[mi], 0, 0, 0);
                    acc2[mi] = __builtin_amdgcn_mfma_f32_32x32x2f32(c4.z, a4.z, acc2[mi], 0, 0, 0);
                    acc2[mi] = __builtin_amdgcn_mfma_f32_32x32x2f32(c4.w, a4.w, acc2[mi], 0, 0, 0);
                }
            }
        }
#undef PG_FRAGS
    };

    int slot = 0, g = 0;
    auto pre = [&](int ks, int t) {
        const bool next = g + 1 < total;
        int closed = 0;
        if (ks == 0 && g > 0) closed = 1;
        if ((nk == 1 || ks == 1) && g > 1) ++closed;
        if (next) {
            if (closed == 2) pg_wait_vm<NLD + 2 * NST>();
            else if (closed == 1) pg_wait_vm<NLD + NST>();
            else pg_wait_vm<NLD>();
        } else {
            if (closed == 2) pg_wait_vm<2 * NST>();
            else if (closed == 1) pg_wait_vm<NST>();
            else pg_wait_vm<0>();
        }
        __builtin_amdgcn_s_barrier();
        if (STAMP && ks == 0 && t < 15) stamp(3 + 4 * t);
        const int slot2 = slot == 0 ? 2 : slot - 1;
        if (g + 2 < total) issue(slot2);
        __builtin_amdgcn_sched_barrier(0);
    };
    for (int t = 0; t < nt; ++t) {
        const int tile_m = run.tile(t);
        if (t < 15) stamp(2 + 4 * t);
        pre(0, t);
        kstep(slot * (STAGE * 4), std::true_type{}, std::integral_constant<int, 0>{});
        slot = slot == 2 ? 0 : slot + 1;
        ++g;
        for (int ks = 1; ks < nk; ++ks, ++g) {
            pre(ks, t);
            if (DS && ks == c_lo) kstep(slot * (STAGE * 4), std::false_type{}, std::integral_constant<int, 1>{});
            else if (DS && ks > c_lo && ks < c_hi) kstep(slot * (STAGE * 4), std::false_type{}, std::integral_constant<int, 2>{});
            else kstep(slot * (STAGE * 4), std::false_type{}, std::integral_constant<int, 0>{});
            slot = slot == 2 ? 0 : slot + 1;
        }
        if (t < 15) stamp(4 + 4 * t);
#pragma unroll
        for (int mi = 0; mi < MI; ++mi) {
            const int m_base = tile_m * BM + wm * (BM / WM) + mi * 32;
            const int o_off = out_offset(m_base);
            float* o_px = p.out + o_off;
            const bool live = m_base + lr < p.M;
            f32x4 out4[4];
#pragma unroll
            for (int gq = 0; gq < 4; ++gq) {
                f32x2 lo = f32x2{acc[mi][4 * gq], acc[mi][4 * gq + 1]}, hi = f32x2{acc[mi][4 * gq + 2], acc[mi][4 * gq + 3]};
                if (SILU) {
                    const f32x2 tl = lo * nl2e, th = hi * nl2e;
                    const f32x2 dl = f32x2{__builtin_amdgcn_exp2f(tl.x), __builtin_amdgcn_exp2f(tl.y)} + one2;
                    const f32x2 dh = f32x2{__builtin_amdgcn_exp2f(th.x), __builtin_amdgcn_exp2f(th.y)} + one2;
                    lo *= f32x2{__builtin_amdgcn_rcpf(dl.x), __builtin_amdgcn_rcpf(dl.y)};
                    hi *= f32x2{__builtin_amdgcn_rcpf(dh.x), __builtin_amdgcn_rcpf(dh.y)};
                } else if (p.relu == 1) {
                    lo.x = lo.x > 0.f ? lo.x : 0.f; lo.y = lo.y > 0.f ? lo.y : 0.f;
                    hi.x = hi.x > 0.f ? hi.x : 0.f; hi.y = hi.y > 0.f ? hi.y : 0.f;
                }
                if (live) *reinterpret_cast<f32x4*>(o_px + 8 * gq) = f32x4{lo.x, lo.y, hi.x, hi.y};
                if (UP) { out4[gq] = f32x4{lo.x, lo.y, hi.x, hi.y}; }
            }
            if (DS && live) {
                float* o2_px = p.out2 + o_off;
#pragma unroll
                for (int gq = 0; gq < 4; ++gq)
                    *reinterpret_cast<f32x4*>(o2_px + 8 * gq) = f32x4{acc2[mi][4 * gq], acc2[mi][4 * gq + 1], acc2[mi][4 * gq + 2], acc2[mi][4 * gq + 3]};
            }
            if (UP && live) {
                float* u_px = p.up_out + pixel_walk(geom, m_base, lr, p.up_img_stride, up_rs, up_ps, up_wrap_x, up_wrap_y, up_lane);
#pragma unroll
                for (int q4 = 0; q4 < 4; ++q4) {
                    float* u = u_px + (q4 >> 1) * p.up_row_stride + (q4 & 1) * p.up_px_stride;
#pragma unroll
                    for (int gq = 0; gq < 4; ++gq) *reinterpret_cast<f32x4*>(u + 8 * gq) = out4[gq];
                }
            }
        }
        if (t < 15) stamp(5 + 4 * t);
    }
    stamp(63);
}

template <int BM, int BN = 64, bool SILU = true, bool STAMP = false, bool UP = false>
__global__ __launch_bounds__(256, 2) void pgemm_kernel(const GemmParams p) {
    pgemm_body<BM, BN, SILU, STAMP, UP, false>(p);
}

__global__ __launch_bounds__(256, 2) void pgemm_branch_kernel(const GemmParams p) {
    pgemm_body<64, 64, false, false, false, true>(p);
}

hipError_t launch_pgemm(const GemmParams& p_in, int bm, hipStream_t s) {
    GemmParams p = p_in;
    if (p.residual || p.N % 32 != 0 || (bm != 128 && bm != 64 && bm != 0) || persistent_plan(p) != hipSuccess) return hipErrorInvalidValue;
    const bool branch = p.wgt2 || p.out2;
    if (branch) {
        if (!p.wgt2 || !p.out2 || p.taps != 9 || p.kw_taps != 3 || p.stride != 2 || p.in_px_stride != p.chunk || p.splitk > 1 || p.N % 64 != 0 || p.relu == 2 || p.up_out ||
            ((reinterpret_cast<unsigned long long>(p.wgt2) | reinterpret_cast<unsigned long long>(p.out2)) & 15ull))
            return hipErrorInvalidValue;
        bm = 64;
    }
    const int bn = p.N % 64 == 0 ? 64 : 32;
    if (bn == 32) bm = 128;
    p.tiles_n = p.N / bn;
    if (p.tiles_n > 64) return hipErrorInvalidValue;
    auto plan = [&](int bm_, int* lm_out) {
        const int tm = (p.M + bm_ - 1) / bm_, share = (tm + 7) / 8;
        int lm = 64 / p.tiles_n;
        lm = lm < 1 ? 1 : (lm > share ? share : lm);
        *lm_out = lm;
        return (double)((share + lm - 1) / lm) * (bm_ == 128 ? 1.0 : 0.55) * (lm * p.tiles_n <= 32 ? 0.6 : 1.0);
    };
    int lm = 1;
    if (bm == 0) {
        int lm128, lm64;
        const double e128 = plan(128, &lm128), e64 = plan(64, &lm64);
        bm = e128 <= e64 ? 128 : 64;
        lm = bm == 128 ? lm128 : lm64;
    } else {
        (void)plan(bm, &lm);
    }
    p.tiles_m = (p.M + bm - 1) / bm;
    if ((long long)(p.tiles_m - 1) * bm >= p.M || (long long)p.tiles_m * bm < p.M) return hipErrorInvalidValue;
    const int per = lm * p.tiles_n;
    const int grid = per * 8;
    p.pg_per = per;
    const bool silu = p.relu == 2;
    static const char* stamp_file = getenv("PA_PG_STAMP_FILE");
    if (stamp_file && bm == 128 && bn == 64 && silu && !branch) {
        static int sm = 0, sk = 0, sn = 0, skip = getenv("PA_PG_STAMP_SKIP") ? atoi(getenv("PA_PG_STAMP_SKIP")) : 3, seen = 0;
        if (!sm && getenv("PA_PG_STAMP_SHAPE")) sscanf(getenv("PA_PG_STAMP_SHAPE"), "%d,%d,%d", &sm, &sk, &sn);
        if (p.M == sm && p.ktot == sk && p.N == sn && seen++ == skip) {
            const size_t n = (size_t)grid * 4 * 64;
            unsigned long long* d = nullptr;
            if (hipMalloc(&d, n * 8) != hipSuccess) return hipErrorOutOfMemory;
            (void)hipMemsetAsync(d, 0, n * 8, s);
            p.clk = d;
            hipLaunchKernelGGL((pgemm_kernel<128, 64, true, true>), dim3(grid), dim3(256), 0, s, p);
            std::vector<unsigned long long> hst(n);
            (void)hipStreamSynchronize(s);
            (void)hipMemcpy(hst.data(), d, n * 8, hipMemcpyDeviceToHost);
            (void)hipFree(d);
            if (FILE* f = fopen(stamp_file, "wb")) {
                const int hdr[4] = {grid, p.ktot / 32, p.tiles_m, p.tiles_n};
                fwrite(hdr, 4, 4, f);
                fwrite(hst.data(), 8, n, f);
                fclose(f);
            }
            return hipGetLastError();
        }
    }
#define PA_PG_LAUNCH(BM_, BN_)                                                                               \
    do {                                                                                                     \
        if (p.up_out) hipLaunchKernelGGL((pgemm_kernel<BM_, BN_, true, false, true>), dim3(grid), dim3(256), 0, s, p); \
        else if (silu) hipLaunchKernelGGL((pgemm_kernel<BM_, BN_, true>), dim3(grid), dim3(256), 0, s, p);   \
        else hipLaunchKernelGGL((pgemm_kernel<BM_, BN_, false>), dim3(grid), dim3(256), 0, s, p);            \
    } while (0)
    if (p.up_out && (!silu || p.up_px_stride % 4 || p.up_row_stride % 4 || p.up_img_stride % 4 || (reinterpret_cast<unsigned long long>(p.up_out) & 15ull)))
        return hipErrorInvalidValue;
    if (branch) hipLaunchKernelGGL(pgemm_branch_kernel, dim3(grid), dim3(256), 0, s, p);
    else if (bn == 32) PA_PG_LAUNCH(128, 32);
    else if (bm == 128) PA_PG_LAUNCH(128, 64);
    else PA_PG_LAUNCH(64, 64);
#undef PA_PG_LAUNCH
    return hipGetLastError();
}

}
```

playaid_core_amd/wino.py:

```python
from __future__ import annotations

import ctypes as C

import numpy as np
import torch

from . import _lib


def channels_per_workgroup(cout: int, sub_blocks: int) -> int:
    bn = _lib.load().pa_wino_channels_per_workgroup(cout, sub_blocks)
    if bn == 0:
        raise ValueError("cout must be a multiple of 32")
    return bn


def transform_weights(w_oihw: np.ndarray, bn: int = 0) -> np.ndarray:
    lib = _lib.load()
    w = np.ascontiguousarray(np.asarray(w_oihw, dtype=np.float32).transpose(0, 2, 3, 1))
    cout, cin = w.shape[0], w.shape[3]
    n = lib.pa_wino_weight_floats(cin, cout)
    if n == 0:
        raise ValueError("cin must be a multiple of 8, cout a multiple of 32")
    bn = bn or (64 if cout % 64 == 0 else 32)
    ug = np.empty(n, dtype=np.float32)
    rc = lib.pa_wino_transform_weights(w.ctypes.data_as(C.c_void_p), cin, cout, bn, ug.ctypes.data_as(C.c_void_p))
    if rc:
        raise ValueError(f"pa_wino_transform_weights: {rc}")
    return ug


class SplitKScratch:

    def __init__(self, device="cuda:0", slab_floats: int = 256 * 512 * 32, n_tickets: int = 4096):
        self.slab = torch.empty(slab_floats, dtype=torch.float32, device=device)
        self.tickets = torch.zeros(n_tickets, dtype=torch.int32, device=device)


def conv3x3(x_pad: torch.Tensor, ug: torch.Tensor, cin: int, cout: int, bias=None, residual=None, out=None, out_pad: int = 1,
            act: int = 0, res_after: bool = False, out_px_stride: int = None, bn: int = 0, split_k: SplitKScratch = None) -> torch.Tensor:
    lib = _lib.load()
    if x_pad.dtype != torch.float32 or not x_pad.is_cuda or not x_pad.is_contiguous() or x_pad.dim() != 4:
        raise ValueError("x_pad: contiguous float32[n, H + 2, W + 2, C] on the device")
    n, hp, wp, cs = x_pad.shape
    h, w = hp - 2, wp - 2
    ops = out_px_stride or cout
    if out is None:
        out = torch.zeros((n, h + 2 * out_pad, w + 2 * out_pad, ops), dtype=torch.float32, device=x_pad.device)
    ptr = lambda t_: C.c_void_p(t_.data_ptr()) if t_ is not None else C.c_void_p(0)
    stream = C.c_void_p(torch.cuda.current_stream(x_pad.device).cuda_stream)
    args = (ptr(x_pad), ptr(ug), ptr(bias), ptr(residual), ptr(out), n, h, w, cin, cout, bn or (64 if cout % 64 == 0 else 32), cs, out.shape[3], out_pad,
            int(act), int(bool(res_after)))
    if split_k is None:
        rc = lib.pa_wino_conv3x3(*args, stream)
    else:
        rc = lib.pa_wino_conv3x3_splitk(*args, ptr(split_k.slab), split_k.slab.numel(), ptr(split_k.tickets), split_k.tickets.numel(), stream)
    if rc:
        raise ValueError(f"pa_wino_conv3x3: status {rc}")
    return out
```

Measured before the change: 69520 frames/s.

## Add Winograd F(4x4,3x3) path for 4x4 stride-1 conv layers via grouped GEMM

```diff
diff --git a/include/playaid_hip.h b/include/playaid_hip.h
--- a/include/playaid_hip.h
+++ b/include/playaid_hip.h
@@ -468,6 +468,12 @@
 size_t pa_encoder_trainer_floats(const pa_encoder* h);
 int32_t pa_encoder_trainer_max_windows(const pa_encoder* h);
 
+size_t pa_wino4_weight_floats(int32_t cin, int32_t cout);
+int pa_wino4_transform_weights(const float* w_host, int32_t cin, int32_t cout, float* u_host);
+int pa_wino4_conv3x3(const float* x, const float* u, const float* bias, const float* residual, float* out, int32_t n, int32_t height,
+                     int32_t width, int32_t cin, int32_t cout, int32_t in_px_stride, int32_t out_px_stride, int32_t out_pad, int32_t act,
+                     int32_t res_after, float* scratch, size_t scratch_floats, void* stream);
+
 #ifdef __cplusplus
 }
 #endif
diff --git a/playaid_core_amd/_build.py b/playaid_core_amd/_build.py
--- a/playaid_core_amd/_build.py
+++ b/playaid_core_amd/_build.py
@@ -18,6 +18,7 @@
     ("patchconv.hip", []),
     ("patchconv_bf16.hip", []),
     ("wino.hip", []),
+    ("wino4.hip", []),
     ("stem.hip", []),
     ("stem_pool.hip", []),
     ("stem_pool_any.hip", []),
diff --git a/playaid_core_amd/_lib.py b/playaid_core_amd/_lib.py
--- a/playaid_core_amd/_lib.py
+++ b/playaid_core_amd/_lib.py
@@ -283,6 +283,9 @@
     ("pa_encoder_trainer_read", C.c_int, [_P, C.c_int32, _P, C.c_size_t, _P]),
     ("pa_encoder_trainer_floats", C.c_size_t, [_P]),
     ("pa_encoder_trainer_max_windows", C.c_int32, [_P]),
+    ("pa_wino4_weight_floats", C.c_size_t, [C.c_int32, C.c_int32]),
+    ("pa_wino4_transform_weights", C.c_int, [_P, C.c_int32, C.c_int32, _P]),
+    ("pa_wino4_conv3x3", C.c_int, [_P, _P, _P, _P, _P] + [C.c_int32] * 10 + [_P, C.c_size_t, _P]),
 ]
 
 _lib = None
diff --git a/playaid_core_amd/csrc/engine_plan.h b/playaid_core_amd/csrc/engine_plan.h
--- a/playaid_core_amd/csrc/engine_plan.h
+++ b/playaid_core_amd/csrc/engine_plan.h
@@ -6,6 +6,8 @@
 #include <cstdlib>
 
 namespace pa {
+
+constexpr int WINO_F4_MIN_CROPS = 64;
 
 struct EngineKnobs {
     int patch = 1;
@@ -20,6 +22,8 @@
     int wino = 1;
     int wino_min_hw = 4;
     int wino_ds = 1;
+    int wino_f4 = 1;
+    int wino_f4_min = WINO_F4_MIN_CROPS;
     int bf16_ds_fuse = 1;
     int f32_ds_fuse = 1;
     bool profile_layers = false;
@@ -54,6 +58,8 @@
         k.wino = env_int("PA_WINO", k.wino);
         k.wino_min_hw = env_int("PA_WINO_MIN_HW", k.wino_min_hw);
         k.wino_ds = env_int("PA_WINO_DS", k.wino_ds);
+        k.wino_f4 = env_int("PA_WINO_F4", k.wino_f4);
+        k.wino_f4_min = env_int("PA_WINO_F4_MIN", k.wino_f4_min);
         k.bf16_ds_fuse = env_int("PA_BF16_DS_FUSE", k.bf16_ds_fuse);
         k.f32_ds_fuse = env_int("PA_F32_DS_FUSE", k.f32_ds_fuse);
         return k;
@@ -114,6 +120,7 @@
     bool forced = false;
     bool adds_residual = false;
     bool wino = false;
+    bool wino4 = false;
     bool split = false;
     struct {
         BranchPlace place = BRANCH_NONE;
@@ -171,6 +178,10 @@
     return dt != DT_BF16 && L.kh == 3 && L.stride == 1 && k.wino && L.out_hw >= k.wino_min_hw && L.out_hw % 4 == 0;
 }
 
+inline bool wino4_layer(const EngineKnobs& k, ComputeDtype dt, const LayerDesc& L, int max_crops) {
+    return wino_layer(k, dt, L) && k.wino_f4 && L.out_hw == 4 && L.in_hw == 4 && L.cin % 64 == 0 && L.cout % 64 == 0 && max_crops >= k.wino_f4_min;
+}
+
 inline bool opener_can_carry(const LayerDesc& opener, const LayerDesc& conv2, bool same_input, bool extras) {
     return same_input && opener.stride == 2 && opener.cout == conv2.cout && opener.out_hw == conv2.out_hw && opener.out_pad == conv2.out_pad &&
            opener.chunk == conv2.branch.c && !opener.forced && extras;
@@ -219,6 +230,7 @@
     bool tile_256 = false;
     int patch_bm = 0;
     int pgemm_bm = 0;
+    bool wino_f4 = false;
     BranchLaunch branch = BL_NONE;
     LaunchAccount acct;
     BranchPlan branch_gemm;
@@ -268,6 +280,10 @@
     } else if (L.wino && !second_k) {
         P.form = CONV_WINO;
         P.acct.flops_executed = P.acct.flops * 4.0 / 9.0;
+        if (L.wino4 && k.wino_f4 && ncrops >= k.wino_f4_min) {
+            P.wino_f4 = true;
+            P.acct.flops_executed = P.acct.flops / 4.0;
+        }
     } else if (k.patch && L.kh == 3 && L.stride == 1) {
         P.form = CONV_PATCH;
         P.patch_bm = P.tile == TILE_64x64 || P.tile == TILE_64x64_K64 ? 64 : 128;
diff --git a/playaid_core_amd/csrc/pa_api.hip b/playaid_core_amd/csrc/pa_api.hip
--- a/playaid_core_amd/csrc/pa_api.hip
+++ b/playaid_core_amd/csrc/pa_api.hip
@@ -25,6 +25,7 @@
     float* wgt = nullptr;
     float* wino_wgt = nullptr;
     int wino_bn = 0;
+    float* wino4_wgt = nullptr;
     float* bias = nullptr;
     unsigned short* split_wgt = nullptr;
     struct {
@@ -87,6 +88,8 @@
     float* slab = nullptr;
     size_t slab_floats = 0;
     float* wino_tickets = nullptr;
+    float* wino4_scratch = nullptr;
+    size_t wino4_region = 0;
     std::vector<ConvLayer> convs;
     ConvLayer fc;
     float* stem_wgt_bf16 = nullptr;
@@ -387,6 +390,16 @@
         hipError_t pe = hipErrorInvalidValue;
         if (P.form == CONV_PSGEMM) {
             pe = launch_psgemm(p, L.split_wgt, (size_t)ncrops * out_crop, 0, s);
+        } else if (P.form == CONV_WINO && P.wino_f4) {
+            Wino4Params q{};
+            q.act = p.act; q.wgt = L.wino4_wgt; q.bias = p.bias; q.residual = p.residual; q.out = p.out;
+            q.v = e->wino4_scratch + (slab_off ? e->wino4_region : 0);
+            q.m = q.v + (size_t)36 * wino4_rows(ncrops) * L.cin;
+            q.n_img = ncrops; q.cin = L.cin; q.cout = L.cout;
+            q.in_px_stride = p.in_px_stride; q.in_row_stride = p.in_row_stride; q.in_img_stride = p.in_img_stride;
+            q.out_px_stride = p.out_px_stride; q.out_row_stride = p.out_row_stride; q.out_img_stride = p.out_img_stride; q.out_pad = p.out_pad;
+            q.relu = p.relu; q.res_after = p.res_after;
+            pe = launch_wino4_conv3x3(q, s);
         } else if (P.form == CONV_WINO) {
             WinoParams q = wino_params(p, ncrops, L.out_hw, L.out_hw, L.cin, L.wino_wgt, L.wino_bn);
             if (e->wino_tickets && e->slab) {
@@ -740,6 +753,7 @@
     ALLOC(e->clean_g6, e->clean_g6_cap, false);
 
     e->arena_cap = pa_weight_blob_bytes(S, A) / 4 * 13 + (1u << 20);
+    if (e->dtype != DT_BF16 && K.wino && K.wino_f4 && NC >= K.wino_f4_min) e->arena_cap += 3 * (wino4_weight_floats(512, 512) * sizeof(float) + 256);
     {
         void* ar = nullptr;
         HIPCHK(e, hipMalloc(&ar, e->arena_cap));
@@ -751,6 +765,13 @@
     const float* blob_f = e->adopt ? dry_source : reinterpret_cast<const float*>(hdr + 8);
     BlobReader br{blob_f, 0, blob_float_count(S, A), e->adopt};
     std::vector<float> keep_w, keep_b;
+    auto add_wino4 = [&](ConvLayer& L, const std::vector<float>& w) -> int {
+        if (!wino4_layer(K, e->dtype, L, NC)) return PA_OK;
+        L.wino4 = true;
+        std::vector<float> u4(wino4_weight_floats(L.cin, L.cout), 0.f);
+        if (!br.dry) wino4_transform_weights(w.data(), L.cin, L.cout, u4.data());
+        return upload(e, &L.wino4_wgt, u4);
+    };
     auto add_conv = [&](const std::string& name, int cin, int cout, int k, int stride, int in_hw, float* in, float* outb,
                         float* residual, int relu, bool keep = false) -> int {
         ConvLayer L;
@@ -776,6 +797,7 @@
                 if (!br.dry) wino_transform_weights(w.data(), cin, cout, L.wino_bn, ug.data());
                 r2 = upload(e, &L.wino_wgt, ug);
                 if (r2) return r2;
+                if ((r2 = add_wino4(L, w))) return r2;
             }
             L.split = e->emu && k == 3 && stride == 2 && cin % 32 == 0;
             if (L.split && (r2 = upload_split(e, &L.split_wgt, w, cout, 9 * cin, false))) return r2;
@@ -845,6 +867,7 @@
                         if (!br.dry) wino_transform_weights(keep_w.data(), co, co, L.wino_bn, ug.data());
                         rc = upload(e, &L.wino_wgt, ug);
                         if (rc) return rc;
+                        if ((rc = add_wino4(L, keep_w))) return rc;
                         rc = upload(e, &L.ds.wgt, wd);
                         if (rc) return rc;
                         L.branch.split = e->emu;
@@ -960,6 +983,9 @@
             need = std::max(need, (size_t)256 * 512 * 32);
             ALLOC(e->wino_tickets, (size_t)2 * WINO_TICKETS, true);
         }
+        for (const ConvLayer& L : e->convs)
+            if (L.wino4_wgt) e->wino4_region = std::max(e->wino4_region, (size_t)36 * wino4_rows(NC) * (L.cin + L.cout));
+        if (e->wino4_region) ALLOC(e->wino4_scratch, e->wino4_region * (K.interleave ? 2 : 1), false);
         need *= 2;
         e->slab_floats = need;
         ALLOC(e->slab, need, false);
diff --git a/playaid_core_amd/csrc/pa_kernels.h b/playaid_core_amd/csrc/pa_kernels.h
--- a/playaid_core_amd/csrc/pa_kernels.h
+++ b/playaid_core_amd/csrc/pa_kernels.h
@@ -44,10 +44,13 @@
     float* out2;
     unsigned long long* clk;
     int32_t* tickets;
+    int32_t grp_tiles, grp_wgt_bytes;
+    uint32_t grp_magic;
 };
 
 hipError_t launch_igemm(const GemmParams& p, GemmTile tile, hipStream_t s);
 hipError_t launch_pgemm(const GemmParams& p, int bm, hipStream_t s);
+hipError_t launch_pgemm_grouped(const float* a, const float* w, float* out, int groups, int rows, int K, int N, int tile, hipStream_t s);
 int psgemm_pick_bn(int N, int residual);
 size_t psgemm_weight_elems(int N, int ktot, int residual);
 void psgemm_pack_weights(const float* w, int N, int ktot, int residual, unsigned short* out);
@@ -119,6 +122,26 @@
 int wino_pick_bn(int cout, long long n_sb, int cin_split = 0);
 void wino_transform_weights(const float* w, int cin, int cout, int bn, float* ug);
 hipError_t launch_wino3x3(const WinoParams& p, hipStream_t s);
+
+struct Wino4Params {
+    const float* act;
+    const float* wgt;
+    const float* bias;
+    const float* residual;
+    float* out;
+    float* v;
+    float* m;
+    int32_t n_img, cin, cout;
+    int32_t in_px_stride, in_row_stride, in_img_stride;
+    int32_t out_px_stride, out_row_stride, out_img_stride, out_pad;
+    int32_t relu, res_after;
+    int32_t tile;
+    int32_t rows;
+};
+size_t wino4_weight_floats(int cin, int cout);
+int wino4_rows(int n_img);
+void wino4_transform_weights(const float* w, int cin, int cout, float* u);
+hipError_t launch_wino4_conv3x3(const Wino4Params& p, hipStream_t s);
 
 #define PA_KSIZE_MAX 15
 #define PA_CROP_BLANK 0x100
diff --git a/playaid_core_amd/csrc/pigemm.hip b/playaid_core_amd/csrc/pigemm.hip
--- a/playaid_core_amd/csrc/pigemm.hip
+++ b/playaid_core_amd/csrc/pigemm.hip
@@ -18,9 +18,10 @@
 
 }
 
-template <int BM, int BN, bool SILU, bool STAMP, bool UP, bool DS>
+template <int BM, int BN, bool SILU, bool STAMP, bool UP, bool DS, bool GRP = false>
 __device__ __forceinline__ void pgemm_body(const GemmParams& p) {
     static_assert(!DS || (!UP && !STAMP && !SILU), "the branch form is the ResNet openers': ReLU, no up-sampled copy");
+    static_assert(!GRP || (!UP && !STAMP && !SILU && !DS), "the grouped form is a plain product");
     auto stamp = [&](int i) {
         if (STAMP) {
             const unsigned long long t = __builtin_amdgcn_s_memtime();
@@ -52,6 +53,11 @@
             float* po2_ = p.out2;
             asm volatile("" ::"s"(pw2_), "s"(po2_));
         }
+        if (GRP) {
+            const int g0 = p.grp_tiles, g1 = p.grp_wgt_bytes;
+            const unsigned g2 = p.grp_magic;
+            asm volatile("" ::"s"(g0), "s"(g1), "s"(g2));
+        }
     }
     if (nt == 0) return;
     stamp(60);
@@ -108,9 +114,14 @@
     asm volatile("" : "+v"(up_lane));
     IssueCursor cur{run.first, 0, 0, 0, 0};
     int a_off[A_ROWS];
+    int w_grp = 0;
     auto rows_of = [&](int tile_m) {
 #pragma unroll
         for (int i = 0; i < A_ROWS; ++i) a_off[i] = in_offset(tile_m * BM + 32 * i);
+        if (GRP) {
+            int rem;
+            w_grp = pgemm_sdiv(tile_m, p.grp_tiles, p.grp_magic, rem) * p.grp_wgt_bytes;
+        }
     };
     rows_of(cur.tile);
     stamp(61);
@@ -120,7 +131,7 @@
         const int tapoff = cur.tap_offset(p) * 4;
 #pragma unroll
         for (int i = 0; i < A_ROWS; ++i) glds16(act_rs, a_off[i], tapoff, As_w + i * 1024);
-        const int koff = ((cur.ky * p.kw_taps + cur.kx) * p.chunk + cur.kc) * 4;
+        const int koff = ((cur.ky * p.kw_taps + cur.kx) * p.chunk + cur.kc) * 4 + (GRP ? w_grp : 0);
 #pragma unroll
         for (int i = 0; i < B_ROWS; ++i) glds16(wgt_rs, b_off[i], koff, Bs_w + i * 1024);
         if (DS && cur.ky == 1 && cur.kx == 1) {
@@ -158,6 +169,7 @@
 
     f32x16 acc[MI];
     f32x16 acc2[MI];
+    f32x16 accg[GRP ? 3 : 1][MI];
     auto kstep = [&](int sb, auto first_c, auto branch_c) {
         constexpr bool FIRST = decltype(first_c)::value;
         constexpr int BR = decltype(branch_c)::value;
@@ -188,15 +200,16 @@
 #pragma unroll
             for (int mi = 0; mi < MI; ++mi) {
                 const f32x4 a4 = af[kk & 1][mi], b4 = bf[kk & 1];
-                acc[mi] = __builtin_amdgcn_mfma_f32_32x32x2f32(b4.x, a4.x, FIRST && kk == 0 ? biasv : acc[mi], 0, 0, 0);
-                acc[mi] = __builtin_amdgcn_mfma_f32_32x32x2f32(b4.y, a4.y, acc[mi], 0, 0, 0);
+                f32x16& acc_k = GRP && kk > 0 ? accg[GRP ? kk - 1 : 0][mi] : acc[mi];
+                acc_k = __builtin_amdgcn_mfma_f32_32x32x2f32(b4.x, a4.x, FIRST && (GRP || kk == 0) ? biasv : acc_k, 0, 0, 0);
+                acc_k = __builtin_amdgcn_mfma_f32_32x32x2f32(b4.y, a4.y, acc_k, 0, 0, 0);
                 if (mi == 0 && kk + 1 < 4) {
                     __builtin_amdgcn_sched_barrier(0);
                     if (kk == 0) { PG_FRAGS(1, 1); } else if (kk == 1) { PG_FRAGS(0, 2); } else { PG_FRAGS(1, 3); }
                     __builtin_amdgcn_sched_barrier(0);
                 }
-                acc[mi] = __builtin_amdgcn_mfma_f32_32x32x2f32(b4.z, a4.z, acc[mi], 0, 0, 0);
-                acc[mi] = __builtin_amdgcn_mfma_f32_32x32x2f32(b4.w, a4.w, acc[mi], 0, 0, 0);
+                acc_k = __builtin_amdgcn_mfma_f32_32x32x2f32(b4.z, a4.z, acc_k, 0, 0, 0);
+                acc_k = __builtin_amdgcn_mfma_f32_32x32x2f32(b4.w, a4.w, acc_k, 0, 0, 0);
                 if (BR) {
                     const f32x4 c4 = b2f[kk & 1];
                     acc2[mi] = __builtin_amdgcn_mfma_f32_32x32x2f32(c4.x, a4.x, BR == 1 && kk == 0 ? zero16 : acc2[mi], 0, 0, 0);
@@ -247,6 +260,7 @@
         if (t < 15) stamp(4 + 4 * t);
 #pragma unroll
         for (int mi = 0; mi < MI; ++mi) {
+            if (GRP) acc[mi] = (acc[mi] + accg[0][mi]) + (accg[GRP ? 1 : 0][mi] + accg[GRP ? 2 : 0][mi]);
             const int m_base = tile_m * BM + wm * (BM / WM) + mi * 32;
             const int o_off = out_offset(m_base);
             float* o_px = p.out + o_off;
@@ -296,6 +310,11 @@
 
 __global__ __launch_bounds__(256, 2) void pgemm_branch_kernel(const GemmParams p) {
     pgemm_body<64, 64, false, false, false, true>(p);
+}
+
+template <int BM, int BN>
+__global__ __launch_bounds__(256, 2) void pgemm_group_kernel(const GemmParams p) {
+    pgemm_body<BM, BN, false, false, false, false, true>(p);
 }
 
 hipError_t launch_pgemm(const GemmParams& p_in, int bm, hipStream_t s) {
@@ -374,4 +393,43 @@
     return hipGetLastError();
 }
 
-}
+hipError_t launch_pgemm_grouped(const float* a, const float* w, float* out, int groups, int rows, int K, int N, int tile, hipStream_t s) {
+    auto mis = [](const void* q) { return (reinterpret_cast<unsigned long long>(q) & 15ull) != 0; };
+    if (!a || !w || !out || mis(a) || mis(w) || mis(out) || groups < 1 || rows < 64 || rows % 64 || rows >= (1 << 16) || K < 32 || K % 32 || N < 64 || N % 64 ||
+        tile < 0 || tile > 3)
+        return hipErrorInvalidValue;
+    if ((long long)groups * rows * K * 4 >= (1ll << 31) || (long long)groups * N * K * 4 >= (1ll << 31) || (long long)groups * rows * N >= (1ll << 31))
+        return hipErrorInvalidValue;
+    if (tile == 0) tile = 1;
+    if (tile != 1 && rows % 128) tile = 1;
+    const int bm = tile == 1 ? 64 : 128, bn = tile == 3 ? 32 : 64;
+    GemmParams p;
+    memset(&p, 0, sizeof(p));
+    p.act = a; p.wgt = w; p.out = out;
+    p.M = groups * rows; p.N = N; p.ktot = K;
+    p.taps = 1; p.kw_taps = 1; p.chunk = K;
+    p.howo = rows; p.wo = rows;
+    p.in_px_stride = K; p.in_row_stride = rows * K; p.in_img_stride = rows * K; p.stride = 1;
+    p.out_px_stride = N; p.out_row_stride = rows * N; p.out_img_stride = rows * N;
+    p.splitk = 1;
+    if (persistent_plan(p) != hipSuccess) return hipErrorInvalidValue;
+    p.tiles_n = N / bn;
+    p.tiles_m = p.M / bm;
+    if (p.tiles_n > 64) return hipErrorInvalidValue;
+    p.grp_tiles = rows / bm;
+    p.grp_wgt_bytes = N * K * 4;
+    p.grp_magic = (unsigned)std::min<unsigned long long>(((1ull << 32) + p.grp_tiles - 1) / p.grp_tiles, 0xffffffffull);
+    const int share = (p.tiles_m + 7) / 8;
+    int lm = 96 / p.tiles_n;
+    static const int lm_force = getenv("PA_PGEMM_GROUP_LM") ? atoi(getenv("PA_PGEMM_GROUP_LM")) : 0;
+    if (lm_force > 0) lm = lm_force;
+    lm = lm < 1 ? 1 : (lm > share ? share : lm);
+    p.pg_per = lm * p.tiles_n;
+    const int grid = p.pg_per * 8;
+    if (tile == 1) hipLaunchKernelGGL((pgemm_group_kernel<64, 64>), dim3(grid), dim3(256), 0, s, p);
+    else if (tile == 2) hipLaunchKernelGGL((pgemm_group_kernel<128, 64>), dim3(grid), dim3(256), 0, s, p);
+    else hipLaunchKernelGGL((pgemm_group_kernel<128, 32>), dim3(grid), dim3(256), 0, s, p);
+    return hipGetLastError();
+}
+
+}
diff --git a/playaid_core_amd/csrc/wino4.hip b/playaid_core_amd/csrc/wino4.hip
--- /dev/null
+++ b/playaid_core_amd/csrc/wino4.hip
@@ -0,0 +1,186 @@
+#include "tile_common.h"
+
+#include <cstdlib>
+
+namespace pa {
+
+namespace {
+
+__device__ __forceinline__ f32x4 w4_fma(float a, f32x4 x, f32x4 y) {
+    return f32x4{__builtin_fmaf(a, x.x, y.x), __builtin_fmaf(a, x.y, y.y), __builtin_fmaf(a, x.z, y.z), __builtin_fmaf(a, x.w, y.w)};
+}
+
+__device__ __forceinline__ void w4_bt(f32x4 (&d)[6]) {
+    const f32x4 t0 = w4_fma(4.f, d[0], w4_fma(-5.f, d[2], d[4]));
+    const f32x4 t5 = w4_fma(4.f, d[1], w4_fma(-5.f, d[3], d[5]));
+    const f32x4 a = w4_fma(-4.f, d[2], d[4]), b = w4_fma(-4.f, d[1], d[3]);
+    const f32x4 c = d[4] - d[2], e = d[3] - d[1];
+    d[0] = t0; d[1] = a + b; d[2] = a - b; d[3] = w4_fma(2.f, e, c); d[4] = w4_fma(-2.f, e, c); d[5] = t5;
+}
+
+__device__ __forceinline__ void w4_at(const f32x4 (&m)[6], f32x4 (&y)[4]) {
+    const f32x4 s = m[1] + m[2], d = m[1] - m[2], u = m[3] + m[4], v = m[3] - m[4];
+    y[0] = (m[0] + s) + u;
+    y[1] = w4_fma(2.f, v, d);
+    y[2] = w4_fma(4.f, u, s);
+    y[3] = w4_fma(8.f, v, d) + m[5];
+}
+
+__global__ __launch_bounds__(64) void wino4_input_kernel(const Wino4Params p) {
+    const int cq_n = p.cin >> 2;
+    const int idx = blockIdx.x * 64 + threadIdx.x;
+    const int row = idx / cq_n, c = (idx - row * cq_n) * 4;
+    if (row >= p.rows) return;
+    float* v = p.v + (size_t)row * p.cin + c;
+    const size_t plane = (size_t)p.rows * p.cin;
+    if (row >= p.n_img) {
+#pragma unroll
+        for (int q = 0; q < 36; ++q) *reinterpret_cast<f32x4*>(v + q * plane) = f32x4{0.f, 0.f, 0.f, 0.f};
+        return;
+    }
+    const float* x = p.act + (size_t)row * p.in_img_stride + c;
+    f32x4 d[6][6];
+#pragma unroll
+    for (int i = 0; i < 6; ++i)
+#pragma unroll
+        for (int j = 0; j < 6; ++j) d[i][j] = *reinterpret_cast<const f32x4*>(x + i * p.in_row_stride + j * p.in_px_stride);
+#pragma unroll
+    for (int j = 0; j < 6; ++j) {
+        f32x4 l[6];
+#pragma unroll
+        for (int i = 0; i < 6; ++i) l[i] = d[i][j];
+        w4_bt(l);
+#pragma unroll
+        for (int i = 0; i < 6; ++i) d[i][j] = l[i];
+    }
+#pragma unroll
+    for (int i = 0; i < 6; ++i) {
+        w4_bt(d[i]);
+#pragma unroll
+        for (int j = 0; j < 6; ++j) *reinterpret_cast<f32x4*>(v + (i * 6 + j) * plane) = d[i][j];
+    }
+}
+
+__global__ __launch_bounds__(64) void wino4_output_kernel(const Wino4Params p) {
+    const int cq_n = p.cout >> 2;
+    const int idx = blockIdx.x * 64 + threadIdx.x;
+    const int row = idx / cq_n, c = (idx - row * cq_n) * 4;
+    if (row >= p.n_img) return;
+    const float* m = p.m + (size_t)row * p.cout + c;
+    const size_t plane = (size_t)p.rows * p.cout;
+    f32x4 t[4][6];
+#pragma unroll
+    for (int j = 0; j < 6; ++j) {
+        f32x4 l[6], y[4];
+#pragma unroll
+        for (int i = 0; i < 6; ++i) l[i] = *reinterpret_cast<const f32x4*>(m + (i * 6 + j) * plane);
+        w4_at(l, y);
+#pragma unroll
+        for (int i = 0; i < 4; ++i) t[i][j] = y[i];
+    }
+    const f32x4 bias4 = p.bias ? *reinterpret_cast<const f32x4*>(p.bias + c) : f32x4{0.f, 0.f, 0.f, 0.f};
+    const size_t o00 = (size_t)row * p.out_img_stride + (size_t)p.out_pad * (p.out_row_stride + p.out_px_stride) + c;
+    f32x4 res4[4][4];
+#pragma unroll
+    for (int oy = 0; oy < 4; ++oy)
+#pragma unroll
+        for (int ox = 0; ox < 4; ++ox)
+            res4[oy][ox] = p.residual ? *reinterpret_cast<const f32x4*>(p.residual + o00 + (size_t)oy * p.out_row_stride + ox * p.out_px_stride)
+                                      : f32x4{0.f, 0.f, 0.f, 0.f};
+#pragma unroll
+    for (int oy = 0; oy < 4; ++oy) {
+        f32x4 y[4];
+        w4_at(t[oy], y);
+#pragma unroll
+        for (int ox = 0; ox < 4; ++ox)
+            *reinterpret_cast<f32x4*>(p.out + o00 + (size_t)oy * p.out_row_stride + ox * p.out_px_stride) = epilogue4(y[ox], bias4, res4[oy][ox], p.relu, p.res_after);
+    }
+}
+
+}
+
+size_t wino4_weight_floats(int cin, int cout) { return (size_t)36 * cin * cout; }
+
+int wino4_rows(int n_img) { return (n_img + 63) / 64 * 64; }
+
+void wino4_transform_weights(const float* w, int cin, int cout, float* u) {
+    static const double Gm[6][3] = {{1.0 / 4, 0, 0},          {-1.0 / 6, -1.0 / 6, -1.0 / 6}, {-1.0 / 6, 1.0 / 6, -1.0 / 6},
+                                    {1.0 / 24, 1.0 / 12, 1.0 / 6}, {1.0 / 24, -1.0 / 12, 1.0 / 6},  {0, 0, 1}};
+    const size_t plane = (size_t)cout * cin;
+    for (int co = 0; co < cout; ++co)
+        for (int ci = 0; ci < cin; ++ci) {
+            double g[3][3], tmp[6][3];
+            for (int ky = 0; ky < 3; ++ky)
+                for (int kx = 0; kx < 3; ++kx) g[ky][kx] = (double)w[((size_t)co * 9 + ky * 3 + kx) * cin + ci];
+            for (int i = 0; i < 6; ++i)
+                for (int kx = 0; kx < 3; ++kx) tmp[i][kx] = Gm[i][0] * g[0][kx] + Gm[i][1] * g[1][kx] + Gm[i][2] * g[2][kx];
+            for (int i = 0; i < 6; ++i)
+                for (int j = 0; j < 6; ++j)
+                    u[(size_t)(i * 6 + j) * plane + (size_t)co * cin + ci] = (float)(tmp[i][0] * Gm[j][0] + tmp[i][1] * Gm[j][1] + tmp[i][2] * Gm[j][2]);
+        }
+}
+
+hipError_t launch_wino4_conv3x3(const Wino4Params& p_in, hipStream_t s) {
+    Wino4Params p = p_in;
+    if (!p.act || !p.wgt || !p.out || !p.v || !p.m || p.n_img < 1 || p.cin < 64 || p.cin % 64 || p.cout < 64 || p.cout % 64 || p.in_px_stride < p.cin ||
+        p.out_px_stride < p.cout || p.out_pad < 0)
+        return hipErrorInvalidValue;
+    auto mis = [](const void* q) { return (reinterpret_cast<unsigned long long>(q) & 15ull) != 0; };
+    if (p.in_px_stride % 4 || p.out_px_stride % 4 || p.in_row_stride % 4 || p.in_img_stride % 4 || p.out_row_stride % 4 || p.out_img_stride % 4 || mis(p.act) ||
+        mis(p.wgt) || mis(p.out) || mis(p.v) || mis(p.m) || (p.bias && mis(p.bias)) || (p.residual && mis(p.residual)))
+        return hipErrorInvalidValue;
+    p.rows = wino4_rows(p.n_img);
+    const long long in_threads = (long long)p.rows * (p.cin / 4), out_threads = (long long)p.n_img * (p.cout / 4);
+    if (in_threads >= (1ll << 31) || out_threads >= (1ll << 31)) return hipErrorInvalidValue;
+    hipLaunchKernelGGL(wino4_input_kernel, dim3((unsigned)((in_threads + 63) / 64)), dim3(64), 0, s, p);
+    static const int tile_env = getenv("PA_WINO_F4_TILE") ? atoi(getenv("PA_WINO_F4_TILE")) : 0;
+    const hipError_t e = launch_pgemm_grouped(p.v, p.wgt, p.m, 36, p.rows, p.cin, p.cout, p.tile ? p.tile : tile_env, s);
+    if (e != hipSuccess) return e;
+    hipLaunchKernelGGL(wino4_output_kernel, dim3((unsigned)((out_threads + 63) / 64)), dim3(64), 0, s, p);
+    return hipGetLastError();
+}
+
+}
+
+#include "../../include/playaid_hip.h"
+
+extern "C" {
+
+size_t pa_wino4_weight_floats(int32_t cin, int32_t cout) {
+    if (cin < 64 || cin % 64 || cout < 64 || cout % 64) return 0;
+    return pa::wino4_weight_floats(cin, cout);
+}
+
+int pa_wino4_transform_weights(const float* w_host, int32_t cin, int32_t cout, float* u_host) {
+    if (!w_host || !u_host || cin < 64 || cin % 64 || cout < 64 || cout % 64) return PA_ERR_INVALID_ARG;
+    pa::wino4_transform_weights(w_host, cin, cout, u_host);
+    return PA_OK;
+}
+
+int pa_wino4_conv3x3(const float* x, const float* u, const float* bias, const float* residual, float* out, int32_t n, int32_t height, int32_t width,
+                     int32_t cin, int32_t cout, int32_t in_px_stride, int32_t out_px_stride, int32_t out_pad, int32_t act, int32_t res_after,
+                     float* scratch, size_t scratch_floats, void* stream) {
+    if (!x || !u || !out || !scratch || n < 1 || height != 4 || width != 4 || out_pad < 0 || act < 0 || act > 2 || cin < 64 || cin % 64 || cout < 64 ||
+        cout % 64 || (reinterpret_cast<unsigned long long>(scratch) & 15ull))
+        return PA_ERR_INVALID_ARG;
+    const size_t rows = (size_t)pa::wino4_rows(n);
+    if (scratch_floats < 36 * rows * ((size_t)cin + cout)) return PA_ERR_INVALID_ARG;
+    pa::Wino4Params p{};
+    p.act = x; p.wgt = u; p.bias = bias; p.residual = residual; p.out = out;
+    p.v = scratch;
+    p.m = scratch + 36 * rows * cin;
+    p.n_img = n; p.cin = cin; p.cout = cout;
+    p.in_px_stride = in_px_stride;
+    p.in_row_stride = 6 * in_px_stride;
+    p.in_img_stride = 6 * p.in_row_stride;
+    p.out_px_stride = out_px_stride;
+    p.out_row_stride = (4 + 2 * out_pad) * out_px_stride;
+    p.out_img_stride = (4 + 2 * out_pad) * p.out_row_stride;
+    p.out_pad = out_pad;
+    p.relu = act;
+    p.res_after = res_after;
+    const hipError_t e = pa::launch_wino4_conv3x3(p, (hipStream_t)stream);
+    return e == hipSuccess ? PA_OK : (e == hipErrorInvalidValue ? PA_ERR_INVALID_ARG : PA_ERR_HIP);
+}
+
+}
diff --git a/playaid_core_amd/wino.py b/playaid_core_amd/wino.py
--- a/playaid_core_amd/wino.py
+++ b/playaid_core_amd/wino.py
@@ -58,3 +58,44 @@
     if rc:
         raise ValueError(f"pa_wino_conv3x3: status {rc}")
     return out
+
+
+
+
+def transform_weights_f4(w_oihw: np.ndarray) -> np.ndarray:
+    lib = _lib.load()
+    w = np.ascontiguousarray(np.asarray(w_oihw, dtype=np.float32).transpose(0, 2, 3, 1))
+    cout, cin = w.shape[0], w.shape[3]
+    n = lib.pa_wino4_weight_floats(cin, cout)
+    if n == 0:
+        raise ValueError("cin and cout must be multiples of 64")
+    u = np.empty(n, dtype=np.float32)
+    rc = lib.pa_wino4_transform_weights(w.ctypes.data_as(C.c_void_p), cin, cout, u.ctypes.data_as(C.c_void_p))
+    if rc:
+        raise ValueError(f"pa_wino4_transform_weights: {rc}")
+    return u.reshape(36, cout, cin)
+
+
+def scratch_floats_f4(n: int, cin: int, cout: int) -> int:
+    return 36 * ((n + 63) // 64 * 64) * (cin + cout)
+
+
+def conv3x3_f4(x_pad: torch.Tensor, u: torch.Tensor, cin: int, cout: int, bias=None, residual=None, out=None, out_pad: int = 1,
+               act: int = 0, res_after: bool = False, out_px_stride: int = None, scratch: torch.Tensor = None) -> torch.Tensor:
+    lib = _lib.load()
+    if x_pad.dtype != torch.float32 or not x_pad.is_cuda or not x_pad.is_contiguous() or x_pad.dim() != 4:
+        raise ValueError("x_pad: contiguous float32[n, 6, 6, C] on the device")
+    n, hp, wp, cs = x_pad.shape
+    h, w = hp - 2, wp - 2
+    ops = out_px_stride or cout
+    if out is None:
+        out = torch.zeros((n, h + 2 * out_pad, w + 2 * out_pad, ops), dtype=torch.float32, device=x_pad.device)
+    if scratch is None:
+        scratch = torch.empty(scratch_floats_f4(n, cin, cout), dtype=torch.float32, device=x_pad.device)
+    ptr = lambda t_: C.c_void_p(t_.data_ptr()) if t_ is not None else C.c_void_p(0)
+    stream = C.c_void_p(torch.cuda.current_stream(x_pad.device).cuda_stream)
+    rc = lib.pa_wino4_conv3x3(ptr(x_pad), ptr(u), ptr(bias), ptr(residual), ptr(out), n, h, w, cin, cout, cs, out.shape[3], out_pad, int(act),
+                              int(bool(res_after)), ptr(scratch), scratch.numel(), stream)
+    if rc:
+        raise ValueError(f"pa_wino4_conv3x3: status {rc}")
+    return out
```

Result: faster. 75120 frames/s (median of 6 runs) (+8.0%).
